# ywq/psnerf

Measured on AMD Instinct MI355X. Metric: ray-samples/sec (train step) on BEAR stage2, higher is better.
Workload: dtype f32

## Files before the change

include/psnerf_hip.h:

```cpp
#ifndef PSNERF_HIP_H
#define PSNERF_HIP_H

#include <stdint.h>

#ifdef __cplusplus
extern "C" {
#endif

#define PSN_OK 0
#define PSN_E_ARG (-1)
#define PSN_E_LAUNCH (-2)
#define PSN_E_UNSUPPORTED (-3)

const char* psn_last_error(void);
int psn_version(void);

int psn_composite_fwd(const float* alpha, const float* rgb, int64_t n_rays, int n_samples, int white_bg,
                      float* weights, float* rgb_out, float* acc_out, void* stream);
int psn_composite_bwd(const float* alpha, const float* rgb, const float* d_rgb_out, const float* d_acc_out,
                      int64_t n_rays, int n_samples, int white_bg, float* d_alpha, float* d_rgb, void* stream);

int psn_pe_encode(const float* x, int64_t n, int n_freqs, float scale, float* out, int out_stride, void* stream);
int psn_app_input(const float* p, const float* v, const float* normal, int64_t n, int n_freqs, float* out, void* stream);

// ... 206 lines not shown

int psn_stage2_loss_fwd(const float* rgb, const float* rgb_gt, int L, const float* alb, const float* alb_j, const float* wgt,
                        const float* wgt_j, int nb, const float* vis, const float* vis_gt, int V, const float* nrm,
                        const float* nrm_gt, const float* nrm_j, const unsigned char* mask_a, const unsigned char* mask_b,
                        int64_t N, int l2, const float* inv_denom, const float* weight, const float* count_dev, float* partial,
                        float* out, void* stream);
int psn_stage2_loss_bwd(const float* g_total, const float* rgb, const float* rgb_gt, int L, float k_rgb, float* d_rgb,
                        const float* alb, const float* alb_j, float k_alb, float* d_alb, float* d_alb_j, const float* wgt,
                        const float* wgt_j, int nb, float k_wgt, float* d_wgt, float* d_wgt_j, const float* vis, const float* vis_gt,
                        int V, float k_vis, float* d_vis, const float* nrm, const float* nrm_gt, const float* nrm_j, float k_nrm,
                        float k_nrmj, float* d_nrm, float* d_nrm_j, const unsigned char* mask_a, const unsigned char* mask_b,
                        int64_t N, int l2, const float* count_dev, void* stream);

int psn_stage1_loss_partial_floats(void);
int psn_stage1_loss_fwd(const float* rgb, const float* rgb_gt, const float* diff, const unsigned char* hit, const float* normal,
                        const float* normal_gt, const unsigned char* norm_mask, const float* acc, const float* mask_gt,
                        const unsigned char* mask_valid, int64_t N, int64_t n_rays, const float* weights, float* partial,
                        float* sums, float* terms, void* stream);
int psn_stage1_loss_terms(const float* sums, int64_t n_rays, const float* weights, int has_grad, int has_norm, int has_mask,
                          float* terms, void* stream);
int psn_stage1_loss_bwd(const float* g_loss, const float* sums, const float* rgb, const float* rgb_gt, const unsigned char* hit,
                        const float* normal, const float* normal_gt, const unsigned char* norm_mask, const float* acc,
                        const float* mask_gt, const unsigned char* mask_valid, int64_t N, int64_t n_rays, const float* weights,
                        float* d_rgb, float* d_diff, float* d_normal, float* d_acc, void* stream);
int psn_surface_normals_fwd(const float* g, const unsigned char* hit, int64_t N, float eps, float* norm_pred, float* diff,
                            void* stream);
int psn_surface_normals_bwd(const float* g, const unsigned char* hit, int64_t N, float eps, const float* d_norm_pred,
                            const float* d_diff, float* dg, void* stream);

#define PSN_PAIR_SUMS_MAX_V 16
#define PSN_PAIR_SUMS_MAX_CHUNKS 2048
int psn_pair_sums(const float* x, int V, int64_t Ns, int C, float* sx, float* sl_part, int* n_chunks, void* stream);
#define PSN_PAIR_GROUP_MAX 4
typedef struct { const float* x; float* sx; float* dWl; float* bias; } PsnPairSumsItem;
int64_t psn_pair_sums_group_workspace(int n_items, int V, int64_t Ns, int C);
int psn_pair_sums_group(int n_items, const PsnPairSumsItem* items, int V, int64_t Ns, int C, const float* pe_l, int64_t ld_pe, int n_pe,
                        int64_t ld_w, float* workspace, void* stream);

#define PSN_ROW_ADAM_MAX 4
typedef struct {
    float* param; const float* grad; float* exp_avg; float* exp_avg_sq;
    int64_t rows; int cols;
    float one_minus_beta1, one_minus_beta2, eps, step_size;
} PsnRowAdamItem;
int psn_row_adam(int n_items, const PsnRowAdamItem* items, const int64_t* idx, int n_idx, void* stream);
int psn_row_adam_dev(int n_items, const PsnRowAdamItem* items, const int64_t* idx, int n_idx, const float* step_sizes_dev, void* stream);

int psn_normalize_rows_fwd(const float* x, int64_t n, float eps, float* y, void* stream);
int psn_normalize_rows_bwd(const float* x, const float* g, int64_t n, float eps, float* dx, void* stream);
int psn_light_rows_fwd(const float* dir_table, const float* int_table, const int64_t* idx, int n_idx, float eps, float* dir_out,
                       float* int_out, void* stream);
int psn_light_rows_bwd(const float* dir_table, const int64_t* idx, int n_idx, int64_t n_rows, float eps, const float* g_dir,
                       const float* g_int, float* d_dir_table, float* d_int_table, void* stream);
int psn_camera_rays(const float* uv, const float* pose, const float* intrinsics, const int64_t* idx, int64_t n, float scale,
                    float* out, void* stream);
int psn_stage1_rays(const float* pix, const float* camera_mat, int k_ld, const float* world_mat, float radius2, int64_t n,
                    float* cam, float* rays, float* far, void* stream);
int psn_surface_points(const float* d_pred, const int* flags, const float* cam, const float* rays, int64_t n, float* d_i,
                       float* dists, unsigned char* obj_mask, float* points, void* stream);
int psn_stage1_targets(const float* pix, int64_t n, int h, int w, const float* img, const float* mask, const float* mask_valid,
                       const float* normal, const float* norm_mask, const float* world_mat, int use_angle, float cos_thresh,
                       float* rgb_gt, float* mask_gt, unsigned char* mask_valid_out, float* normal_gt,
                       unsigned char* norm_mask_out, void* stream);
#define PSN_COPY2D_MAX 24
typedef struct {
    const float* src; int64_t ld_src;
    float* dst; int64_t ld_dst;
    int rows, cols;
} PsnCopy2dItem;
int psn_copy2d_group(int n_items, const PsnCopy2dItem* items, void* stream);
#define PSN_COPY_BYTES_MAX 24
typedef struct { const void* src; void* dst; int64_t n_bytes; int aligned; } PsnCopyBytesItem;
int psn_copy_bytes_group(int n_items, const PsnCopyBytesItem* items, void* stream);
int psn_mask_count(const unsigned char* mask_a, const unsigned char* mask_b, int64_t n, float* out, void* stream);
int psn_surface_index(const unsigned char* mask, int64_t n, int64_t cap, int64_t* idx, float* count, void* stream);
int psn_inverse_index(const int64_t* idx, int64_t ns, int64_t n_pix, int* inv, const float* count, void* stream);
typedef struct {
    const void* images; int image_type; const float* lut;
    const unsigned char* object_mask; const unsigned char* surface_mask;
    const float* points; const float* normal; const float* visibility; const float* vis_plus; const float* light_direction;
    int64_t hw; int width;
    const int64_t* lidx; int n_lights;
    const int64_t* pix; int64_t pix0; int64_t n;
    const int64_t* vidx; int n_vis;
    float* rgb; unsigned char* object_mask_out; unsigned char* surface_mask_out; float* uv; float* points_out; float* normal_out;
    float* visibility_out; float* vis_train_gt; int64_t* sampling_idx_out; float* light_direction_out;
} PsnViewBatch;
int psn_view_batch(const PsnViewBatch* b, void* stream);
#define PSN_ADAM_MAX_SEGS 16
typedef struct {
    int64_t offset, grad_offset, n;
    float neg_step_size;
    float bias_correction2_sqrt;
} PsnAdamSeg;
int psn_adam_flat(float* param, const float* grad, float* exp_avg, float* exp_avg_sq, int n_segs, const PsnAdamSeg* segs,
                  float one_minus_beta1, float beta2, float one_minus_beta2, float eps, void* stream);
int psn_adam_flat_dev(float* param, const float* grad, float* exp_avg, float* exp_avg_sq, int n_segs, const PsnAdamSeg* segs,
                      float one_minus_beta1, float beta2, float one_minus_beta2, float eps, const float* seg_scalars_dev, void* stream);

#define PSN_WN_MAX_ITEMS 16
typedef struct {
    const float* v;
    const float* g;
    float* w;
    const float* dw;
    float* dv;
    float* dg;
    int rows, cols;
    float scale;
} PsnWnItem;
int psn_weight_norm_fwd(int n_items, const PsnWnItem* items, void* stream);
int psn_weight_norm_bwd(int n_items, const PsnWnItem* items, void* stream);

typedef struct {
    int32_t n_hidden;
    int32_t n_out;
    int32_t out_act;
    int32_t reserved;
    uint8_t has_in[PSN_MLP_MAX_LAYERS + 4];
} PsnBf16Desc;

int psn_lowp_pack(const float* W, int64_t ldw, int rows, int cols, int permuted, int n_ot, int ks0, int n_ks, int n_planes,
                  uint16_t* dst, void* stream);
int psn_lowp_pack_bias(const float* V, int64_t n, int n_pieces, uint16_t* dst, void* stream);

int psn_mlp_infer_bf16(const PsnBf16Desc* desc, const uint16_t* packed_w, const float* final_bias, const uint16_t* tab_a,
                       int64_t a_div, int64_t a_mod, const uint16_t* tab_b, int64_t b_div, int64_t b_mod, int64_t n_rows,
                       float* out, void* stream);

int psn_mlp_infer_bf16_grouped(const PsnBf16Desc* desc, const uint16_t* packed_w, const float* final_bias,
                               const uint16_t* tab_a, int64_t rows_per_group, const uint16_t* group_bias, int64_t n_groups,
                               float* out, void* stream);

int psn_mlp_infer_x3_grouped(const PsnBf16Desc* desc, const uint16_t* packed_w, const uint16_t* bias_steps, const float* final_bias,
                             const float* U, int64_t rows_per_group, const float* V, int64_t n_groups, float* out, void* stream);
int psn_mlp_infer_x3_occ(const PsnBf16Desc* desc, const uint16_t* packed_w, const uint16_t* bias_steps, const float* final_bias,
                         const float* points, int64_t n_rows, const long long* n_rows_dev, const int64_t* out_rows, int pe_octaves,
                         float pe_scale, int skip_layer, int pe_first, float* out, void* stream);
int psn_march_sweep_x3(const PsnBf16Desc* desc, const uint16_t* packed_w, const uint16_t* bias_steps, const float* final_bias,
                       const float* origin, const float* dir, const float* far, const float* u, const float* omu, float near,
                       int64_t n_rays, int n_steps, float tau, int pe_octaves, float pe_scale, int skip_layer, int pe_first,
                       int* skip, float* occ, unsigned long long* n_blocks, void* stream);


int psn_sg_shade_fwd(const float* light_dir, const float* view, const float* normal, const float* albedo,
                     const float* weights, const float* lobe, const float* light_int, int int_ch, float light_int_scalar,
                     const float* vis, int L, int64_t Ns, int nb, int specular_rgb, float* rgb, float* spec,
                     void* stream);
int psn_sg_shade_bwd(const float* light_dir, const float* view, const float* normal, const float* albedo,
                     const float* weights, const float* lobe, const float* light_int, float light_int_scalar,
                     const float* vis, int L, int64_t Ns, int nb, int specular_rgb, const float* g_rgb,
                     const float* g_spec, float* d_albedo, float* d_weights, float* d_normal, float* d_vis,
                     float* d_light_dir, float* d_light_int, float* workspace, void* stream);

int psn_mf_shade_fwd(const float* light_dir, const float* view, const float* normal, const float* albedo,
                     const float* rough, const float* light_int, float light_int_scalar, float f0, const float* vis,
                     int L, int64_t Ns, float* rgb, void* stream);
int psn_mf_shade_bwd(const float* light_dir, const float* view, const float* normal, const float* albedo,
                     const float* rough, const float* light_int, float light_int_scalar, float f0, const float* vis,
                     int L, int64_t Ns, const float* g_rgb, float* d_albedo, float* d_rough, float* d_normal,
                     float* d_vis, float* d_light_dir, float* d_light_int, float* workspace, void* stream);

#define PSN_MESH_MAX_RESOLUTION 1024
int psn_mise_collect(unsigned char* flags, int resolution, float box_size, int64_t capacity, int64_t* rows, float* points,
                     long long* count, void* stream);
int psn_mise_refine(const float* grid, unsigned char* flags, unsigned char* vox, int resolution0, int depth, double threshold,
                    long long* pending, void* stream);
int psn_grid_ffill(float* grid, int n, void* stream);
int64_t psn_mc_blocks(int n);
int psn_mc_count(const float* grid, int n, double threshold, unsigned char* code, int* block_v, int* block_t, void* stream);
int psn_mc_emit(const float* grid, int n, double threshold, const unsigned char* code, const int64_t* v_base, const int64_t* t_base,
                int64_t n_vertices, int64_t n_faces, double box_size, int* v_off, double* vertices, int64_t* faces, void* stream);

#define PSN_TRI_GRID_MAX_CELLS_PER_AXIS 256
#define PSN_TRI_GRID_MAX_FACES 2147483646LL
typedef struct {
    double lo[3];
    double hi[3];
    double cell;
    int n[3];
    int max_span;
} PsnTriGrid;
int psn_tri_grid_count(const PsnTriGrid* grid, const double* vertices, const int64_t* faces, int64_t n_faces, int* cell_count,
                       int* over_list, long long* n_over, void* stream);
int psn_tri_grid_fill(const PsnTriGrid* grid, const double* vertices, const int64_t* faces, int64_t n_faces, int* cursor,
                      int64_t n_entries, int* list, void* stream);
int psn_closest_point(const PsnTriGrid* grid, const double* vertices, const int64_t* faces, int64_t n_faces, const int* cell_start,
                      const int* list, const int* over_list, int64_t n_over, const double* points, const int64_t* order,
                      int64_t n_points, double* closest, double* dist, int64_t* tri, long long* n_tests, void* stream);

#define PSN_RAY_FIRST_HIT 0
#define PSN_RAY_ANY_HIT 1
int psn_ray_cast(const PsnTriGrid* grid, const double* vertices, const int64_t* faces, int64_t n_faces, const int* cell_start,
                 const int* list, const int* over_list, int64_t n_over, const double* origins, const double* directions,
                 const int64_t* order, int64_t n_rays, double t_min, double t_max, int mode, double* t, int64_t* tri, double* bary,
                 unsigned char* hit, long long* n_tests, void* stream);

#define PSN_OCC_LOCAL 0
#define PSN_OCC_WORLD 1
#define PSN_OCC_MAX_DIRS 1024
int psn_occlusion_rows(const PsnTriGrid* grid, const double* vertices, const int64_t* faces, int64_t n_faces, const int* cell_start,
                       const int* list, const int* over_list, int64_t n_over, const double* points, const double* normals, int64_t n_rows,
                       const double* table, int n_dirs, int mode, double bias, double t_max, int* hits, int* visible, double* ao,
                       double* bent, int* words, long long* n_tests, void* stream);

#define PSN_CROSSINGS_MAX_POINTS 137438953408LL
int psn_mesh_crossings(const PsnTriGrid* grid, const double* vertices, const int64_t* faces, int64_t n_faces, const int* cell_start,
                       const int* list, const int* over_list, int64_t n_over, const double* points, const int64_t* order,
                       int64_t n_points, int axis, int* above, int* below, int* on, long long* n_tests, void* stream);

#define PSN_CC_MAX_VERTICES 2147483646LL
#define PSN_CC_MAX_FACES 274877906944LL
#define PSN_CC_E_INDEX 1
#define PSN_CC_E_BOUND 2
int psn_cc_label(const int64_t* faces, int64_t n_faces, int64_t n_vertices, int* parent, int* labels, int* status, void* stream);
int psn_cc_stats(const double* vertices, const int64_t* faces, int64_t n_faces, int64_t n_vertices, const int* labels,
                 long long* vertex_count, long long* face_count, double* area, int* status, void* stream);
int psn_cc_flag(const int64_t* faces, int64_t n_faces, int64_t n_vertices, const int* labels, const unsigned char* keep_label,
                unsigned char* face_keep, unsigned char* vertex_keep, void* stream);
int psn_cc_compact(const double* vertices, const void* normals, int normal_bytes, const int64_t* faces, int64_t n_faces,
                   int64_t n_vertices, const unsigned char* face_keep, const unsigned char* vertex_keep, const int64_t* face_pos,
                   const int64_t* vertex_pos, int64_t n_out_faces, int64_t n_out_vertices, double* out_vertices, void* out_normals,
                   int64_t* out_faces, void* stream);

#define PSN_VC_MAX_RESOLUTION 4096
#define PSN_VC_MAX_CLUSTERS 2097151
#define PSN_VC_MAX_FACES 274877906944LL
#define PSN_VC_E_INDEX 1
#define PSN_VC_E_CLUSTER 2
int psn_vc_cell_keys(const double* vertices, int64_t n_vertices, double ox, double oy, double oz, double h, int dx, int dy, int dz,
                     int64_t* keys, void* stream);
int psn_vc_face_keys(const int64_t* faces, int64_t n_faces, int64_t n_vertices, const int64_t* cluster, int64_t* corner_keys,
                     int64_t* face_keys, int64_t* g, int* status, void* stream);
int psn_vc_solve(const double* vertices, const int64_t* faces, int64_t n_faces, int64_t n_vertices, const int64_t* vertex_order,
                 const int64_t* vertex_start, const int64_t* cell_key_sorted, const int64_t* corner_sorted,
                 const int64_t* corner_start, int64_t n_clusters, double ox, double oy, double oz, double h, int dx, int dy, int dz,
                 double regularisation, double* positions, unsigned char* clamped, void* stream);
int psn_vc_face_flags(const double* vertices, const int64_t* faces, int64_t n_faces, int64_t n_vertices, const int64_t* g,
                      const double* positions, int64_t n_clusters, const unsigned char* face_keep, unsigned char* vertex_keep,
                      unsigned char* flipped, void* stream);

#define PSN_IMG_F32 0
#define PSN_IMG_U8 1
#define PSN_IMG_MIN_EXTENT 11
#define PSN_IMG_MAX_EXTENT 16384
#define PSN_IMG_WS_SCALE_SUMS 0
#define PSN_IMG_WS_METRICS 1
#define PSN_IMG_WS_NORMAL_MAE 2
int64_t psn_img_workspace(int which, int B, int H, int W);
int psn_img_scale_sums(const void* pred, const void* gt, int image_type, const unsigned char* mask, int mask_batch, int B, int H, int W,
                       double* partial, double* sums, void* stream);
int psn_img_metrics(const void* pred, const void* gt, int image_type, const unsigned char* mask, int mask_batch, const double* scale, int B,
                    int H, int W, double* partial, double* sums, double* ssim, double* psnr, double* ssim_map, void* stream);
int psn_normal_mae(const float* pred, const float* gt, const unsigned char* mask, int mask_batch, int normalize, int B, int64_t n_pixels,
                   double* partial, double* sums, double* err_map, void* stream);

#define PSN_PS_MAX_LIGHTS 256
#define PSN_PS_MIN_LIGHTS 3
#define PSN_PS_TILE_LIGHTS 96
#define PSN_PS_MAX_PIXELS 1073741824
#define PSN_PS_PATH_AUTO 0
#define PSN_PS_PATH_TILE 1
#define PSN_PS_PATH_REFORM 2
int64_t psn_ps_workspace(int L, int64_t n_pixels);
int psn_ps_normals(const void* images, int image_type, const unsigned char* mask, const double* light_dir, const double* light_int, int L,
                   int64_t n_pixels, double low, double high, double dark, int min_lights, double cond, int path, double* normal,
                   double* albedo, unsigned char* valid, int32_t* kept, void* stream);
int psn_ps_light_intensity(const void* images, int image_type, const double* normal, const double* albedo, const unsigned char* valid,
                           const double* light_dir, int L, int64_t n_pixels, double dark, double bright, double* partial, double* sums,
                           double* intensity, void* stream);
int psn_ps_light_average(const void* images, int image_type, const unsigned char* mask, const double* relat_int, int L, int64_t n_pixels,
                         double* mean, unsigned char* mean_u8, unsigned char* norm_u8, void* stream);

#define PSN_ATLAS_MIN_CELL 4
#define PSN_ATLAS_MAX_SIZE 32768
#define PSN_ATLAS_MAX_CHANNELS 32
int psn_atlas_points(const double* vertices, int64_t n_vertices, const int64_t* faces, int64_t n_faces, const double* vertex_normals, int T,
                     int cell, int64_t f0, int64_t f1, double* points, float* points_f32, double* normals, void* stream);
int psn_atlas_scatter(const float* rows, int C, int T, int cell, int64_t n_faces, int64_t f0, int64_t f1, void* texture, int texture_type,
                      void* stream);
int psn_atlas_fill(float fill, int C, int T, int cell, int64_t n_faces, void* texture, int texture_type, void* stream);
int psn_atlas_sample(const int64_t* face, const double* bary, int64_t n_queries, const float* texture, int C, int T, int cell,
                     int64_t n_faces, double* out, void* stream);

#define PSN_HULL_MAX_RADIUS 64
#define PSN_HULL_VIEW_CHUNK 32
#define PSN_HULL_F32 0
#define PSN_HULL_F64 1
int64_t psn_mask_dilate_workspace(int V, int H, int W);
int psn_mask_dilate(const unsigned char* masks, int V, int H, int W, const int32_t* half_widths, int r, int border, int invert,
                    unsigned long long* workspace, unsigned char* out, void* stream);
int psn_hull_points(const void* points, int point_type, int64_t n_points, const double* views, int V, const unsigned char* masks, int H,
                    int W, unsigned char* keep, int32_t* carved_by, void* stream);
int psn_hull_grid(float* grid, int n, const double* axis, const double* views, int V, const unsigned char* masks, int H, int W, float value,
                  unsigned long long* count, void* stream);

#ifdef __cplusplus
}
#endif
#endif
```

psnerf_amd/csrc/common.h:

```cpp
#pragma once
#include <hip/hip_runtime.h>
#include <stdint.h>
#include <stdio.h>
#include "../../include/psnerf_hip.h"

namespace psn {

void set_error(const char* fmt, ...);

#define PSN_CHECK_ARG(cond, ...)          \
    do {                                  \
        if (!(cond)) {                    \
            psn::set_error(__VA_ARGS__);  \
            return PSN_E_ARG;             \
        }                                 \
    } while (0)

#define PSN_CHECK_LAUNCH(what)                                                   \
    do {                                                                         \
        hipError_t e__ = hipGetLastError();                                      \
        if (e__ != hipSuccess) {                                                 \
            psn::set_error("%s: launch failed: %s", what, hipGetErrorString(e__)); \
            return PSN_E_LAUNCH;                                                 \
        }                                                                        \
    } while (0)

__device__ __forceinline__ void lds_barrier() { asm volatile("s_waitcnt lgkmcnt(0)\n\ts_barrier" ::: "memory"); }


template <int OFF>
__device__ __forceinline__ void lds_dma_16(const void* gbase, unsigned lds, unsigned voff) {
    asm volatile("s_mov_b32 m0, %2\n\ts_nop 0\n\tglobal_load_lds_dwordx4 %0, %1 offset:%3" ::"v"(voff), "s"(gbase), "s"(lds), "n"(OFF));
}
__device__ __forceinline__ unsigned lds_addr(const void* p) {
    return (unsigned)(__UINTPTR_TYPE__)(__attribute__((address_space(3))) const void*)p;
}

typedef float floatx16 __attribute__((ext_vector_type(16)));
typedef float floatx4 __attribute__((ext_vector_type(4)));

__device__ __forceinline__ float relu1(float x) {
    float o;
    asm("v_max_f32 %0, 0, %1" : "=v"(o) : "v"(x));
    return o;
}

__device__ __forceinline__ float exp_neg_abs(float at) {
    const float L2E_HI = 1.44269502162933349609375f;
    const float L2E_LO = 1.925963033500011e-8f;
    float hi = -at * L2E_HI;
    float lo = fmaf(-at, L2E_HI, -hi);
    lo = fmaf(-at, L2E_LO, lo);
    float u = __builtin_amdgcn_exp2f(hi);
    return fmaf(u, lo * 0.693147182464599609375f, u);
}

__device__ __forceinline__ float log1p_unit(float u, float w, float rw) {
    return fmaf(__builtin_amdgcn_logf(w), 0.693147182464599609375f, (u - (w - 1.0f)) * rw);
}

typedef float f32x2 __attribute__((ext_vector_type(2)));
__device__ __forceinline__ f32x2 pk_fma(f32x2 a, f32x2 b, f32x2 c) { return __builtin_elementwise_fma(a, b, c); }
__device__ __forceinline__ f32x2 pk2(float a) { return f32x2{a, a}; }

template <bool WITH_SIG>
__device__ __forceinline__ void softplus100_pair(f32x2 z, f32x2& sp, f32x2& s) {
    const float L2E = 1.44269502162933349609375f;
    const float LN2_HI = 0.693147182464599609375f;
    const float LN2_LO = -1.904654323148236e-9f;
    const float C_HI = 0.00999999977648258209228515625f;
    const float C_LO = 2.2351741811588166e-10f;
    const f32x2 t = z * 100.0f;
    const f32x2 nat = {fminf(t.x, -t.x), fminf(t.y, -t.y)};
    const f32x2 hi = nat * L2E;
    f32x2 r = pk_fma(-hi, pk2(LN2_HI), nat);
    r = pk_fma(-hi, pk2(LN2_LO), r);
    const f32x2 u0 = {__builtin_amdgcn_exp2f(hi.x), __builtin_amdgcn_exp2f(hi.y)};
    const f32x2 u = pk_fma(u0, r, u0);
    const f32x2 w = u + 1.0f;
    const f32x2 lw = {__builtin_amdgcn_logf(w.x), __builtin_amdgcn_logf(w.y)};
    const f32x2 c = w - 1.0f;
    const f32x2 d = u - c;
    f32x2 rw;
    if constexpr (WITH_SIG) {
        const f32x2 r0 = {__builtin_amdgcn_rcpf(w.x), __builtin_amdgcn_rcpf(w.y)};
        rw = pk_fma(pk_fma(-w, r0, pk2(1.0f)), r0, r0);
        const f32x2 ur = u * rw;
        s = f32x2{t.x >= 0.0f ? rw.x : ur.x, t.y >= 0.0f ? rw.y : ur.y};
    } else {
        rw = pk_fma(c, pk_fma(c, pk2(0.5f), pk2(-1.0f)), pk2(1.0f));
    }
    const f32x2 l = pk_fma(lw, pk2(LN2_HI), d * rw);
    const f32x2 zr = {relu1(z.x), relu1(z.y)};
    sp = pk_fma(l, pk2(C_HI), pk_fma(l, pk2(C_LO), zr));
}
__device__ __forceinline__ void softplus100_sig(float z, float& sp, float& s) {
    f32x2 a, b;
    softplus100_pair<true>(f32x2{z, z}, a, b);
    sp = a.x; s = b.x;
}
__device__ __forceinline__ float softplus100(float z) {
    f32x2 a, b;
    softplus100_pair<false>(f32x2{z, z}, a, b);
    return a.x;
}
__device__ __forceinline__ float sigmoidf_(float x) {
    float u = exp_neg_abs(fabsf(x));
    float r = 1.0f / (1.0f + u);
    return x >= 0.0f ? r : u * r;
}

}
```

psnerf_amd/csrc/loss.hip:

```cpp
#include "common.h"

namespace psn {

struct LossArgs {
    const float* rgb; const float* rgb_gt; int L;
    const float* alb; const float* alb_j;
    const float* wgt; const float* wgt_j; int nb;
    const float* vis; const float* vis_gt; int V;
    const float* nrm; const float* nrm_gt; const float* nrm_j;
    const unsigned char* mask_a; const unsigned char* mask_b;
    int64_t N;
    int l2;
    float* partial;
    const float* g_total;
    const float* count_dev;
    float k_rgb, k_alb, k_wgt, k_vis, k_nrm, k_nrmj;
    float* d_rgb; float* d_alb; float* d_alb_j; float* d_wgt; float* d_wgt_j; float* d_vis; float* d_nrm; float* d_nrm_j;
};

__device__ __forceinline__ float img_term(float a, float b, int l2) { const float d = a - b; return l2 ? d * d : fabsf(d); }
__device__ __forceinline__ float img_grad(float a, float b, int l2) {
    const float d = a - b;
    return l2 ? 2.0f * d : (d > 0.0f ? 1.0f : (d < 0.0f ? -1.0f : 0.0f));
}

__global__ __launch_bounds__(256) void stage2_loss_fwd_kernel(LossArgs a) {
    float s[6] = {0.f, 0.f, 0.f, 0.f, 0.f, 0.f};
    const int lc = (a.L + gridDim.y - 1) / gridDim.y;
    const int l0 = blockIdx.y * lc, l1 = min(a.L, l0 + lc);
    for (int64_t n = (int64_t)blockIdx.x * 256 + threadIdx.x; n < a.N; n += (int64_t)gridDim.x * 256) {
        if (!(a.mask_a[n] && a.mask_b[n])) continue;
        if (a.rgb != nullptr) {
#pragma unroll 4
            for (int l = l0; l < l1; ++l) {
                const float* p = a.rgb + ((int64_t)l * a.N + n) * 3;
                const float* q = a.rgb_gt + ((int64_t)l * a.N + n) * 3;
                s[0] += img_term(p[0], q[0], a.l2) + img_term(p[1], q[1], a.l2) + img_term(p[2], q[2], a.l2);
            }
        }
        if (blockIdx.y != 0) continue;
        if (a.alb != nullptr) {
#pragma unroll
            for (int c = 0; c < 3; ++c) s[1] += fabsf(a.alb[n * 3 + c] - a.alb_j[n * 3 + c]);
        }
        if (a.wgt != nullptr) {
            for (int k = 0; k < a.nb; ++k) s[2] += fabsf(a.wgt[n * a.nb + k] - a.wgt_j[n * a.nb + k]);
        }
        if (a.vis != nullptr) {
            for (int v = 0; v < a.V; ++v) s[3] += img_term(a.vis[((int64_t)v * a.N + n) * 3], a.vis_gt[(int64_t)v * a.N + n], a.l2);
        }
        if (a.nrm != nullptr) {
            const float gx = a.nrm_gt[n * 3], gy = a.nrm_gt[n * 3 + 1], gz = a.nrm_gt[n * 3 + 2];
            const float inv = 1.0f / fmaxf(sqrtf(gx * gx + gy * gy + gz * gz), 1e-12f);
            const float dx = a.nrm[n * 3] - gx * inv, dy = a.nrm[n * 3 + 1] - gy * inv, dz = a.nrm[n * 3 + 2] - gz * inv;
            s[4] += dx * dx + dy * dy + dz * dz;
            if (a.nrm_j != nullptr) {
#pragma unroll
                for (int c = 0; c < 3; ++c) s[5] += fabsf(a.nrm[n * 3 + c] - a.nrm_j[n * 3 + c]);
            }
        }
    }
    __shared__ float red[4][6];
#pragma unroll
    for (int i = 0; i < 6; ++i) {
        float v = s[i];
#pragma unroll
        for (int o = 32; o > 0; o >>= 1) v += __shfl_xor(v, o, 64);
        if ((threadIdx.x & 63) == 0) red[threadIdx.x >> 6][i] = v;
    }
    __syncthreads();
    if (threadIdx.x < 6)
        a.partial[((int64_t)blockIdx.y * gridDim.x + blockIdx.x) * 6 + threadIdx.x] = (red[0][threadIdx.x] + red[1][threadIdx.x]) + (red[2][threadIdx.x] + red[3][threadIdx.x]);
}

struct LossScale { float inv_denom[6]; float weight[6]; const float* count_dev; };
__global__ __launch_bounds__(256) void stage2_loss_final_kernel(const float* __restrict__ partial, int blocks, LossScale sc,
                                                               float* __restrict__ out) {
    __shared__ float red[32][8];
    const int i = threadIdx.x & 7, j = threadIdx.x >> 3;
    float s = 0.f;
    if (i < 6)
        for (int b = j; b < blocks; b += 32) s += partial[(int64_t)b * 6 + i];
    red[j][i] = s;
    __syncthreads();
    if (threadIdx.x < 8) {
        float tot = 0.f;
#pragma unroll
        for (int k = 0; k < 32; ++k) tot += red[k][threadIdx.x];
        const float cnt = sc.count_dev != nullptr ? sc.count_dev[0] : 1.0f;
        const float term = (threadIdx.x < 6 && cnt > 0.0f) ? tot * sc.inv_denom[threadIdx.x] / cnt : 0.f;
        if (threadIdx.x < 6) out[threadIdx.x] = term;
        float w = threadIdx.x < 6 ? sc.weight[threadIdx.x] * term : 0.f;
#pragma unroll
        for (int o = 4; o > 0; o >>= 1) w += __shfl_xor(w, o, 64);
        if (threadIdx.x == 0) out[6] = w;
    }
}

__global__ __launch_bounds__(256) void pair_sums_kernel(const float* __restrict__ x, int V, int64_t Ns, int C, int rows_per_block,
                                                        float* __restrict__ sx, float* __restrict__ sl_part) {
    const int cg = threadIdx.x & 63, rl = threadIdx.x >> 6;
    const int64_t n0 = (int64_t)blockIdx.x * rows_per_block, n1 = min(Ns, n0 + rows_per_block);
    const bool live = 4 * cg < C;
    float4 sl[PSN_PAIR_SUMS_MAX_V];
#pragma unroll
    for (int v = 0; v < PSN_PAIR_SUMS_MAX_V; ++v) sl[v] = make_float4(0.f, 0.f, 0.f, 0.f);
    if (live) {
        for (int64_t n = n0 + rl; n < n1; n += 4) {
            float4 acc = make_float4(0.f, 0.f, 0.f, 0.f);
#pragma unroll
            for (int v = 0; v < PSN_PAIR_SUMS_MAX_V; ++v) {
                if (v < V) {
                    const float4 t = *reinterpret_cast<const float4*>(x + ((int64_t)v * Ns + n) * C + 4 * cg);
                    acc.x += t.x; acc.y += t.y; acc.z += t.z; acc.w += t.w;
                    sl[v].x += t.x; sl[v].y += t.y; sl[v].z += t.z; sl[v].w += t.w;
                }
            }
            *reinterpret_cast<float4*>(sx + n * C + 4 * cg) = acc;
        }
#pragma unroll
        for (int v = 0; v < PSN_PAIR_SUMS_MAX_V; ++v)
            if (v < V) *reinterpret_cast<float4*>(sl_part + (((int64_t)blockIdx.x * 4 + rl) * V + v) * C + 4 * cg) = sl[v];
    }
}

struct PairGroupArgs { PsnPairSumsItem it[PSN_PAIR_GROUP_MAX]; int V; int64_t Ns; int C; int rows_per_block; int chunks; float* part;
                       const float* pe_l; int64_t ld_pe; int n_pe; int64_t ld_w;
                       int slices; float* part2; };
__global__ __launch_bounds__(256) void pair_group_sums_kernel(PairGroupArgs a) {
    const PsnPairSumsItem it = a.it[blockIdx.y];
    const int V = a.V, C = a.C;
    const int64_t Ns = a.Ns;
    const int cg = threadIdx.x & 63, rl = threadIdx.x >> 6;
    const int64_t n0 = (int64_t)blockIdx.x * a.rows_per_block, n1 = min(Ns, n0 + a.rows_per_block);
    const bool live = 4 * cg < C;
    float4 sl[PSN_PAIR_SUMS_MAX_V];
#pragma unroll
    for (int v = 0; v < PSN_PAIR_SUMS_MAX_V; ++v) sl[v] = make_float4(0.f, 0.f, 0.f, 0.f);
    if (live) {
        for (int64_t n = n0 + rl; n < n1; n += 4) {
            float4 acc = make_float4(0.f, 0.f, 0.f, 0.f);
#pragma unroll
            for (int v = 0; v < PSN_PAIR_SUMS_MAX_V; ++v) {
                if (v < V) {
                    const float4 t = *reinterpret_cast<const float4*>(it.x + ((int64_t)v * Ns + n) * C + 4 * cg);
                    acc.x += t.x; acc.y += t.y; acc.z += t.z; acc.w += t.w;
                    sl[v].x += t.x; sl[v].y += t.y; sl[v].z += t.z; sl[v].w += t.w;
                }
            }
            *reinterpret_cast<float4*>(it.sx + n * C + 4 * cg) = acc;
        }
    }
    __shared__ float4 red[3][64];
    float* dst = a.part + (((int64_t)blockIdx.y * a.chunks + blockIdx.x) * V) * C;
#pragma unroll
    for (int v = 0; v < PSN_PAIR_SUMS_MAX_V; ++v) {
        if (v < V) {
            __syncthreads();
            if (rl > 0) red[rl - 1][cg] = sl[v];
            __syncthreads();
            if (rl == 0 && live) {
                float4 t = sl[v];
#pragma unroll
                for (int q = 0; q < 3; ++q) { const float4 o = red[q][cg]; t.x += o.x; t.y += o.y; t.z += o.z; t.w += o.w; }
                *reinterpret_cast<float4*>(dst + (int64_t)v * C + 4 * cg) = t;
            }
        }
    }
}
__global__ __launch_bounds__(1024) void pair_group_final_kernel(PairGroupArgs a) {
    const PsnPairSumsItem it = a.it[blockIdx.y];
    const int V = a.V, C = a.C;
    const int c0 = blockIdx.x * 64;
    const int cl = threadIdx.x & 63, v = threadIdx.x >> 6;
    __shared__ float dzl[PSN_PAIR_SUMS_MAX_V][64];
    __shared__ float pel[PSN_PAIR_SUMS_MAX_V][64];
    int ch = 0, ch_end = a.chunks;
    if (a.slices > 1) {
        const int per = (a.chunks + a.slices - 1) / a.slices;
        ch = blockIdx.z * per;
        ch_end = min(a.chunks, ch + per);
    }
    float s = 0.0f;
    if (v < V && c0 + cl < C) {
        const float* p = a.part + ((int64_t)blockIdx.y * a.chunks * V + v) * C + c0 + cl;
        const int64_t step = (int64_t)V * C;
        for (; ch + 4 <= ch_end; ch += 4) {
            const float t0 = p[(int64_t)ch * step], t1 = p[(int64_t)(ch + 1) * step], t2 = p[(int64_t)(ch + 2) * step], t3 = p[(int64_t)(ch + 3) * step];
            s += t0; s += t1; s += t2; s += t3;
        }
        for (; ch < ch_end; ++ch) s += p[(int64_t)ch * step];
        if (a.slices > 1) a.part2[(((int64_t)blockIdx.y * a.slices + blockIdx.z) * V + v) * C + c0 + cl] = s;
    }
    if (a.slices > 1) return;
    dzl[v][cl] = s;
    pel[v][cl] = (v < V && cl < a.n_pe) ? a.pe_l[(int64_t)v * a.ld_pe + cl] : 0.0f;
    __syncthreads();
    for (int e = threadIdx.x; e < 64 * a.n_pe; e += 1024) {
        const int c = e / a.n_pe, k = e - c * a.n_pe;
        if (c0 + c < C) {
            float w = 0.0f;
            for (int u = 0; u < V; ++u) w += dzl[u][c] * pel[u][k];
            it.dWl[(int64_t)(c0 + c) * a.ld_w + k] = w;
        }
    }
    if (it.bias != nullptr && threadIdx.x < 64 && c0 + (int)threadIdx.x < C) {
        float b = 0.0f;
        for (int u = 0; u < V; ++u) b += dzl[u][threadIdx.x];
        it.bias[c0 + threadIdx.x] = b;
    }
}

__global__ __launch_bounds__(256) void stage2_loss_bwd_kernel(LossArgs a) {
    float g = a.g_total[0];
    if (a.count_dev != nullptr) {
        const float cnt = a.count_dev[0];
        g = cnt > 0.0f ? g / cnt : 0.0f;
    }
    const int lc = (a.L + gridDim.y - 1) / gridDim.y;
    const int l0 = blockIdx.y * lc, l1 = min(a.L, l0 + lc);
    for (int64_t n = (int64_t)blockIdx.x * 256 + threadIdx.x; n < a.N; n += (int64_t)gridDim.x * 256) {
        const bool m = a.mask_a[n] && a.mask_b[n];
        if (a.d_rgb != nullptr) {
            const float k = g * a.k_rgb;
#pragma unroll 4
            for (int l = l0; l < l1; ++l) {
                const int64_t o = ((int64_t)l * a.N + n) * 3;
#pragma unroll
                for (int c = 0; c < 3; ++c) a.d_rgb[o + c] = m ? k * img_grad(a.rgb[o + c], a.rgb_gt[o + c], a.l2) : 0.f;
            }
        }
        if (blockIdx.y != 0) continue;
        if (a.d_alb != nullptr) {
            const float k = g * a.k_alb;
#pragma unroll
            for (int c = 0; c < 3; ++c) {
                const float v = m ? k * img_grad(a.alb[n * 3 + c], a.alb_j[n * 3 + c], 0) : 0.f;
                a.d_alb[n * 3 + c] = v;
                a.d_alb_j[n * 3 + c] = -v;
            }
        }
        if (a.d_wgt != nullptr) {
            const float k = g * a.k_wgt;
            for (int q = 0; q < a.nb; ++q) {
                const float v = m ? k * img_grad(a.wgt[n * a.nb + q], a.wgt_j[n * a.nb + q], 0) : 0.f;
                a.d_wgt[n * a.nb + q] = v;
                a.d_wgt_j[n * a.nb + q] = -v;
            }
        }
        if (a.d_vis != nullptr) {
            const float k = g * a.k_vis;
            for (int v = 0; v < a.V; ++v) {
                const int64_t o = ((int64_t)v * a.N + n) * 3;
                a.d_vis[o] = m ? k * img_grad(a.vis[o], a.vis_gt[(int64_t)v * a.N + n], a.l2) : 0.f;
                a.d_vis[o + 1] = 0.f;
                a.d_vis[o + 2] = 0.f;
            }
        }
        if (a.d_nrm != nullptr) {
            float gn[3] = {0.f, 0.f, 0.f}, gj[3] = {0.f, 0.f, 0.f};
            if (m) {
                const float gx = a.nrm_gt[n * 3], gy = a.nrm_gt[n * 3 + 1], gz = a.nrm_gt[n * 3 + 2];
                const float inv = 1.0f / fmaxf(sqrtf(gx * gx + gy * gy + gz * gz), 1e-12f);
                const float t[3] = {gx * inv, gy * inv, gz * inv};
#pragma unroll
                for (int c = 0; c < 3; ++c) gn[c] = g * a.k_nrm * 2.0f * (a.nrm[n * 3 + c] - t[c]);
                if (a.nrm_j != nullptr) {
#pragma unroll
                    for (int c = 0; c < 3; ++c) {
                        const float v = g * a.k_nrmj * img_grad(a.nrm[n * 3 + c], a.nrm_j[n * 3 + c], 0);
                        gn[c] += v;
                        gj[c] = -v;
                    }
                }
            }
#pragma unroll
            for (int c = 0; c < 3; ++c) {
                a.d_nrm[n * 3 + c] = gn[c];
                if (a.d_nrm_j != nullptr) a.d_nrm_j[n * 3 + c] = gj[c];
            }
        }
    }
}

constexpr int kLossBlocksX = 256, kLossChunksY = 8;

}

extern "C" int psn_stage2_loss_fwd(const float* rgb, const float* rgb_gt, int L, const float* alb, const float* alb_j,
                                   const float* wgt, const float* wgt_j, int nb, const float* vis, const float* vis_gt, int V,
                                   const float* nrm, const float* nrm_gt, const float* nrm_j, const unsigned char* mask_a,
                                   const unsigned char* mask_b, int64_t N, int l2, const float* inv_denom, const float* weight,
                                   const float* count_dev, float* partial, float* out, void* stream) {
    using namespace psn;
    PSN_CHECK_ARG(mask_a && mask_b && partial && out && inv_denom && weight, "stage2_loss_fwd: null pointer");
    PSN_CHECK_ARG((rgb == nullptr || rgb_gt) && (alb == nullptr || alb_j) && (wgt == nullptr || (wgt_j && nb > 0)) &&
                  (vis == nullptr || vis_gt) && (nrm == nullptr || nrm_gt), "stage2_loss_fwd: incomplete term");
    LossArgs a = {};
    a.rgb = rgb; a.rgb_gt = rgb_gt; a.L = L; a.alb = alb; a.alb_j = alb_j; a.wgt = wgt; a.wgt_j = wgt_j; a.nb = nb;
    a.vis = vis; a.vis_gt = vis_gt; a.V = V; a.nrm = nrm; a.nrm_gt = nrm_gt; a.nrm_j = nrm_j; a.mask_a = mask_a; a.mask_b = mask_b;
    a.N = N; a.l2 = l2; a.partial = partial;
    int bx = (int)((N + 255) / 256);
    if (bx > kLossBlocksX) bx = kLossBlocksX;
    if (bx < 1) bx = 1;
    const int by = (rgb != nullptr && L >= 2 * kLossChunksY) ? kLossChunksY : 1;
    hipLaunchKernelGGL(stage2_loss_fwd_kernel, dim3(bx, by), dim3(256), 0, (hipStream_t)stream, a);
    PSN_CHECK_LAUNCH("stage2_loss_fwd");
    LossScale sc;
    for (int i = 0; i < 6; ++i) { sc.inv_denom[i] = inv_denom[i]; sc.weight[i] = weight[i]; }
    sc.count_dev = count_dev;
    hipLaunchKernelGGL(stage2_loss_final_kernel, dim3(1), dim3(256), 0, (hipStream_t)stream, partial, bx * by, sc, out);
    PSN_CHECK_LAUNCH("stage2_loss_fwd (final)");
    return PSN_OK;
}

extern "C" int psn_stage2_loss_bwd(const float* g_total, const float* rgb, const float* rgb_gt, int L, float k_rgb, float* d_rgb,
                                   const float* alb, const float* alb_j, float k_alb, float* d_alb, float* d_alb_j,
                                   const float* wgt, const float* wgt_j, int nb, float k_wgt, float* d_wgt, float* d_wgt_j,
                                   const float* vis, const float* vis_gt, int V, float k_vis, float* d_vis,
                                   const float* nrm, const float* nrm_gt, const float* nrm_j, float k_nrm, float k_nrmj, float* d_nrm,
                                   float* d_nrm_j, const unsigned char* mask_a, const unsigned char* mask_b, int64_t N, int l2,
                                   const float* count_dev, void* stream) {
    using namespace psn;
    PSN_CHECK_ARG(g_total && mask_a && mask_b, "stage2_loss_bwd: null pointer");
    LossArgs a = {};
    a.g_total = g_total; a.count_dev = count_dev; a.rgb = rgb; a.rgb_gt = rgb_gt; a.L = L; a.k_rgb = k_rgb; a.d_rgb = d_rgb;
    a.alb = alb; a.alb_j = alb_j; a.k_alb = k_alb; a.d_alb = d_alb; a.d_alb_j = d_alb_j;
    a.wgt = wgt; a.wgt_j = wgt_j; a.nb = nb; a.k_wgt = k_wgt; a.d_wgt = d_wgt; a.d_wgt_j = d_wgt_j;
    a.vis = vis; a.vis_gt = vis_gt; a.V = V; a.k_vis = k_vis; a.d_vis = d_vis;
    a.nrm = nrm; a.nrm_gt = nrm_gt; a.nrm_j = nrm_j; a.k_nrm = k_nrm; a.k_nrmj = k_nrmj; a.d_nrm = d_nrm; a.d_nrm_j = d_nrm_j;
    a.mask_a = mask_a; a.mask_b = mask_b; a.N = N; a.l2 = l2;
    PSN_CHECK_ARG((d_rgb == nullptr || (rgb && rgb_gt)) && (d_alb == nullptr || (alb && alb_j && d_alb_j)) &&
                  (d_wgt == nullptr || (wgt && wgt_j && d_wgt_j)) && (d_vis == nullptr || (vis && vis_gt)) &&
                  (d_nrm == nullptr || (nrm && nrm_gt)), "stage2_loss_bwd: incomplete term");
    if (N <= 0) return PSN_OK;
    int64_t blocks = (N + 255) / 256;
    if (blocks > 1024) blocks = 1024;
    const int by = (d_rgb != nullptr && L >= 2 * kLossChunksY) ? kLossChunksY : 1;
    hipLaunchKernelGGL(stage2_loss_bwd_kernel, dim3((unsigned)blocks, by), dim3(256), 0, (hipStream_t)stream, a);
    PSN_CHECK_LAUNCH("stage2_loss_bwd");
    return PSN_OK;
}

namespace psn {
struct RowAdamArgs { PsnRowAdamItem it[PSN_ROW_ADAM_MAX]; const int64_t* idx; int n_idx; int n;
                     const float* dev; };
__global__ __launch_bounds__(256) void row_adam_kernel(RowAdamArgs a) {
    const int item = blockIdx.y;
    if (item >= a.n) return;
    PsnRowAdamItem it = a.it[item];
    if (a.dev != nullptr) it.step_size = a.dev[item];
    const int64_t r = (int64_t)blockIdx.x * 256 + threadIdx.x;
    __shared__ int64_t sidx[256];
    bool touched = false;
    for (int i0 = 0; i0 < a.n_idx; i0 += 256) {
        const int m = a.n_idx - i0 < 256 ? a.n_idx - i0 : 256;
        __syncthreads();
        if ((int)threadIdx.x < m) sidx[threadIdx.x] = a.idx[i0 + threadIdx.x];
        __syncthreads();
        for (int j = 0; j < m; ++j) touched = touched || sidx[j] == r;
    }
    if (r >= it.rows || !touched) return;
    for (int c = 0; c < it.cols; ++c) {
        const int64_t e = r * it.cols + c;
        const float g = it.grad[e];
        float m = it.exp_avg[e], v = it.exp_avg_sq[e];
        m += (g - m) * it.one_minus_beta1;
        v += (g * g - v) * it.one_minus_beta2;
        it.exp_avg[e] = m;
        it.exp_avg_sq[e] = v;
        it.param[e] += (m / (sqrtf(v) + it.eps)) * (-it.step_size);
    }
}
}

static int row_adam_impl(int n_items, const PsnRowAdamItem* items, const int64_t* idx, int n_idx, const float* step_sizes_dev, void* stream) {
    using namespace psn;
    PSN_CHECK_ARG(items && (idx || n_idx == 0) && n_items >= 1 && n_items <= PSN_ROW_ADAM_MAX && n_idx >= 0, "row_adam: bad arguments");
    RowAdamArgs a = {};
    a.dev = step_sizes_dev;
    int64_t max_rows = 0;
    for (int i = 0; i < n_items; ++i) {
        PSN_CHECK_ARG(items[i].param && items[i].grad && items[i].exp_avg && items[i].exp_avg_sq && items[i].rows >= 0 && items[i].cols >= 1,
                      "row_adam: item %d", i);
        a.it[i] = items[i];
        if (items[i].rows > max_rows) max_rows = items[i].rows;
    }
    a.idx = idx; a.n_idx = n_idx; a.n = n_items;
    if (max_rows <= 0 || n_idx == 0) return PSN_OK;
    hipLaunchKernelGGL(row_adam_kernel, dim3((unsigned)((max_rows + 255) / 256), n_items), dim3(256), 0, (hipStream_t)stream, a);
    PSN_CHECK_LAUNCH("row_adam");
    return PSN_OK;
}

extern "C" int psn_row_adam(int n_items, const PsnRowAdamItem* items, const int64_t* idx, int n_idx, void* stream) {
    return row_adam_impl(n_items, items, idx, n_idx, nullptr, stream);
}

extern "C" int psn_row_adam_dev(int n_items, const PsnRowAdamItem* items, const int64_t* idx, int n_idx, const float* step_sizes_dev,
                                void* stream) {
    PSN_CHECK_ARG(step_sizes_dev != nullptr, "row_adam_dev: step_sizes_dev is required");
    return row_adam_impl(n_items, items, idx, n_idx, step_sizes_dev, stream);
}

constexpr int kPairSlices = 32;

extern "C" int64_t psn_pair_sums_group_workspace(int n_items, int V, int64_t Ns, int C) {
    int rows = 16;
    int64_t chunks = (Ns + rows - 1) / rows;
    while (chunks > PSN_PAIR_SUMS_MAX_CHUNKS) { rows *= 2; chunks = (Ns + rows - 1) / rows; }
    return (int64_t)n_items * ((chunks > 0 ? chunks : 1) + kPairSlices) * V * C;
}

extern "C" int psn_pair_sums_group(int n_items, const PsnPairSumsItem* items, int V, int64_t Ns, int C, const float* pe_l, int64_t ld_pe,
                                   int n_pe, int64_t ld_w, float* workspace, void* stream) {
    using namespace psn;
    PSN_CHECK_ARG(items && pe_l && workspace && n_items >= 1 && n_items <= PSN_PAIR_GROUP_MAX, "pair_sums_group: bad arguments (n_items=%d)", n_items);
    PSN_CHECK_ARG(V >= 1 && V <= PSN_PAIR_SUMS_MAX_V && C >= 4 && C <= 256 && C % 4 == 0 && Ns >= 0, "pair_sums_group: V=%d C=%d", V, C);
    PSN_CHECK_ARG(n_pe >= 1 && n_pe <= 64 && ld_pe >= n_pe && ld_w >= n_pe, "pair_sums_group: n_pe=%d", n_pe);
    PairGroupArgs a = {};
    for (int i = 0; i < n_items; ++i) {
        PSN_CHECK_ARG(items[i].x && items[i].sx && items[i].dWl && ((((uintptr_t)items[i].x | (uintptr_t)items[i].sx)) & 15) == 0, "pair_sums_group: item %d", i);
        a.it[i] = items[i];
    }
    int rows = 16;
    int64_t chunks = (Ns + rows - 1) / rows;
    while (chunks > PSN_PAIR_SUMS_MAX_CHUNKS) { rows *= 2; chunks = (Ns + rows - 1) / rows; }
    a.V = V; a.Ns = Ns; a.C = C; a.rows_per_block = rows; a.chunks = (int)chunks; a.part = workspace;
    a.pe_l = pe_l; a.ld_pe = ld_pe; a.n_pe = n_pe; a.ld_w = ld_w;
    PSN_CHECK_ARG((((uintptr_t)workspace) & 15) == 0, "pair_sums_group: workspace must be 16-byte aligned");
    if (chunks > 0) {
        hipLaunchKernelGGL(pair_group_sums_kernel, dim3((unsigned)chunks, n_items), dim3(256), 0, (hipStream_t)stream, a);
        PSN_CHECK_LAUNCH("pair_sums_group (sums)");
    }
    if (chunks > 128) {
        a.slices = kPairSlices;
        a.part2 = workspace + (int64_t)n_items * chunks * V * C;
        hipLaunchKernelGGL(pair_group_final_kernel, dim3((unsigned)((C + 63) / 64), n_items, kPairSlices), dim3(1024), 0, (hipStream_t)stream, a);
        PSN_CHECK_LAUNCH("pair_sums_group (slices)");
        a.part = a.part2; a.chunks = kPairSlices; a.slices = 1; a.part2 = nullptr;
    }
    hipLaunchKernelGGL(pair_group_final_kernel, dim3((unsigned)((C + 63) / 64), n_items), dim3(1024), 0, (hipStream_t)stream, a);
    PSN_CHECK_LAUNCH("pair_sums_group (final)");
    return PSN_OK;
}

extern "C" int psn_pair_sums(const float* x, int V, int64_t Ns, int C, float* sx, float* sl_part, int* n_chunks, void* stream) {
    using namespace psn;
    PSN_CHECK_ARG(x && sx && sl_part && n_chunks, "pair_sums: null pointer");
    PSN_CHECK_ARG(V >= 1 && V <= PSN_PAIR_SUMS_MAX_V && C >= 1 && C <= 256 && Ns >= 0, "pair_sums: V=%d C=%d (V <= %d, C <= 256)", V, C, PSN_PAIR_SUMS_MAX_V);
    PSN_CHECK_ARG(C % 4 == 0 && (((uintptr_t)x | (uintptr_t)sx | (uintptr_t)sl_part) & 15) == 0, "pair_sums: C must be a multiple of 4, buffers 16-byte aligned");
    int rows = 32;
    int64_t chunks = (Ns + rows - 1) / rows;
    while (chunks * 4 > PSN_PAIR_SUMS_MAX_CHUNKS) { rows *= 2; chunks = (Ns + rows - 1) / rows; }
    *n_chunks = (int)chunks * 4;
    if (Ns <= 0) return PSN_OK;
    hipLaunchKernelGGL(pair_sums_kernel, dim3((unsigned)chunks), dim3(256), 0, (hipStream_t)stream, x, V, Ns, C, rows, sx, sl_part);
    PSN_CHECK_LAUNCH("pair_sums");
    return PSN_OK;
}
```

psnerf_amd/csrc/shade.hip:

```cpp
#include "common.h"

namespace psn {

constexpr int kShadeThreads = 64;

constexpr int kMaxBasis = 9;

struct ShadeArgs {
    const float* light_dir;
    const float* view;
    const float* normal;
    const float* albedo;
    const float* weights;
    const float* lobe;
    const float* light_int;
    int int_ch;
    float light_int_scalar;
    const float* vis;
    int L, nb, specular_rgb;
    int64_t Ns;
};

__device__ __forceinline__ float wave_sum_f(float v) {
#pragma unroll
    for (int d = 32; d >= 1; d >>= 1) v += __shfl_xor(v, d, 64);
    return v;
}

struct PointCtx {
    float v[3], n[3], alb[3];
    float w[3][kMaxBasis];
    float lam[kMaxBasis];
};

__device__ __forceinline__ void load_point(const ShadeArgs& a, int64_t n, bool ok, PointCtx& p) {
    const int nw = a.specular_rgb ? 3 * a.nb : a.nb;
#pragma unroll
    for (int c = 0; c < 3; ++c) {
        p.v[c] = ok ? a.view[n * 3 + c] : 0.f;
        p.n[c] = ok ? a.normal[n * 3 + c] : 0.f;
        p.alb[c] = ok ? a.albedo[n * 3 + c] : 0.f;
    }
#pragma unroll
    for (int k = 0; k < kMaxBasis; ++k) {
        p.lam[k] = k < a.nb ? fmaxf(a.lobe[k], 0.0f) : 0.0f;
#pragma unroll
        for (int c = 0; c < 3; ++c) {
            float wv = 0.f;
            if (ok && k < a.nb) wv = a.specular_rgb ? a.weights[n * nw + c * a.nb + k] : a.weights[n * nw + k];
            p.w[c][k] = wv;
        }
    }
}

struct Fwd {
    float h[3], inv_norm, hn, D[kMaxBasis], s[3], brdf[3], cosv, vcl, I[3], pre[3];
};

__device__ __forceinline__ void shade_one(const ShadeArgs& a, const PointCtx& p, const float l[3], const float I[3],
                                          float vis, bool has_vis, Fwd& f) {
    float u0 = l[0] + p.v[0], u1 = l[1] + p.v[1], u2 = l[2] + p.v[2];
    float nrm = sqrtf(u0 * u0 + u1 * u1 + u2 * u2);
    float den = fmaxf(nrm, 1e-12f);
    f.inv_norm = 1.0f / den;
    f.h[0] = u0 / den;
    f.h[1] = u1 / den;
    f.h[2] = u2 / den;
    f.hn = f.h[0] * p.n[0] + f.h[1] * p.n[1] + f.h[2] * p.n[2];
    float t = f.hn - 1.0f;
    float s0 = 0.f, s1 = 0.f, s2 = 0.f;
#pragma unroll
    for (int k = 0; k < kMaxBasis; ++k) {
        float d = (k < a.nb) ? expf(p.lam[k] * t) : 0.0f;
        f.D[k] = d;
        s0 += p.w[0][k] * d;
        s1 += p.w[1][k] * d;
        s2 += p.w[2][k] * d;
    }
    f.s[0] = s0;
    f.s[1] = a.specular_rgb ? s1 : s0;
    f.s[2] = a.specular_rgb ? s2 : s0;
    f.cosv = l[0] * p.n[0] + l[1] * p.n[1] + l[2] * p.n[2];
    f.vcl = has_vis ? fminf(fmaxf(vis, 0.0f), 1.0f) : 1.0f;
#pragma unroll
    for (int c = 0; c < 3; ++c) {
        f.I[c] = I[c];
        f.brdf[c] = p.alb[c] + fmaxf(f.s[c], 0.0f);
        float x = f.brdf[c] * I[c] * f.cosv;
        if (has_vis) x = x * f.vcl;
        f.pre[c] = x;
    }
}

constexpr int kSgPhases = 4;
__global__ __launch_bounds__(kShadeThreads * kSgPhases) void sg_shade_fwd_kernel(ShadeArgs a, float* __restrict__ rgb, float* __restrict__ spec) {
    const int64_t n = (int64_t)blockIdx.x * kShadeThreads + (threadIdx.x & (kShadeThreads - 1));
    const int phase = threadIdx.x / kShadeThreads;
    const bool ok = n < a.Ns;
    PointCtx p;
    load_point(a, n, ok, p);
    const bool has_vis = a.vis != nullptr;
    const int sc = a.specular_rgb ? 3 : 1;
    for (int l = phase; l < a.L; l += kSgPhases) {
        float ld[3] = {a.light_dir[l * 3 + 0], a.light_dir[l * 3 + 1], a.light_dir[l * 3 + 2]};
        float I[3];
#pragma unroll
        for (int c = 0; c < 3; ++c)
            I[c] = a.light_int != nullptr ? a.light_int[l * a.int_ch + (a.int_ch == 3 ? c : 0)] : a.light_int_scalar;
        const int64_t row = (int64_t)l * a.Ns + n;
        float vis = (has_vis && ok) ? a.vis[row] : 1.0f;
        Fwd f;
        shade_one(a, p, ld, I, vis, has_vis, f);
        if (ok) {
#pragma unroll
            for (int c = 0; c < 3; ++c) rgb[row * 3 + c] = fminf(fmaxf(f.pre[c], 0.0f), 1.0f);
            if (a.specular_rgb) {
#pragma unroll
                for (int c = 0; c < 3; ++c) spec[row * 3 + c] = fmaxf(f.s[c], 0.0f);
            } else {
                spec[row] = fmaxf(f.s[0], 0.0f);
            }
        }
    }
    (void)sc;
}

__global__ __launch_bounds__(kShadeThreads * kSgPhases) void sg_shade_bwd_kernel(ShadeArgs a, const float* __restrict__ g_rgb,
                                                           const float* __restrict__ g_spec,
                                                           float* __restrict__ d_albedo, float* __restrict__ d_weights,
                                                           float* __restrict__ d_normal, float* __restrict__ d_vis,
                                                           float* __restrict__ d_light_partial) {
    const int64_t n = (int64_t)blockIdx.x * kShadeThreads + (threadIdx.x & (kShadeThreads - 1));
    const int phase = threadIdx.x / kShadeThreads;
    const bool ok = n < a.Ns;
    const int lane = threadIdx.x & 63;
    PointCtx p;
    load_point(a, n, ok, p);
    const bool has_vis = a.vis != nullptr;
    float dalb[3] = {0.f, 0.f, 0.f}, dn[3] = {0.f, 0.f, 0.f};
    float dw[3][kMaxBasis];
#pragma unroll
    for (int c = 0; c < 3; ++c)
#pragma unroll
        for (int k = 0; k < kMaxBasis; ++k) dw[c][k] = 0.f;

    for (int l = phase; l < a.L; l += kSgPhases) {
        float ld[3] = {a.light_dir[l * 3 + 0], a.light_dir[l * 3 + 1], a.light_dir[l * 3 + 2]};
        float I[3];
#pragma unroll
        for (int c = 0; c < 3; ++c)
            I[c] = a.light_int != nullptr ? a.light_int[l * a.int_ch + (a.int_ch == 3 ? c : 0)] : a.light_int_scalar;
        const int64_t row = (int64_t)l * a.Ns + n;
        float vis = (has_vis && ok) ? a.vis[row] : 1.0f;
        Fwd f;
        shade_one(a, p, ld, I, vis, has_vis, f);
        float dl[3] = {0.f, 0.f, 0.f}, dI = 0.f, dcos = 0.f, dvcl = 0.f, ds[3];
        if (ok) {
#pragma unroll
            for (int c = 0; c < 3; ++c) {
                float g = g_rgb[row * 3 + c];
                float gp = (f.pre[c] >= 0.0f && f.pre[c] <= 1.0f) ? g : 0.0f;
                float dbrdf = gp * I[c] * f.cosv * f.vcl;
                dI += gp * f.brdf[c] * f.cosv * f.vcl;
                dcos += gp * f.brdf[c] * I[c] * f.vcl;
                dvcl += gp * f.brdf[c] * I[c] * f.cosv;
                dalb[c] += dbrdf;
                float dspec = dbrdf;
                if (g_spec != nullptr) dspec += a.specular_rgb ? g_spec[row * 3 + c] : (c == 0 ? g_spec[row] : 0.0f);
                ds[c] = f.s[c] >= 0.0f ? dspec : 0.0f;
            }
            if (!a.specular_rgb) {
                ds[0] = ds[0] + ds[1] + ds[2];
                ds[1] = 0.f;
                ds[2] = 0.f;
            }
            float dhn = 0.f;
#pragma unroll
            for (int k = 0; k < kMaxBasis; ++k) {
                float dD = ds[0] * p.w[0][k] + ds[1] * p.w[1][k] + ds[2] * p.w[2][k];
                dhn += dD * p.lam[k] * f.D[k];
                dw[0][k] += ds[0] * f.D[k];
                dw[1][k] += ds[1] * f.D[k];
                dw[2][k] += ds[2] * f.D[k];
            }
            float dh[3];
#pragma unroll
            for (int c = 0; c < 3; ++c) {
                dh[c] = dhn * p.n[c];
                dn[c] += dhn * f.h[c] + dcos * ld[c];
                dl[c] = dcos * p.n[c];
            }
            float hd = f.h[0] * dh[0] + f.h[1] * dh[1] + f.h[2] * dh[2];
#pragma unroll
            for (int c = 0; c < 3; ++c) dl[c] += (dh[c] - f.h[c] * hd) * f.inv_norm;
            if (d_vis != nullptr) d_vis[row] = (vis >= 0.0f && vis <= 1.0f) ? dvcl : 0.0f;
        }
        float r0 = wave_sum_f(dl[0]), r1 = wave_sum_f(dl[1]), r2 = wave_sum_f(dl[2]), r3 = wave_sum_f(dI);
        if (lane == 0) *reinterpret_cast<float4*>(d_light_partial + ((int64_t)blockIdx.x * a.L + l) * 4) = make_float4(r0, r1, r2, r3);
    }
    __shared__ float pred[kSgPhases - 1][6 + 3 * kMaxBasis][kShadeThreads];
    if (phase > 0) {
#pragma unroll
        for (int c = 0; c < 3; ++c) {
            pred[phase - 1][c][lane] = dalb[c];
            pred[phase - 1][3 + c][lane] = dn[c];
        }
#pragma unroll
        for (int c = 0; c < 3; ++c)
#pragma unroll
            for (int k = 0; k < kMaxBasis; ++k) pred[phase - 1][6 + c * kMaxBasis + k][lane] = dw[c][k];
    }
    __syncthreads();
    if (phase == 0) {
#pragma unroll
        for (int c = 0; c < 3; ++c) {
            dalb[c] = (dalb[c] + pred[0][c][lane]) + (pred[1][c][lane] + pred[2][c][lane]);
            dn[c] = (dn[c] + pred[0][3 + c][lane]) + (pred[1][3 + c][lane] + pred[2][3 + c][lane]);
        }
#pragma unroll
        for (int c = 0; c < 3; ++c)
#pragma unroll
            for (int k = 0; k < kMaxBasis; ++k)
                dw[c][k] = (dw[c][k] + pred[0][6 + c * kMaxBasis + k][lane]) + (pred[1][6 + c * kMaxBasis + k][lane] + pred[2][6 + c * kMaxBasis + k][lane]);
    }
    if (ok && phase == 0) {
        const int nw = a.specular_rgb ? 3 * a.nb : a.nb;
#pragma unroll
        for (int c = 0; c < 3; ++c) {
            d_albedo[n * 3 + c] = dalb[c];
            d_normal[n * 3 + c] = dn[c];
        }
#pragma unroll
        for (int k = 0; k < kMaxBasis; ++k) {
            if (k < a.nb) {
                if (a.specular_rgb) {
#pragma unroll
                    for (int c = 0; c < 3; ++c) d_weights[n * nw + c * a.nb + k] = dw[c][k];
                } else {
                    d_weights[n * nw + k] = dw[0][k];
                }
            }
        }
    }
}

__global__ __launch_bounds__(256) void sg_light_reduce_kernel(const float* __restrict__ partial, int n_blocks, int L,
                                                              float* __restrict__ d_light_dir,
                                                              float* __restrict__ d_light_int) {
    __shared__ float red[3][64];
    const int i = blockIdx.x * 64 + (threadIdx.x & 63), ph = threadIdx.x >> 6;
    float s = 0.f;
    if (i < L * 4)
        for (int b = ph; b < n_blocks; b += 4) s += partial[(int64_t)b * L * 4 + i];
    if (ph > 0) red[ph - 1][threadIdx.x & 63] = s;
    __syncthreads();
    if (ph > 0 || i >= L * 4) return;
    s = (s + red[0][threadIdx.x]) + (red[1][threadIdx.x] + red[2][threadIdx.x]);
    const int l = i >> 2, c = i & 3;
    if (c < 3) d_light_dir[l * 3 + c] = s;
    else if (d_light_int != nullptr) d_light_int[l] = s;
}

struct MfArgs {
    const float* light_dir;
    const float* view;
    const float* normal;
    const float* albedo;
    const float* rough;
    const float* light_int;
    float light_int_scalar, f0;
    const float* vis;
    int L;
    int64_t Ns;
};

__device__ __forceinline__ float dnn(float x, float y) {
    float a = x / (y + 1e-6f);
    return (isinf(a) || isnan(a)) ? 0.0f : a;
}
__device__ __forceinline__ bool dnn_ok(float x, float y) {
    float a = x / (y + 1e-6f);
    return !(isinf(a) || isnan(a));
}
__device__ __forceinline__ void normalize_eps(const float x[3], float eps, float out[3], float& inv) {
    float n = sqrtf(x[0] * x[0] + x[1] * x[1] + x[2] * x[2]);
    float d = fmaxf(n, eps);
    inv = 1.0f / d;
    out[0] = x[0] / d;
    out[1] = x[1] / d;
    out[2] = x[2] / d;
}
__device__ __forceinline__ void normalize_bwd(const float y[3], float inv, bool clamped, const float dy[3], float dx[3]) {
    if (clamped) {
        dx[0] = dy[0] * inv; dx[1] = dy[1] * inv; dx[2] = dy[2] * inv;
    } else {
        float yd = y[0] * dy[0] + y[1] * dy[1] + y[2] * dy[2];
        dx[0] = (dy[0] - y[0] * yd) * inv;
        dx[1] = (dy[1] - y[1] * yd) * inv;
        dx[2] = (dy[2] - y[2] * yd) * inv;
    }
}

struct MfFwd {
    float lh[3], inv_l, hh[3], inv_h, cm, cv, lhh, ln, a2, F, D, G, fgd, den2, mf, cosv, vcl;
    float t_m, den_d, t_v_raw, t_v, sq, den_g, chi_d, chi_g;
    bool cl_l, cl_h, ok_tm, ok_d, ok_tv, ok_g, ok_mf;
};

__device__ __forceinline__ void mf_one(const float l[3], const float vh[3], const float nh[3], const float nraw[3],
                                       float rough, float f0, float vis, bool has_vis, MfFwd& f) {
    const float PI = 3.14159265358979323846f;
    normalize_eps(l, 1e-6f, f.lh, f.inv_l);
    f.cl_l = sqrtf(l[0] * l[0] + l[1] * l[1] + l[2] * l[2]) < 1e-6f;
    float u[3] = {f.lh[0] + vh[0], f.lh[1] + vh[1], f.lh[2] + vh[2]};
    normalize_eps(u, 1e-6f, f.hh, f.inv_h);
    f.cl_h = sqrtf(u[0] * u[0] + u[1] * u[1] + u[2] * u[2]) < 1e-6f;
    f.lhh = f.lh[0] * f.hh[0] + f.lh[1] * f.hh[1] + f.lh[2] * f.hh[2];
    float om = 1.0f - f.lhh;
    f.F = f0 + (1.0f - f0) * (om * om * om * om * om);
    float alpha = rough * rough;
    f.a2 = alpha * alpha;
    f.cm = f.hh[0] * nh[0] + f.hh[1] * nh[1] + f.hh[2] * nh[2];
    f.chi_d = f.cm > 0.0f ? 1.0f : 0.0f;
    float cm2 = f.cm * f.cm;
    f.ok_tm = dnn_ok(1.0f - cm2, cm2);
    f.t_m = dnn(1.0f - cm2, cm2);
    float q = f.a2 + f.t_m;
    f.den_d = PI * (cm2 * cm2) * (q * q);
    f.ok_d = dnn_ok(f.a2 * f.chi_d, f.den_d);
    f.D = dnn(f.a2 * f.chi_d, f.den_d);
    f.cv = nh[0] * vh[0] + nh[1] * vh[1] + nh[2] * vh[2];
    float hv = f.hh[0] * vh[0] + f.hh[1] * vh[1] + f.hh[2] * vh[2];
    f.chi_g = dnn(hv, f.cv) > 0.0f ? 1.0f : 0.0f;
    float cv2 = fminf(fmaxf(f.cv * f.cv, 0.0f), 1.0f);
    f.ok_tv = dnn_ok(1.0f - cv2, cv2);
    f.t_v_raw = dnn(1.0f - cv2, cv2);
    f.t_v = fmaxf(f.t_v_raw, 0.0f);
    f.sq = sqrtf(1.0f + f.a2 * f.t_v);
    f.den_g = 1.0f + f.sq;
    f.ok_g = dnn_ok(f.chi_g * 2.0f, f.den_g);
    f.G = dnn(f.chi_g * 2.0f, f.den_g);
    f.ln = f.lh[0] * nh[0] + f.lh[1] * nh[1] + f.lh[2] * nh[2];
    f.den2 = 4.0f * fabsf(f.ln) * fabsf(f.cv);
    f.fgd = f.F * f.G * f.D;
    f.ok_mf = dnn_ok(f.fgd, f.den2);
    f.mf = dnn(f.fgd, f.den2);
    f.cosv = l[0] * nraw[0] + l[1] * nraw[1] + l[2] * nraw[2];
    f.vcl = has_vis ? fminf(fmaxf(vis, 0.0f), 1.0f) : 1.0f;
}

__global__ __launch_bounds__(kShadeThreads) void mf_shade_fwd_kernel(MfArgs a, float* __restrict__ rgb) {
    const int64_t n = (int64_t)blockIdx.x * kShadeThreads + threadIdx.x;
    const bool ok = n < a.Ns;
    float v[3], nr[3], alb[3], vh[3], nh[3], inv;
#pragma unroll
    for (int c = 0; c < 3; ++c) {
        v[c] = ok ? a.view[n * 3 + c] : 1.f;
        nr[c] = ok ? a.normal[n * 3 + c] : 1.f;
        alb[c] = ok ? a.albedo[n * 3 + c] : 0.f;
    }
    const float rough = ok ? a.rough[n] : 0.5f;
    normalize_eps(v, 1e-6f, vh, inv);
    normalize_eps(nr, 1e-6f, nh, inv);
    const bool has_vis = a.vis != nullptr;
    for (int l = 0; l < a.L; ++l) {
        float ld[3] = {a.light_dir[l * 3 + 0], a.light_dir[l * 3 + 1], a.light_dir[l * 3 + 2]};
        float I = a.light_int != nullptr ? a.light_int[l] : a.light_int_scalar;
        const int64_t row = (int64_t)l * a.Ns + n;
        float vis = (has_vis && ok) ? a.vis[row] : 1.0f;
        MfFwd f;
        mf_one(ld, vh, nh, nr, rough, a.f0, vis, has_vis, f);
        if (ok) {
#pragma unroll
            for (int c = 0; c < 3; ++c) {
                float x = (f.mf + alb[c] / 3.14159265358979323846f) * I * f.cosv;
                if (has_vis) x = x * f.vcl;
                rgb[row * 3 + c] = fminf(fmaxf(x, 0.0f), 1.0f);
            }
        }
    }
}

__global__ __launch_bounds__(kShadeThreads) void mf_shade_bwd_kernel(MfArgs a, const float* __restrict__ g_rgb,
                                                           float* __restrict__ d_albedo, float* __restrict__ d_rough,
                                                           float* __restrict__ d_normal, float* __restrict__ d_vis,
                                                           float* __restrict__ d_light_partial) {
    const float PI = 3.14159265358979323846f;
    const int64_t n = (int64_t)blockIdx.x * kShadeThreads + threadIdx.x;
    const bool ok = n < a.Ns;
    const int lane = threadIdx.x & 63;
    float v[3], nr[3], alb[3], vh[3], nh[3], inv_v, inv_n;
#pragma unroll
    for (int c = 0; c < 3; ++c) {
        v[c] = ok ? a.view[n * 3 + c] : 1.f;
        nr[c] = ok ? a.normal[n * 3 + c] : 1.f;
        alb[c] = ok ? a.albedo[n * 3 + c] : 0.f;
// ... 9 lines not shown
        float I = a.light_int != nullptr ? a.light_int[l] : a.light_int_scalar;
        const int64_t row = (int64_t)l * a.Ns + n;
        float vis = (has_vis && ok) ? a.vis[row] : 1.0f;
        MfFwd f;
        mf_one(ld, vh, nh, nr, rough, a.f0, vis, has_vis, f);
        float dl[3] = {0.f, 0.f, 0.f}, dI = 0.f;
        if (ok) {
            float dmf = 0.f, dcos = 0.f, dvcl = 0.f;
#pragma unroll
            for (int c = 0; c < 3; ++c) {
                float brdf = f.mf + alb[c] / PI;
                float pre = brdf * I * f.cosv;
                if (has_vis) pre = pre * f.vcl;
                float g = g_rgb[row * 3 + c];
                float gp = (pre >= 0.0f && pre <= 1.0f) ? g : 0.0f;
                float dbrdf = gp * I * f.cosv * f.vcl;
                dI += gp * brdf * f.cosv * f.vcl;
                dcos += gp * brdf * I * f.vcl;
                dvcl += gp * brdf * I * f.cosv;
                dalb[c] += dbrdf / PI;
                dmf += dbrdf;
            }
            float dfgd = 0.f, dden2 = 0.f;
            if (f.ok_mf) {
                float r = 1.0f / (f.den2 + 1e-6f);
                dfgd = dmf * r;
                dden2 = -dmf * f.fgd * r * r;
            }
            float dF = dfgd * f.G * f.D, dG = dfgd * f.F * f.D, dD = dfgd * f.F * f.G;
            float sgn_ln = f.ln > 0.f ? 1.f : (f.ln < 0.f ? -1.f : 0.f);
            float sgn_cv = f.cv > 0.f ? 1.f : (f.cv < 0.f ? -1.f : 0.f);
            float dln = dden2 * 4.0f * sgn_ln * fabsf(f.cv);
            float dcv = dden2 * 4.0f * fabsf(f.ln) * sgn_cv;
            float dlhh = dF * (-5.0f) * (1.0f - a.f0) * ((1.0f - f.lhh) * (1.0f - f.lhh) * (1.0f - f.lhh) * (1.0f - f.lhh));
            float dcm = 0.f, da2_l = 0.f;
            if (f.ok_d) {
                float r = 1.0f / (f.den_d + 1e-6f);
                float dden_d = -dD * f.a2 * f.chi_d * r * r;
                da2_l += dD * f.chi_d * r;
                float cm2 = f.cm * f.cm;
                float q = f.a2 + f.t_m;
                float dq = dden_d * PI * cm2 * cm2 * 2.0f * q;
                float dcm2 = dden_d * PI * 2.0f * cm2 * q * q;
                da2_l += dq;
                if (f.ok_tm) {
                    float rr = 1.0f / (cm2 + 1e-6f);
                    dcm2 += dq * (-(rr) - (1.0f - cm2) * rr * rr);
                }
                dcm += dcm2 * 2.0f * f.cm;
            }
            if (f.ok_g) {
                float r = 1.0f / (f.den_g + 1e-6f);
                float dden_g = -dG * 2.0f * f.chi_g * r * r;
                float dsq = dden_g;
                float dinner = f.sq > 0.f ? dsq * 0.5f / f.sq : 0.f;
                da2_l += dinner * f.t_v;
                float dtv = dinner * f.a2;
                if (f.t_v_raw >= 0.0f && f.ok_tv) {
                    float c2 = f.cv * f.cv;
                    if (c2 >= 0.0f && c2 <= 1.0f) {
                        float cv2 = fminf(fmaxf(c2, 0.0f), 1.0f);
                        float rr = 1.0f / (cv2 + 1e-6f);
                        float dcv2 = dtv * (-(rr) - (1.0f - cv2) * rr * rr);
                        dcv += dcv2 * 2.0f * f.cv;
                    }
                }
            }
            da2 += da2_l;
            float dhh[3], dlh[3];
#pragma unroll
            for (int c = 0; c < 3; ++c) {
                dnh[c] += dcm * f.hh[c] + dcv * vh[c] + dln * f.lh[c];
                dhh[c] = dcm * nh[c] + dlhh * f.lh[c];
                dlh[c] = dlhh * f.hh[c] + dln * nh[c];
                dnraw[c] += dcos * ld[c];
                dl[c] = dcos * nr[c];
            }
            float du[3];
            normalize_bwd(f.hh, f.inv_h, f.cl_h, dhh, du);
#pragma unroll
            for (int c = 0; c < 3; ++c) dlh[c] += du[c];
            float dlraw[3];
            normalize_bwd(f.lh, f.inv_l, f.cl_l, dlh, dlraw);
#pragma unroll
            for (int c = 0; c < 3; ++c) dl[c] += dlraw[c];
            if (d_vis != nullptr) d_vis[row] = (vis >= 0.0f && vis <= 1.0f) ? dvcl : 0.0f;
        }
        float r0 = wave_sum_f(dl[0]), r1 = wave_sum_f(dl[1]), r2 = wave_sum_f(dl[2]), r3 = wave_sum_f(dI);
        if (lane == 0) *reinterpret_cast<float4*>(d_light_partial + ((int64_t)blockIdx.x * a.L + l) * 4) = make_float4(r0, r1, r2, r3);
    }
    if (ok) {
        float dn_from_nh[3];
        normalize_bwd(nh, inv_n, cl_n, dnh, dn_from_nh);
#pragma unroll
        for (int c = 0; c < 3; ++c) {
            d_albedo[n * 3 + c] = dalb[c];
            d_normal[n * 3 + c] = dnraw[c] + dn_from_nh[c];
        }
        d_rough[n] = da2 * 4.0f * rough * rough * rough;
    }
}

static int fill_args(ShadeArgs& a, const float* light_dir, const float* view, const float* normal, const float* albedo,
                     const float* weights, const float* lobe, const float* light_int, int int_ch, float light_int_scalar,
                     const float* vis, int L, int64_t Ns, int nb, int specular_rgb) {
    PSN_CHECK_ARG(light_dir && view && normal && albedo && weights && lobe, "sg_shade: null pointer");
    PSN_CHECK_ARG(L >= 1 && Ns >= 0 && nb >= 1 && nb <= kMaxBasis, "sg_shade: L=%d nb=%d", L, nb);
    a.light_dir = light_dir; a.view = view; a.normal = normal; a.albedo = albedo; a.weights = weights; a.lobe = lobe;
    PSN_CHECK_ARG(int_ch == 1 || int_ch == 3, "sg_shade: light intensity must have 1 or 3 channels");
    a.light_int = light_int; a.int_ch = int_ch; a.light_int_scalar = light_int_scalar; a.vis = vis; a.L = L; a.Ns = Ns; a.nb = nb;
    a.specular_rgb = specular_rgb ? 1 : 0;
    return PSN_OK;
}

}

extern "C" int psn_sg_shade_fwd(const float* light_dir, const float* view, const float* normal, const float* albedo,
                                const float* weights, const float* lobe, const float* light_int, int int_ch,
                                float light_int_scalar, const float* vis, int L, int64_t Ns, int nb, int specular_rgb,
                                float* rgb, float* spec, void* stream) {
    using namespace psn;
    ShadeArgs a;
    int rc = fill_args(a, light_dir, view, normal, albedo, weights, lobe, light_int, int_ch, light_int_scalar, vis, L, Ns, nb, specular_rgb);
    if (rc) return rc;
    PSN_CHECK_ARG(rgb && spec, "sg_shade_fwd: null output");
    if (Ns == 0) return PSN_OK;
    hipLaunchKernelGGL(sg_shade_fwd_kernel, dim3((unsigned)((Ns + kShadeThreads - 1) / kShadeThreads)), dim3(kShadeThreads * kSgPhases), 0, (hipStream_t)stream, a, rgb, spec);
    PSN_CHECK_LAUNCH("sg_shade_fwd");
    return PSN_OK;
}

extern "C" int psn_sg_shade_bwd(const float* light_dir, const float* view, const float* normal, const float* albedo,
                                const float* weights, const float* lobe, const float* light_int,
                                float light_int_scalar, const float* vis, int L, int64_t Ns, int nb, int specular_rgb,
                                const float* g_rgb, const float* g_spec, float* d_albedo, float* d_weights,
                                float* d_normal, float* d_vis, float* d_light_dir, float* d_light_int,
                                float* workspace, void* stream) {
    using namespace psn;
    ShadeArgs a;
    int rc = fill_args(a, light_dir, view, normal, albedo, weights, lobe, light_int, 1, light_int_scalar, vis, L, Ns, nb, specular_rgb);
    if (rc) return rc;
    PSN_CHECK_ARG(g_rgb && d_albedo && d_weights && d_normal && d_light_dir && workspace, "sg_shade_bwd: null pointer");
    if (Ns == 0) return PSN_OK;
    const int n_blocks = (int)((Ns + kShadeThreads - 1) / kShadeThreads);
    hipLaunchKernelGGL(sg_shade_bwd_kernel, dim3(n_blocks), dim3(kShadeThreads * kSgPhases), 0, (hipStream_t)stream, a, g_rgb, g_spec, d_albedo,
                       d_weights, d_normal, d_vis, workspace);
    PSN_CHECK_LAUNCH("sg_shade_bwd");
    hipLaunchKernelGGL(sg_light_reduce_kernel, dim3((L * 4 + 63) / 64), dim3(256), 0, (hipStream_t)stream, workspace,
                       n_blocks, L, d_light_dir, d_light_int);
    PSN_CHECK_LAUNCH("sg_shade_bwd light reduce");
    return PSN_OK;
}

extern "C" int psn_mf_shade_fwd(const float* light_dir, const float* view, const float* normal, const float* albedo,
                                const float* rough, const float* light_int, float light_int_scalar, float f0,
                                const float* vis, int L, int64_t Ns, float* rgb, void* stream) {
    using namespace psn;
    PSN_CHECK_ARG(light_dir && view && normal && albedo && rough && rgb, "mf_shade_fwd: null pointer");
    PSN_CHECK_ARG(L >= 1 && Ns >= 0, "mf_shade_fwd: L=%d", L);
    if (Ns == 0) return PSN_OK;
    MfArgs a{light_dir, view, normal, albedo, rough, light_int, light_int_scalar, f0, vis, L, Ns};
    hipLaunchKernelGGL(mf_shade_fwd_kernel, dim3((unsigned)((Ns + kShadeThreads - 1) / kShadeThreads)), dim3(kShadeThreads), 0, (hipStream_t)stream, a, rgb);
    PSN_CHECK_LAUNCH("mf_shade_fwd");
    return PSN_OK;
}

extern "C" int psn_mf_shade_bwd(const float* light_dir, const float* view, const float* normal, const float* albedo,
                                const float* rough, const float* light_int, float light_int_scalar, float f0,
                                const float* vis, int L, int64_t Ns, const float* g_rgb, float* d_albedo,
                                float* d_rough, float* d_normal, float* d_vis, float* d_light_dir, float* d_light_int,
                                float* workspace, void* stream) {
    using namespace psn;
    PSN_CHECK_ARG(light_dir && view && normal && albedo && rough && g_rgb && d_albedo && d_rough && d_normal &&
                  d_light_dir && workspace, "mf_shade_bwd: null pointer");
    PSN_CHECK_ARG(L >= 1 && Ns >= 0, "mf_shade_bwd: L=%d", L);
    if (Ns == 0) return PSN_OK;
    MfArgs a{light_dir, view, normal, albedo, rough, light_int, light_int_scalar, f0, vis, L, Ns};
    const int n_blocks = (int)((Ns + kShadeThreads - 1) / kShadeThreads);
    hipLaunchKernelGGL(mf_shade_bwd_kernel, dim3(n_blocks), dim3(kShadeThreads), 0, (hipStream_t)stream, a, g_rgb, d_albedo, d_rough,
                       d_normal, d_vis, workspace);
    PSN_CHECK_LAUNCH("mf_shade_bwd");
    hipLaunchKernelGGL(sg_light_reduce_kernel, dim3((L * 4 + 63) / 64), dim3(256), 0, (hipStream_t)stream, workspace,
                       n_blocks, L, d_light_dir, d_light_int);
    PSN_CHECK_LAUNCH("mf_shade_bwd light reduce");
    return PSN_OK;
}
```

psnerf_amd/hip.py:

```python
import ctypes
import os

import torch

from . import cabi

_HERE = os.path.dirname(os.path.abspath(__file__))
LIB_PATH = os.path.join(_HERE, 'libpsnerf_hip.so')

if not os.path.exists(LIB_PATH):
    raise ImportError(
        'psnerf_amd: %s is missing. Build it with `python -m psnerf_amd.build` (hipcc, gfx950). '
        'There is no fallback path.' % LIB_PATH)
_lib = ctypes.CDLL(LIB_PATH)

HEADER_PATH = os.path.join(_HERE, '..', 'include', 'psnerf_hip.h')
if not os.path.exists(HEADER_PATH):
    raise ImportError('psnerf_amd: %s is missing: the binding is derived from it. There is no fallback path.' % HEADER_PATH)

_constants, _structs, SIGNATURES = cabi.parse(HEADER_PATH)
globals().update({_k[len('PSN_'):]: _v for _k, _v in _constants.items()})
globals().update(_structs)
MAX_LAYERS = MLP_MAX_LAYERS
for _name, (_res, _args) in SIGNATURES.items():
# ... 1061 lines not shown
        _check(_lib.psn_weight_norm_bwd(n, ctypes.addressof(arr), _stream()), 'weight_norm_bwd')
    return dvs, dgs


def lowp_pack(W, permuted, n_ot, ks0, n_ks, dst, planes=1):
    assert W.dim() == 2 and W.stride(1) == 1 and W.is_cuda and W.dtype == torch.float32
    assert dst.dtype == torch.bfloat16 and dst.is_contiguous() and dst.numel() == n_ks * n_ot * planes * 512
    _check(_lib.psn_lowp_pack(W.data_ptr(), W.stride(0), W.shape[0], W.shape[1], int(permuted), n_ot, ks0, n_ks, planes,
                              dst.data_ptr(), _stream()), 'lowp_pack')


def lowp_pack_bias(V, pieces, dst=None):
    assert V.is_cuda and V.dtype == torch.float32 and V.is_contiguous() and V.dim() == 2 and V.shape[1] == 256
    if dst is None:
        dst = torch.empty(V.shape[0], 4096, device=V.device, dtype=torch.bfloat16)
    assert dst.dtype == torch.bfloat16 and dst.is_contiguous() and dst.numel() == V.shape[0] * 4096
    _check(_lib.psn_lowp_pack_bias(V.data_ptr(), V.shape[0], pieces, dst.data_ptr(), _stream()), 'lowp_pack_bias')
    return dst


def _bf16_stream(t, name):
    if not (t.is_cuda and t.dtype == torch.bfloat16 and t.is_contiguous()):
        raise RuntimeError('%s: must be a contiguous bfloat16 HIP tensor' % name)
    return t.data_ptr()


def _n_in(desc):
    return sum(1 for l in range(desc.n_hidden) if desc.has_in[l])


def _bf16_table(t, name):
    if t is not None and (t.dim() != 2 or t.shape[1] != 64):
        raise RuntimeError('%s: must be a contiguous [n, 64] bfloat16 HIP tensor' % name)
    return _tptr(t, name, torch.bfloat16, allow_none=True)


def mlp_infer_bf16(desc, packed_w, final_bias, tab_a, a_div, a_mod, tab_b, b_div, b_mod, n_rows, out=None):
    if out is None:
        out = torch.empty(n_rows, desc.n_out, device=packed_w.device, dtype=torch.float32)
    assert packed_w.dtype == torch.bfloat16 and packed_w.is_cuda and packed_w.is_contiguous()
    assert final_bias.numel() == 32
    ptrs = (_tptr(final_bias, 'final_bias'), _bf16_table(tab_a, 'tab_a'), _bf16_table(tab_b, 'tab_b'), _tptr(out, 'out'))
    if n_rows == 0:
        return out
    with _Prof('mlp_infer_bf16', n_rows):
        _check(_lib.psn_mlp_infer_bf16(ctypes.byref(desc), packed_w.data_ptr(), ptrs[0], ptrs[1], a_div, a_mod, ptrs[2], b_div, b_mod,
                                       n_rows, ptrs[3], _stream()), 'mlp_infer_bf16')
    return out


def mlp_infer_bf16_grouped(desc, packed_w, final_bias, tab_a, group_bias, n_groups, out=None):
    rows = tab_a.shape[0]
    if out is None:
        out = torch.empty(n_groups * rows, desc.n_out, device=packed_w.device, dtype=torch.float32)
    assert packed_w.dtype == torch.bfloat16 and packed_w.is_cuda and packed_w.is_contiguous()
    assert final_bias.numel() == 32
    n_in = _n_in(desc)
    if not (group_bias.is_cuda and group_bias.dtype == torch.bfloat16 and group_bias.is_contiguous()
            and group_bias.numel() == n_groups * n_in * 4096):
        raise RuntimeError('group_bias: must be a contiguous [n_groups * %d, 4096] bfloat16 HIP tensor' % n_in)
    assert out.numel() == n_groups * rows * desc.n_out
    ptrs = (_tptr(final_bias, 'final_bias'), _bf16_table(tab_a, 'tab_a'), _tptr(out, 'out'))
    if n_groups * rows == 0:
        return out
    with _Prof('mlp_infer_bf16', n_groups * rows):
        _check(_lib.psn_mlp_infer_bf16_grouped(ctypes.byref(desc), packed_w.data_ptr(), ptrs[0], ptrs[1], rows, group_bias.data_ptr(), n_groups,
                                               ptrs[2], _stream()), 'mlp_infer_bf16_grouped')
    return out


X3_KS = 8 * 3 * 512


def mlp_infer_x3_grouped(desc, packed_w, bias_steps, final_bias, U, V, out=None, macs_per_row=None):
    rows, n_groups = U.shape[0], V.shape[0]
    if out is None:
        out = torch.empty(n_groups * rows, desc.n_out, device=packed_w.device, dtype=torch.float32)
    n_in = _n_in(desc)
    streams = (_bf16_stream(packed_w, 'packed_w'), _bf16_stream(bias_steps, 'bias_steps'))
    assert U.shape[1] == V.shape[1] == n_in * 256 and bias_steps.numel() == desc.n_hidden * 4096
    assert final_bias.numel() == 32 and out.numel() == n_groups * rows * desc.n_out
    ptrs = (_tptr(final_bias, 'final_bias'), _tptr(U, 'U'), _tptr(V, 'V'), _tptr(out, 'out'))
    if n_groups * rows == 0:
        return out
    with _Prof('mlp_infer_x3', n_groups * rows, None if macs_per_row is None else 2.0 * macs_per_row * n_groups * rows):
        _check(_lib.psn_mlp_infer_x3_grouped(ctypes.byref(desc), streams[0], streams[1], ptrs[0],
                                             ptrs[1], rows, ptrs[2], n_groups, ptrs[3], _stream()), 'mlp_infer_x3_grouped')
    return out


def mlp_infer_x3_occ(desc, packed_w, bias_steps, final_bias, points, pe_octaves, pe_scale, skip_layer, pe_first, out=None,
                     n_rows_dev=None, out_rows=None, macs_per_row=None):
    Q = points.shape[0]
    assert points.dim() == 2 and points.shape[1] == 3
    if out is None:
        assert out_rows is None
        out = torch.empty(Q, desc.n_out, device=points.device, dtype=torch.float32)
    streams = (_bf16_stream(packed_w, 'packed_w'), _bf16_stream(bias_steps, 'bias_steps'))
    assert bias_steps.numel() == desc.n_hidden * 4096 and final_bias.numel() == 32 and desc.n_out == 1
    if n_rows_dev is not None:
        assert n_rows_dev.is_cuda and n_rows_dev.dtype == torch.int64 and n_rows_dev.numel() == 1
    if out_rows is not None:
        assert out_rows.is_cuda and out_rows.dtype == torch.int64 and out_rows.is_contiguous() and out_rows.numel() >= Q
    ptrs = (_tptr(final_bias, 'final_bias'), _tptr(points, 'points'), _tptr(out, 'out'))
    if Q == 0:
        return out
    with _Prof('mlp_infer_x3_occ', Q, None if macs_per_row is None else 2.0 * macs_per_row * Q):
        _check(_lib.psn_mlp_infer_x3_occ(ctypes.byref(desc), streams[0], streams[1], ptrs[0],
                                         ptrs[1], Q, None if n_rows_dev is None else n_rows_dev.data_ptr(),
                                         None if out_rows is None else out_rows.data_ptr(), int(pe_octaves), float(pe_scale),
                                         int(skip_layer), int(pe_first), ptrs[2], _stream()), 'mlp_infer_x3_occ')
    return out


def sg_shade_fwd(light_dir, view, normal, albedo, weights, lobe, light_int, light_int_scalar, vis, specular_rgb):
    L, Ns, nb = light_dir.shape[0], view.shape[0], lobe.shape[0]
    rgb = torch.empty(L * Ns, 3, device=view.device, dtype=torch.float32)
    spec = torch.empty(L * Ns, 3 if specular_rgb else 1, device=view.device, dtype=torch.float32)
    if Ns == 0:
        return rgb, spec
    _check(_lib.psn_sg_shade_fwd(_tptr(light_dir, 'light_dir'), _tptr(view, 'view'), _tptr(normal, 'normal'),
                                 _tptr(albedo, 'albedo'), _tptr(weights, 'weights'), _tptr(lobe, 'lobe'),
                                 _tptr(light_int, 'light_int', allow_none=True),
                                 1 if light_int is None or light_int.dim() == 1 else light_int.shape[1],
                                 float(light_int_scalar), _tptr(vis, 'vis', allow_none=True),
                                 L, Ns, nb, int(bool(specular_rgb)), _tptr(rgb, 'rgb'), _tptr(spec, 'spec'), _stream()),
           'sg_shade_fwd')
    return rgb, spec


def sg_shade_bwd(light_dir, view, normal, albedo, weights, lobe, light_int, light_int_scalar, vis, specular_rgb,
                 g_rgb, g_spec, want_vis):
    L, Ns, nb = light_dir.shape[0], view.shape[0], lobe.shape[0]
    dev = view.device
    d_albedo = torch.empty(Ns, 3, device=dev)
    d_weights = torch.empty_like(weights)
    d_normal = torch.empty(Ns, 3, device=dev)
    d_vis = torch.empty(L * Ns, device=dev) if want_vis else None
    d_ldir = torch.empty(L, 3, device=dev)
    d_lint = torch.empty(L, device=dev) if light_int is not None else None
    if Ns == 0:
        return d_albedo, d_weights, d_normal, d_vis, torch.zeros_like(d_ldir), None if d_lint is None else torch.zeros_like(d_lint)
    ws = workspace(((Ns + 63) // 64) * L * 4, dev)
    _check(_lib.psn_sg_shade_bwd(_tptr(light_dir, 'light_dir'), _tptr(view, 'view'), _tptr(normal, 'normal'),
                                 _tptr(albedo, 'albedo'), _tptr(weights, 'weights'), _tptr(lobe, 'lobe'),
                                 _tptr(light_int, 'light_int', allow_none=True), float(light_int_scalar), _tptr(vis, 'vis', allow_none=True),
                                 L, Ns, nb, int(bool(specular_rgb)), _tptr(g_rgb, 'g_rgb'), _tptr(g_spec, 'g_spec', allow_none=True),
                                 _tptr(d_albedo, 'd_albedo'), _tptr(d_weights, 'd_weights'), _tptr(d_normal, 'd_normal'),
                                 _tptr(d_vis, 'd_vis', allow_none=True), _tptr(d_ldir, 'd_ldir'), _tptr(d_lint, 'd_lint', allow_none=True),
                                 ws.data_ptr(), _stream()), 'sg_shade_bwd')
    return d_albedo, d_weights, d_normal, d_vis, d_ldir, d_lint


def mf_shade_fwd(light_dir, view, normal, albedo, rough, light_int, light_int_scalar, f0, vis):
    L, Ns = light_dir.shape[0], view.shape[0]
    rgb = torch.empty(L * Ns, 3, device=view.device, dtype=torch.float32)
    if Ns == 0:
        return rgb
    _check(_lib.psn_mf_shade_fwd(_tptr(light_dir, 'light_dir'), _tptr(view, 'view'), _tptr(normal, 'normal'),
                                 _tptr(albedo, 'albedo'), _tptr(rough, 'rough'), _tptr(light_int, 'light_int', allow_none=True),
                                 float(light_int_scalar), float(f0), _tptr(vis, 'vis', allow_none=True), L, Ns, _tptr(rgb, 'rgb'),
                                 _stream()), 'mf_shade_fwd')
    return rgb


def mf_shade_bwd(light_dir, view, normal, albedo, rough, light_int, light_int_scalar, f0, vis, g_rgb, want_vis):
    L, Ns = light_dir.shape[0], view.shape[0]
    dev = view.device
    d_albedo = torch.empty(Ns, 3, device=dev)
    d_rough = torch.empty(Ns, device=dev)
    d_normal = torch.empty(Ns, 3, device=dev)
    d_vis = torch.empty(L * Ns, device=dev) if want_vis else None
    d_ldir = torch.empty(L, 3, device=dev)
    d_lint = torch.empty(L, device=dev) if light_int is not None else None
    if Ns == 0:
        return d_albedo, d_rough, d_normal, d_vis, torch.zeros_like(d_ldir), None if d_lint is None else torch.zeros_like(d_lint)
    ws = workspace(((Ns + 63) // 64) * L * 4, dev)
    _check(_lib.psn_mf_shade_bwd(_tptr(light_dir, 'light_dir'), _tptr(view, 'view'), _tptr(normal, 'normal'),
                                 _tptr(albedo, 'albedo'), _tptr(rough, 'rough'), _tptr(light_int, 'light_int', allow_none=True),
                                 float(light_int_scalar), float(f0), _tptr(vis, 'vis', allow_none=True), L, Ns, _tptr(g_rgb, 'g_rgb'),
                                 _tptr(d_albedo, 'd_albedo'), _tptr(d_rough, 'd_rough'), _tptr(d_normal, 'd_normal'),
                                 _tptr(d_vis, 'd_vis', allow_none=True), _tptr(d_ldir, 'd_ldir'), _tptr(d_lint, 'd_lint', allow_none=True),
                                 ws.data_ptr(), _stream()), 'mf_shade_bwd')
    return d_albedo, d_rough, d_normal, d_vis, d_ldir, d_lint


def march_sweep_x3(desc, packed_w, bias_steps, final_bias, origin, direction, far, u, omu, near, n_steps, tau, pe_octaves, pe_scale,
                   skip_layer, pe_first, early_exit=True, macs_per_row=None):
    N = origin.shape[0]
    assert origin.shape == (N, 3) and direction.shape == (N, 3) and far.shape == (N,) and u.numel() == n_steps == omu.numel()
    streams = (_bf16_stream(packed_w, 'packed_w'), _bf16_stream(bias_steps, 'bias_steps'))
    occ = torch.empty(N, n_steps, device=origin.device, dtype=torch.float32)
    skip = torch.zeros(N, device=origin.device, dtype=torch.int32) if early_exit else None
    if N == 0:
        return occ, skip
    count = torch.zeros(1, device=origin.device, dtype=torch.int64) if PROFILE_EVENTS is not None else None
    with _Prof('march_sweep_x3', N * n_steps, None if (macs_per_row is None or count is None) else (count, 2.0 * macs_per_row * 128)):
        _check(_lib.psn_march_sweep_x3(ctypes.byref(desc), streams[0], streams[1], _tptr(final_bias, 'final_bias'),
                                       _tptr(origin, 'origin'), _tptr(direction, 'direction'), _tptr(far, 'far'), _tptr(u, 'u'), _tptr(omu, 'omu'),
                                       float(near), N, int(n_steps), float(tau), int(pe_octaves), float(pe_scale), int(skip_layer), int(pe_first),
                                       None if skip is None else skip.data_ptr(), occ.data_ptr(), None if count is None else count.data_ptr(),
                                       _stream()), 'march_sweep_x3')
    return occ, skip


def mise_flags(resolution, device):
    n3 = (resolution + 1) ** 3
    return torch.zeros((n3 + 3) // 4 * 4, dtype=torch.uint8, device=device)


def mise_collect(flags, resolution, box_size, capacity, count):
    assert flags.numel() == ((resolution + 1) ** 3 + 3) // 4 * 4 and count.numel() == 1
    rows = torch.empty(capacity, dtype=torch.int64, device=flags.device)
    points = torch.empty(capacity, 3, dtype=torch.float32, device=flags.device)
    _check(_lib.psn_mise_collect(_tptr(flags, 'flags', torch.uint8), int(resolution), float(box_size), int(capacity), rows.data_ptr(),
                                 points.data_ptr(), _tptr(count, 'count', torch.int64), _stream()), 'mise_collect')
    return rows, points


def mise_refine(grid, flags, vox, resolution0, depth, threshold, pending):
    res = resolution0 << depth
    assert grid.numel() == (res + 1) ** 3 and flags.numel() == ((res + 1) ** 3 + 3) // 4 * 4 and pending.numel() == 1
    assert vox.numel() == sum((resolution0 << l) ** 3 for l in range(depth))
    _check(_lib.psn_mise_refine(_tptr(grid, 'grid'), _tptr(flags, 'flags', torch.uint8), _tptr(vox, 'vox', torch.uint8), int(resolution0),
                                int(depth), float(threshold), _tptr(pending, 'pending', torch.int64), _stream()), 'mise_refine')


def grid_ffill(grid):
    n = grid.shape[0]
    assert grid.shape == (n, n, n)
    with _Prof('grid_ffill', 8 * grid.numel()):
        _check(_lib.psn_grid_ffill(_tptr(grid, 'grid'), n, _stream()), 'grid_ffill')
    return grid


def marching_cubes(grid, threshold, box_size=0.0):
    n = grid.shape[0]
    assert grid.shape == (n, n, n)
    dev = grid.device
    nb = int(_lib.psn_mc_blocks(n))
    if nb == 0:
        raise RuntimeError('marching_cubes: %d points per axis are not supported (2 .. %d)' % (n, MESH_MAX_RESOLUTION + 1))
    n_cells = (n + 1) ** 3
    code = torch.empty(n_cells, dtype=torch.uint8, device=dev)
    blk = torch.empty(2, nb, dtype=torch.int32, device=dev)
    with _Prof('mc_count', 4 * grid.numel()):
        _check(_lib.psn_mc_count(_tptr(grid, 'grid'), n, float(threshold), code.data_ptr(), blk[0].data_ptr(), blk[1].data_ptr(), _stream()),
               'mc_count')
    incl = torch.cumsum(blk, dim=1, dtype=torch.int64)
    base = (incl - blk).contiguous()
    n_v, n_f = (int(x) for x in incl[:, -1].tolist())
    vertices = torch.empty(n_v, 3, dtype=torch.float64, device=dev)
    faces = torch.empty(n_f, 3, dtype=torch.int64, device=dev)
    if n_v == 0:
        return vertices, faces
    v_off = torch.empty(n_cells, dtype=torch.int32, device=dev)
    with _Prof('mc_emit', 24 * n_v + 24 * n_f):
        _check(_lib.psn_mc_emit(_tptr(grid, 'grid'), n, float(threshold), code.data_ptr(), base[0].data_ptr(), base[1].data_ptr(), n_v, n_f,
                                float(box_size), v_off.data_ptr(), vertices.data_ptr(), faces.data_ptr(), _stream()), 'mc_emit')
    return vertices, faces


def tri_grid(lo, hi, cell, n, max_span):
    g = PsnTriGrid()
    for a in range(3):
        g.lo[a], g.hi[a], g.n[a] = float(lo[a]), float(hi[a]), int(n[a])
    g.cell, g.max_span = float(cell), int(max_span)
    return g


def _mesh_ptrs(vertices, faces):
    if vertices.dim() != 2 or vertices.shape[1] != 3 or faces.dim() != 2 or faces.shape[1] != 3:
        raise RuntimeError('mesh: vertices [V, 3] and faces [F, 3] expected, got %s / %s' % (tuple(vertices.shape), tuple(faces.shape)))
    return _tptr(vertices, 'vertices', torch.float64), _tptr(faces, 'faces', torch.int64)


def tri_grid_count(grid, vertices, faces, n_over):
    vp, fp = _mesh_ptrs(vertices, faces)
    cells = grid.n[0] * grid.n[1] * grid.n[2]
    assert n_over.numel() == 1
    cell_count = torch.empty(cells, dtype=torch.int32, device=vertices.device)
    over_list = torch.empty(faces.shape[0], dtype=torch.int32, device=vertices.device)
    with _Prof('tri_grid_count', 96 * faces.shape[0]):
        _check(_lib.psn_tri_grid_count(ctypes.byref(grid), vp, fp, faces.shape[0], cell_count.data_ptr(), over_list.data_ptr(),
                                       _tptr(n_over, 'n_over', torch.int64), _stream()), 'tri_grid_count')
    return cell_count, over_list


def tri_grid_fill(grid, vertices, faces, cursor, n_entries):
    vp, fp = _mesh_ptrs(vertices, faces)
    assert cursor.numel() == grid.n[0] * grid.n[1] * grid.n[2]
    lst = torch.empty(int(n_entries), dtype=torch.int32, device=vertices.device)
    with _Prof('tri_grid_fill', 96 * faces.shape[0]):
        _check(_lib.psn_tri_grid_fill(ctypes.byref(grid), vp, fp, faces.shape[0], _tptr(cursor, 'cursor', torch.int32), int(n_entries),
                                      lst.data_ptr(), _stream()), 'tri_grid_fill')
    return lst


def closest_point(grid, vertices, faces, cell_start, lst, over_list, n_over, points, order=None, n_tests=None):
    vp, fp = _mesh_ptrs(vertices, faces)
    if points.dim() != 2 or points.shape[1] != 3:
        raise RuntimeError('closest_point: points [Q, 3] expected, got %s' % (tuple(points.shape),))
    assert cell_start.numel() == grid.n[0] * grid.n[1] * grid.n[2] + 1 and 0 <= n_over <= over_list.numel()
    q = points.shape[0]
    assert order is None or order.numel() == q
    dev = vertices.device
# ... 510 lines not shown
```

psnerf_amd/ops.py:

```python
import collections

import torch

from . import fused, hip


HITS = collections.Counter()


def _hit(name):
    HITS[name] += 1


import os as _os0
STRICT = _os0.environ.get('PSN_STRICT', '0') == '1'
FALLBACKS = collections.Counter()


def fallback(name, tensor=None, why=''):
    if tensor is not None and not getattr(tensor, 'is_cuda', False):
        return
    FALLBACKS[name] += 1
    if STRICT:
        raise RuntimeError('psnerf_amd.ops.STRICT: %s left the fused engines on a device tensor%s' % (name, (' (' + why + ')') if why else ''))
# ... 172 lines not shown


class FusedPairMLP(torch.autograd.Function):

    @staticmethod
    def forward(ctx, tab_a, tab_b, in_cols, skip_at, *params):
        _hit('FusedPairMLP')
        Ws, bs = params[0::2], params[1::2]
        nA, nB = tab_a.shape[0], tab_b.shape[0]
        din_half = in_cols.numel() // 2
        packed = fused.pack_relu_mlp(list(Ws), list(bs), din_half, din_half, skip_at)
        out = packed(tab_a, nA * nB, a_div=1, a_mod=nA, tab_b=tab_b, b_div=nA, b_mod=nB)
        ctx.save_for_backward(tab_a, tab_b, in_cols, *params)
        ctx.skip_at = skip_at
        return out

    @staticmethod
    def backward(ctx, d_out):
        tab_a, tab_b, in_cols = ctx.saved_tensors[:3]
        params = [p.detach().requires_grad_(True) for p in ctx.saved_tensors[3:]]
        nA, nB = tab_a.shape[0], tab_b.shape[0]
        ta = tab_a.detach().requires_grad_(ctx.needs_input_grad[0])
        tb = tab_b.detach().requires_grad_(ctx.needs_input_grad[1])
        with torch.enable_grad():
            x = torch.cat([ta.tile(nB, 1), tb.repeat_interleave(nA, dim=0)], dim=1)
            out = ReluMLP.apply(x, in_cols, ctx.skip_at, False, *params)
            wanted = [t for t in [ta, tb] + params if t.requires_grad]
            got = torch.autograd.grad(out, wanted, d_out, allow_unused=True)
        it = iter(got)
        res = []
        for t in [ta, tb]:
            res.append(next(it) if t.requires_grad else None)
        pg = [next(it) for _ in params]
        return (res[0], res[1], None, None) + tuple(pg)


class SplitRows(torch.autograd.Function):

    @staticmethod
    def forward(ctx, t, k):
        _hit('SplitRows')
        ctx.k, ctx.shape = k, t.shape
        return t[:k], t[k:]

    @staticmethod
    def backward(ctx, ga, gb):
        k, shape = ctx.k, ctx.shape
        if ga is None:
            ga = gb.new_zeros((k,) + tuple(shape[1:]))
        if gb is None:
            gb = ga.new_zeros((shape[0] - k,) + tuple(shape[1:]))
        return torch.cat([ga, gb], dim=0), None


class ScatterRows(torch.autograd.Function):

    @staticmethod
    def forward(ctx, idx, inv, specs, *rows):
        _hit('ScatterRows')
        ctx.set_materialize_grads(False)
        ctx.specs, ctx.n_pix, ctx.ns = specs, inv.numel(), idx.numel()
        ctx.save_for_backward(idx, inv)
        return tuple(hip.scatter_rows(list(specs), [r.detach() for r in rows], inv, inv.numel(), idx.numel()))

    @staticmethod
    def backward(ctx, *grads):
        idx, inv = ctx.saved_tensors
        sel = [k for k, g in enumerate(grads) if g is not None and ctx.needs_input_grad[3 + k]]
        out = [None] * len(grads)
        if sel:
            got = hip.gather_rows([ctx.specs[k] for k in sel], [grads[k].contiguous() for k in sel], idx, ctx.n_pix, ctx.ns, inv=inv)
            for k, g in zip(sel, got):
                out[k] = g
        return (None, None, None) + tuple(out)


class WeightNormAll(torch.autograd.Function):

    @staticmethod
    def forward(ctx, scales, *gv):
        _hit('WeightNormAll')
        gs, vs = [t.detach().contiguous() for t in gv[0::2]], [t.detach().contiguous() for t in gv[1::2]]
        ctx.scales = scales
        ctx.save_for_backward(*gs, *vs)
        return tuple(hip.weight_norm_fwd(vs, [g.reshape(-1) for g in gs], scales))

    @staticmethod
    def backward(ctx, *dws):
        n = len(ctx.scales)
        sv = ctx.saved_tensors
        gs, vs = sv[:n], sv[n:]
        dws = [torch.zeros_like(v) if d is None else d.contiguous() for d, v in zip(dws, vs)]
        dvs, dgs = hip.weight_norm_bwd(list(vs), [g.reshape(-1) for g in gs], ctx.scales, dws)
        out = [None]
        for g, dg, dv in zip(gs, dgs, dvs):
            out += [dg.view_as(g), dv]
        return tuple(out)


def sg_shade(light_dir, view, normal, albedo, weights, lobe, light_int, vis, specular_rgb):
    return SGShade.apply(light_dir, view, normal, albedo, weights, lobe, light_int, vis, specular_rgb)


class SGShade(torch.autograd.Function):

    @staticmethod
    def forward(ctx, light_dir, view, normal, albedo, weights, lobe, light_int, vis, specular_rgb):
        _hit('SGShade')
        li_t, li_s = None, 0.0
        rgb_lights = False
        if torch.is_tensor(light_int):
            if light_int.dim() == 2 and light_int.shape[1] == 3:
                if any(ctx.needs_input_grad):
                    raise RuntimeError('sg_shade: RGB light intensities are supported on the forward-only path')
                li_t = light_int.contiguous()
                rgb_lights = True
            elif light_int.numel() > 1:
                li_t = light_int.reshape(-1).contiguous()
            else:
                li_t = light_int.reshape(-1).expand(light_dir.shape[0]).contiguous()
        else:
            li_s = float(light_int)
        ctx.set_materialize_grads(False)
        vis_f = None if vis is None else vis.reshape(-1).contiguous()
        args = (light_dir.contiguous(), view.contiguous(), normal.contiguous(), albedo.contiguous(),
                weights.contiguous(), lobe.contiguous())
        rgb, spec = hip.sg_shade_fwd(*args, li_t, li_s, vis_f, specular_rgb)
        ctx.save_for_backward(*args, *([li_t] if li_t is not None else []), *([vis_f] if vis_f is not None else []))
        ctx.has_li, ctx.has_vis, ctx.li_s, ctx.specular_rgb = li_t is not None, vis_f is not None, li_s, specular_rgb
        ctx.li_shape = light_int.shape if torch.is_tensor(light_int) else None
        ctx.vis_shape = None if vis is None else vis.shape
        return rgb, spec

    @staticmethod
    def backward(ctx, g_rgb, g_spec):
        sv = list(ctx.saved_tensors)
        light_dir, view, normal, albedo, weights, lobe = sv[:6]
        k = 6
        li_t = sv[k] if ctx.has_li else None
        k += 1 if ctx.has_li else 0
        vis_f = sv[k] if ctx.has_vis else None
        want_vis = ctx.has_vis and ctx.needs_input_grad[7]
        g_spec_c = None if g_spec is None else g_spec.contiguous()
        if g_rgb is None:
            g_rgb = torch.zeros(light_dir.shape[0] * view.shape[0], 3, device=view.device)
        d_alb, d_w, d_n, d_vis, d_ld, d_li = hip.sg_shade_bwd(light_dir, view, normal, albedo, weights, lobe, li_t,
                                                              ctx.li_s, vis_f, ctx.specular_rgb, g_rgb.contiguous(),
                                                              g_spec_c, want_vis)
        if d_li is not None:
            d_li = d_li.sum().reshape(ctx.li_shape) if int(torch.tensor(ctx.li_shape).prod()) == 1 else d_li.reshape(ctx.li_shape)
        if d_vis is not None:
            d_vis = d_vis.reshape(ctx.vis_shape)
        return d_ld, None, d_n, d_alb, d_w, None, d_li, d_vis, None


def _buf(rows, cols, device):
    pad = (cols + 3) // 4 * 4
    return torch.empty(rows, pad, device=device, dtype=torch.float32)[:, :cols]


class GeoField(torch.autograd.Function):

    @staticmethod
    def forward(ctx, p, n_octaves, scale, skips, with_grad, *params):
        _hit('GeoField')
        Ws, bs = [w.contiguous() for w in params[0::2]], [b.contiguous() for b in params[1::2]]
        n = len(Ws)
        p = p.contiguous()
        Q = p.shape[0]
        dev = p.device
        d_pe = 3 + 6 * n_octaves
        kp = (d_pe + 3) // 4 * 4
        H = Ws[1].shape[1]
        pe = hip.pe_encode(p, n_octaves, kp, scale)
        W0p = torch.nn.functional.pad(Ws[0], (0, kp - d_pe)).contiguous()
        A, S = [None] * n, [None] * (n - 1)
        A[0] = pe
        for l in range(n - 1):
            o = Ws[l].shape[0]
            if (l + 1) in skips:
                nxt = torch.empty(Q, o + d_pe, device=dev, dtype=torch.float32)
                dst = nxt[:, :o]
                nxt[:, o:] = pe[:, :d_pe]
            else:
                nxt = _buf(Q, o, dev)
                dst = nxt
            S[l] = _buf(Q, o, dev)
            hip.gemm(A[l], W0p if l == 0 else Ws[l], trans_b=True, bias=bs[l], epi=hip.EPI_BIAS_SOFTPLUS, out=dst,
                     aux_out=S[l])
            A[l + 1] = nxt
        out = hip.gemm(A[n - 1], Ws[n - 1], trans_b=True, bias=bs[n - 1], epi=hip.EPI_BIAS)
        grad = None
        U, R = [None] * (n - 1), [None] * n
        if with_grad:
            w_last = Ws[n - 1][0:1, :]
            U[n - 2] = S[n - 2] * w_last
            d_pe_acc = None
            for l in range(n - 2, 0, -1):
                in_a = Ws[l].shape[1] - d_pe if l in skips else Ws[l].shape[1]
                R[l] = _buf(Q, in_a, dev)
                U[l - 1] = _buf(Q, in_a, dev)
                hip.gemm(U[l], Ws[l][:, :in_a], epi=hip.EPI_MUL_AUX_RAW, aux_in=S[l - 1], out=U[l - 1], aux_out=R[l])
                if l in skips:
                    g_skip = hip.gemm(U[l], Ws[l][:, in_a:])
                    d_pe_acc = g_skip if d_pe_acc is None else d_pe_acc + g_skip
            d_pe_t = hip.gemm(U[0], W0p)
            if d_pe_acc is not None:
                d_pe_t[:, :d_pe] += d_pe_acc
            grad = hip.pe_encode_bwd(p, d_pe_t, n_octaves, scale)
        if any(ctx.needs_input_grad):
            ctx.n, ctx.skips, ctx.with_grad, ctx.d_pe, ctx.kp = n, list(skips), with_grad, d_pe, kp
            ctx.n_octaves, ctx.scale = n_octaves, scale
            keep = [p, W0p] + Ws + A + S
            if with_grad:
                keep += U + R[1:n - 1]
                if ctx.needs_input_grad[0]:
                    keep.append(d_pe_t)
            ctx.save_for_backward(*keep)
        if grad is None:
            grad = torch.zeros(Q, 3, device=dev)
            ctx.mark_non_differentiable(grad)
        return out, grad

    @staticmethod
    def backward(ctx, d_out, d_grad):
        n, skips, d_pe, kp = ctx.n, ctx.skips, ctx.d_pe, ctx.kp
        sv = list(ctx.saved_tensors)
        p, W0p = sv[0], sv[1]
        Ws = sv[2:2 + n]
        A = sv[2 + n:2 + 2 * n]
        S = sv[2 + 2 * n:2 + 3 * n - 1]
        Q = p.shape[0]
        dev = p.device
        dW = [None] * n
        db = [None] * n
        sweep = ctx.with_grad and d_grad is not None
        dS = [None] * (n - 1)
        need_p, need_w = ctx.needs_input_grad[0], any(ctx.needs_input_grad[5:])
        dz_pe = {}

        def add_dW(l, a_t, b_mat, with_bias=False):
            if not need_w:
                return
            sk = _split_k_for(Q, a_t.shape[1], b_mat.shape[1])
            cs = torch.empty(a_t.shape[1], device=dev) if with_bias else None
            if dW[l] is None:
                dW[l] = hip.gemm(a_t, b_mat, trans_a=True, split_k=sk, colsum_a=cs)
            else:
                hip.gemm(a_t, b_mat, trans_a=True, split_k=sk, out=dW[l], epi=hip.EPI_ACCUM, colsum_a=cs)
            if with_bias:
                db[l] = cs

        if sweep:
            base = 2 + 3 * n - 1
            U = sv[base:base + n - 1]
            R = [None] + sv[base + n - 1:base + n - 1 + (n - 2)] + [None]
            dd_pe = hip.pe_encode_jvp(p, d_grad.contiguous(), ctx.n_octaves, kp, ctx.scale)
            w_last = Ws[n - 1][0:1, :]
            dR = dd_pe
            for l in range(n - 1):
                Wl = W0p if l == 0 else Ws[l]
                o = Wl.shape[0]
                r_next = R[l + 1] if l + 1 <= n - 2 else w_last.expand(Q, -1)
                if (l + 1) in skips:
                    nxt = torch.empty(Q, o + d_pe, device=dev, dtype=torch.float32)
                    dst = nxt[:, :o]
                    nxt[:, o:] = dd_pe[:, :d_pe]
                else:
                    nxt = _buf(Q, o, dev)
                    dst = nxt
                dS[l] = _buf(Q, o, dev)
                hip.gemm(dR, Wl, trans_b=True, epi=hip.EPI_MUL2, aux_in=S[l], aux_in2=r_next, out=dst, aux_out=dS[l])
                add_dW(l, U[l], dR)
                dR = nxt
            if need_w:
                dW[n - 1] = torch.zeros_like(Ws[n - 1])
                dW[n - 1][0] = hip.colsum(dR)

        g = d_out.contiguous()
        add_dW(n - 1, g, A[n - 1], with_bias=True)
        for l in range(n - 1, 0, -1):
            in_a = Ws[l].shape[1] - d_pe if l in skips else Ws[l].shape[1]
            g_prev = _buf(Q, in_a, dev)
            if sweep:
                hip.gemm(g, Ws[l][:, :in_a], epi=hip.EPI_SOFTPLUS_BWD, aux_in=S[l - 1], aux_in2=dS[l - 1], out=g_prev)
            else:
                hip.gemm(g, Ws[l][:, :in_a], epi=hip.EPI_MUL_AUX, aux_in=S[l - 1], out=g_prev)
            g = g_prev
            if need_p and (l - 1 == 0 or (l - 1) in skips):
                dz_pe[l - 1] = g
            add_dW(l - 1, g, A[l - 1], with_bias=True)
        if need_w:
            dW[0] = dW[0][:, :d_pe]
        d_p = None
        if need_p:
            sks = [l for l in sorted(dz_pe) if l > 0]
            first = sks[0] if sks else None
            d_p = hip.geo_point_grad(p, ctx.n_octaves, ctx.scale, dz_pe[0], W0p,
                                     dzs=None if first is None else dz_pe[first],
                                     ws=None if first is None else Ws[first][:, Ws[first].shape[1] - d_pe:],
                                     g_pe=sv[-1] if sweep else None, d_grad=d_grad.contiguous() if sweep else None)
            for l in sks[1:]:
                d_p = d_p + hip.geo_point_grad(p, ctx.n_octaves, ctx.scale, dz_pe[l], Ws[l][:, Ws[l].shape[1] - d_pe:])
        grads = []
        for l in range(n):
            grads += [dW[l], db[l]]
# ... 285 lines not shown

    @staticmethod
    def forward(ctx, x, normal, feat, d_x, chains, *params):
        _hit('AppNetFused')
        n = len(params) // 2
        Q = x.shape[0]
        feat = feat.contiguous()
        need = any(ctx.needs_input_grad)
        H = [torch.empty(Q, 256, device=x.device) for _ in range(n - 1)] if need else None
        out = chains['fwd'](x, Q, act_init=feat, save=H)
        if need:
            ctx.save_for_backward(x, feat, *H, *params[0::2])
            ctx.meta = (n, d_x, chains)
        return out

    @staticmethod
    def backward(ctx, g):
        n, d_x, chains = ctx.meta
        sv = ctx.saved_tensors
        x, feat = sv[0], sv[1]
        H = sv[2:2 + n - 1]
        Ws = sv[2 + n - 1:]
        Q, dev = x.shape[0], x.device
        g = g.contiguous()
        DZ = [torch.empty(Q, 256, device=dev) for _ in range(n - 1)]
        d_feat = torch.empty(Q, 256, device=dev)
        d_normal = chains['bwd'](None, Q, a_div=1, a_mod=Q, rank_init=(g, Ws[n - 1].contiguous()),
                                 mask=[H[n - 2 - j] for j in range(n - 1)] + [None, None], save=DZ + [d_feat])
        dz0 = DZ[n - 2]
        items = [dict(A=dz0, B=x[:, :d_x], colsum=True), dict(A=dz0, B=feat)]
        items += [dict(A=DZ[n - 2 - l], B=H[l - 1], colsum=True) for l in range(1, n - 1)]
        res = hip.gemm_tn_grouped(items)
        grads = [torch.cat([res[0][0], res[1][0]], dim=1), res[0][1]]
        for l in range(1, n - 1):
            grads += [res[l + 1][0], res[l + 1][1]]
        grads += [hip.colsum(H[n - 2], row_weight=g), _rowsum_small(g)]
        return (None, d_normal, d_feat, None, None) + tuple(grads)


class FusedReluNet(torch.autograd.Function):

    @staticmethod
    def pack(Ws, bs, din, skip_at, final_sigmoid, width):
        with torch.no_grad():
            return fused.pack_relu_mlp(list(Ws), list(bs), din, 0, skip_at,
                                       out_act=hip.OUT_SIGMOID if final_sigmoid else hip.OUT_NONE, precompute=False, width=width)

    @staticmethod
    def forward(ctx, pe, din, skip_at, final_sigmoid, width, packed, *params):
        _hit('FusedReluNet')
        Ws, bs = params[0::2], params[1::2]
        n = len(Ws)
        Q = pe.shape[0]
        if packed is None:
            packed = FusedReluNet.pack(Ws, bs, din, skip_at, final_sigmoid, width)
        need = any(ctx.needs_input_grad[6:])
        H = [torch.empty(Q, width, device=pe.device) for _ in range(n - 1)] if need else None
        bits = _sign_bits(Q, n - 1, pe.device) if (need and RELU_SIGN_BITS) else None
        out = packed(pe, Q, save=H, save_bits=bits)
        if need:
            ctx.save_for_backward(pe, out, *H, *Ws)
            ctx.meta = (n, din, skip_at, final_sigmoid, width)
            ctx.bits = bits
        return out

    @staticmethod
    def backward(ctx, g):
        n, din, skip_at, final_sigmoid, width = ctx.meta
        sv = ctx.saved_tensors
        pe, out = sv[0], sv[1]
        H = sv[2:2 + n - 1]
        Ws = sv[2 + n - 1:]
        Q, dev = pe.shape[0], pe.device
        g = g.contiguous()
        if final_sigmoid:
            g = torch.ops.aten.sigmoid_backward(g, out)
        bits = ctx.bits
        chain = fused.pack_relu_bwd(list(Ws), skip_at, width=width, bits=bits is not None, x3=CHAIN_X3)
        DZ = [torch.empty(Q, width, device=dev) for _ in range(n - 1)]
        masks = [(bits if bits is not None else H)[n - 2 - j] for j in range(n - 1)]
        if Ws[n - 1].shape[0] <= 4:
            chain(None, Q, a_div=1, a_mod=Q, rank_init=(g, Ws[n - 1].contiguous()), mask=masks, save=DZ)
        else:
            dh = hip.gemm(g, Ws[n - 1].contiguous())
            chain(None, Q, a_div=1, a_mod=Q, init_a_direct=dh, mask=masks, save=DZ)
        x_in = pe[:, :din]
        items = [dict(A=g, B=H[n - 2], colsum=True)]
        where = [(n - 1, 'w')]
        for l in range(n - 2, -1, -1):
            dz = DZ[n - 2 - l]
            if l == 0:
                items.append(dict(A=dz, B=x_in, colsum=True))
                where.append((0, 'w'))
            else:
                items.append(dict(A=dz, B=H[l - 1], colsum=True))
                where.append((l, 'w'))
                if l - 1 == skip_at:
                    items.append(dict(A=dz, B=x_in))
                    where.append((l, 'x'))
        res = hip.gemm_tn_grouped(items)
        dW, dWx, db = [None] * n, [None] * n, [None] * n
        for (l, kind), (C, cs) in zip(where, res):
            if kind == 'w':
                dW[l], db[l] = C, cs
            else:
                dWx[l] = C
        grads = []
        for l in range(n):
            grads += [dW[l] if dWx[l] is None else torch.cat([dW[l], dWx[l]], dim=1), db[l]]
        return (None, None, None, None, None, None) + tuple(grads)


class Stage2Losses(torch.autograd.Function):

    @staticmethod
    def forward(ctx, rgb, rgb_gt, alb, alb_j, wgt, wgt_j, vis, vis_gt, nrm, nrm_gt, nrm_j, mask_a, mask_b, l2, inv_denom, weight,
                count_dev=None):
        _hit('Stage2Losses')
        c = lambda t: None if t is None else t.detach().contiguous()
        ts = [c(t) for t in (rgb, rgb_gt, alb, alb_j, wgt, wgt_j, vis, vis_gt, nrm, nrm_gt, nrm_j)]
        ma, mb = mask_a.contiguous(), mask_b.contiguous()
        out = hip.stage2_loss_fwd(*ts, ma, mb, l2, inv_denom, weight, count_dev)
        slots = ts + [ma, mb, count_dev]
        ctx.present = [t is not None for t in slots]
        ctx.save_for_backward(*[t for t in slots if t is not None])
        ctx.l2 = l2
        ctx.k = [w * d for w, d in zip(weight, inv_denom)]
        ctx.need = ctx.needs_input_grad
        terms = out[:6]
        ctx.mark_non_differentiable(terms)
        return out[6], terms

    @staticmethod
    def backward(ctx, g_total, _g_terms):
        saved = iter(ctx.saved_tensors)
        slots = [next(saved) if here else None for here in ctx.present]
        rgb, rgb_gt, alb, alb_j, wgt, wgt_j, vis, vis_gt, nrm, nrm_gt, nrm_j, mask_a, mask_b, count_dev = slots
        k, ng = ctx.k, ctx.need
        need = set()
        if rgb is not None and ng[0] and k[0] != 0.0: need.add('rgb')
        if alb is not None and (ng[2] or ng[3]) and k[1] != 0.0: need.add('alb')
        if wgt is not None and (ng[4] or ng[5]) and k[2] != 0.0: need.add('wgt')
        if vis is not None and ng[6] and k[3] != 0.0: need.add('vis')
        if nrm is not None and (ng[8] or ng[10]) and (k[4] != 0.0 or k[5] != 0.0): need.add('nrm')
        d = {}
        if need:
            d = hip.stage2_loss_bwd(g_total.reshape(1).contiguous(), rgb, rgb_gt, k[0], alb, alb_j, k[1], wgt, wgt_j, k[2], vis, vis_gt,
                                    k[3], nrm, nrm_gt, nrm_j, k[4], k[5], mask_a, mask_b, ctx.l2, need, count_dev)
        g = d.get
        return (g('rgb'), None, g('alb'), g('alb_j'), g('wgt'), g('wgt_j'), g('vis'), None, g('nrm'), None, g('nrm_j'),
                None, None, None, None, None, None)


class SurfaceNormals(torch.autograd.Function):

    @staticmethod
    def forward(ctx, g, hit):
        _hit('SurfaceNormals')
        gc, hc = g.detach().contiguous(), hit.contiguous()
        ctx.save_for_backward(gc, hc)
        return hip.surface_normals_fwd(gc, hc)

    @staticmethod
    def backward(ctx, d_norm_pred, d_diff):
        g, hit = ctx.saved_tensors
        c = lambda t: None if t is None else t.contiguous()
        return hip.surface_normals_bwd(g, hit, c(d_norm_pred), c(d_diff)), None


class Stage1Losses(torch.autograd.Function):

    @staticmethod
    def forward(ctx, rgb, rgb_gt, diff, hit, normal, normal_gt, norm_mask, acc, mask_gt, mask_valid, n_rays, weights, reduce_counts=None):
        _hit('Stage1Losses')
        c = lambda t: None if t is None else t.detach().contiguous()
        rgb, rgb_gt, diff, normal, normal_gt, acc, mask_gt = (c(t) for t in (rgb, rgb_gt, diff, normal, normal_gt, acc, mask_gt))
        hit, norm_mask, mask_valid = (c(t) for t in (hit, norm_mask, mask_valid))
        sums, terms = hip.stage1_loss_fwd(rgb, rgb_gt, diff, hit, normal, normal_gt, norm_mask, acc, mask_gt, mask_valid, n_rays, weights,
                                          finish=reduce_counts is None)
        if reduce_counts is not None:
            reduce_counts(sums[4:7])
            terms = hip.stage1_loss_terms(sums, n_rays, weights, diff is not None and weights[1] != 0.0, normal is not None, acc is not None)
        slots = [rgb, rgb_gt, hit, normal, normal_gt, norm_mask, acc, mask_gt, mask_valid, sums]
        ctx.present = [t is not None for t in slots]
        ctx.save_for_backward(*[t for t in slots if t is not None])
        ctx.n_rays, ctx.weights, ctx.has_diff = n_rays, tuple(float(w) for w in weights), diff is not None
        ctx.need = ctx.needs_input_grad
        loss = terms[4]
        ctx.mark_non_differentiable(terms)
        return loss, terms

    @staticmethod
    def backward(ctx, g_loss, _g_terms):
        saved = iter(ctx.saved_tensors)
        rgb, rgb_gt, hit, normal, normal_gt, norm_mask, acc, mask_gt, mask_valid, sums = (next(saved) if here else None for here in ctx.present)
        w, ng = ctx.weights, ctx.need
        need = set()
        if ng[0] and w[0] != 0.0: need.add('rgb')
        if ctx.has_diff and ng[2] and w[1] != 0.0: need.add('diff')
        if normal is not None and ng[4] and w[2] != 0.0: need.add('normal')
        if acc is not None and ng[7] and w[3] != 0.0: need.add('acc')
        d = {}
        if need:
            d = hip.stage1_loss_bwd(g_loss.reshape(1).contiguous(), sums, rgb, rgb_gt, hit, normal, normal_gt, norm_mask, acc, mask_gt,
                                    mask_valid, ctx.n_rays, w, need)
        g = d.get
        return g('rgb'), None, g('diff'), None, g('normal'), None, None, g('acc'), None, None, None, None, None


class NormalizeRows(torch.autograd.Function):

    @staticmethod
    def forward(ctx, x, eps=1e-12):
        _hit('NormalizeRows')
        xc = x.detach().contiguous()
        ctx.save_for_backward(xc)
        ctx.eps = float(eps)
        return hip.normalize_rows_fwd(xc, eps)

    @staticmethod
    def backward(ctx, g):
        (x,) = ctx.saved_tensors
        return hip.normalize_rows_bwd(x, g.contiguous(), ctx.eps), None


def normalize_rows(x, eps=1e-12):
    if x.is_cuda and x.dim() == 2 and x.shape[1] == 3 and x.dtype == torch.float32:
        return NormalizeRows.apply(x, eps)
    return torch.nn.functional.normalize(x, p=2, dim=-1, eps=eps)


class LightRows(torch.autograd.Function):

    @staticmethod
    def forward(ctx, dir_table, int_table, idx):
        _hit('LightRows')
        dt, it, ix = dir_table.detach().contiguous(), int_table.detach().contiguous(), idx.contiguous()
        ctx.save_for_backward(dt, ix)
        d, i = hip.light_rows_fwd(dt, it, ix)
        return d, i

    @staticmethod
    def backward(ctx, g_dir, g_int):
        dt, ix = ctx.saved_tensors
        need_d, need_i = ctx.needs_input_grad[0], ctx.needs_input_grad[1]
        dd, di = hip.light_rows_bwd(dt, ix, g_dir.contiguous() if (need_d and g_dir is not None) else None,
                                    g_int.contiguous() if (need_i and g_int is not None) else None)
        return dd, di, None
```

psnerf_amd/stage2/loss.py:

```python
import torch
from torch import nn
from torch.nn import functional as F


def _masked_mean(diff, mask_b, count, channels):
    return torch.where(mask_b.bool().unsqueeze(-1), diff, diff.new_zeros(())).sum() / float(count * channels)


class MainLoss(nn.Module):

    def __init__(self, sg_rgb_weight, loss_type='L1', albedo_smooth_weight=0, rough_smooth_weight=0, vis_weight=1.0):
        super().__init__()
        self.sg_rgb_weight = sg_rgb_weight
        self.albedo_smooth_weight = albedo_smooth_weight
        self.rough_smooth_weight = rough_smooth_weight
        self.vis_weight = vis_weight
        if loss_type not in ('L1', 'L2'):
            raise Exception('Unknown loss_type!')
        self.loss_type = loss_type
        self.global_count = None

    def _img(self, a, b):
        return (a - b).abs() if self.loss_type == 'L1' else (a - b) ** 2

    def forward(self, model_outputs, ground_truth, model_input=None, count=None):
        m, om = model_outputs['network_object_mask'], model_outputs['object_mask']
        mask = m & om
        dev = mask.device
        if count is None:
            count = int(mask.sum()) if self.global_count is None else self.global_count(mask)
        zero = torch.zeros((), device=dev)
        rgb_gt = ground_truth['rgb'].to(dev)
        L = rgb_gt.shape[0]
        if count == 0:
            rgb_loss = zero
        else:
            rgb_loss = _masked_mean(self._img(model_outputs['sg_rgb_values'], rgb_gt), mask.expand(L, -1), count * L, 3)
        loss = self.sg_rgb_weight * rgb_loss
        a_loss = r_loss = None
        if 'albedo_jitter' in model_outputs and self.albedo_smooth_weight > 0:
            x, xj = model_outputs['albedo_values'], model_outputs['albedo_jitter']
            a_loss = zero if count == 0 else _masked_mean((x - xj).abs(), mask.expand(x.shape[0], -1),
                                                          count * x.shape[0], x.shape[-1])
            loss = loss + self.albedo_smooth_weight * a_loss
        if 'rough_jitter' in model_outputs and self.rough_smooth_weight > 0:
            x, xj = model_outputs['rough_values'], model_outputs['rough_jitter']
            r_loss = zero if count == 0 else _masked_mean((x - xj).abs(), mask.expand(x.shape[0], -1),
                                                          count * x.shape[0], x.shape[-1])
            loss = loss + self.rough_smooth_weight * r_loss
        terms = {'sg_rgb_loss': rgb_loss, 'albedo_smooth_loss': a_loss, 'rough_smooth_loss': r_loss}
        if 'visibility' in model_input and 'visibility' in model_outputs:
            if 'vis_train_gt' in model_input and 'light_vis_train' in model_input and 'vis_train' in model_outputs:
                v, gt = model_outputs['vis_train'][..., 0], model_input['vis_train_gt']
            elif 'light_vis_train' in model_input and 'vis_train' in model_outputs:
                v, gt = model_outputs['vis_train'][..., 0], model_input['visibility']
            else:
                v, gt = model_outputs['visibility'][..., 0], model_input['visibility']
            if count == 0:
                vis_loss = zero
            else:
                vis_loss = _masked_mean(self._img(v, gt).unsqueeze(-1), mask.expand(gt.shape[0], -1), count * gt.shape[0], 1)
            loss = loss + self.vis_weight * vis_loss
            terms['vis_loss'] = vis_loss
        terms['loss'] = loss
        return terms


class NormalLoss(nn.Module):

    def __init__(self, normal_weight, normal_smooth_weight=0):
        super().__init__()
        self.normal_weight, self.normal_smooth_weight = normal_weight, normal_smooth_weight
        self.global_count = None

    def forward(self, model_outputs, count=None):
        gt = F.normalize(model_outputs['normal_values'], dim=-1)
        mask = model_outputs['network_object_mask'] & model_outputs['object_mask']
        dev = mask.device
        if count is None:
            count = int(mask.sum()) if self.global_count is None else self.global_count(mask)
        zero = torch.zeros((), device=dev)
        if count == 0:
            n_loss = zero
        else:
            n_loss = _masked_mean((model_outputs['normal_pred'] - gt) ** 2, mask, count, 3)
        loss = self.normal_weight * n_loss
        s_loss = None
        if 'normal_jitter' in model_outputs and self.normal_smooth_weight > 0:
            s_loss = zero if count == 0 else _masked_mean(
                (model_outputs['normal_pred'] - model_outputs['normal_jitter']).abs(), mask, count, 3)
            loss = loss + self.normal_smooth_weight * s_loss
        return {'loss': loss, 'normal_loss': n_loss, 'normal_smooth_loss': s_loss}


def fused_losses(main, normal, model_outputs, ground_truth, model_input, count):
    from .. import ops
    o = model_outputs
    need = ('sg_rgb_values', 'normal_pred', 'normal_values', 'network_object_mask', 'object_mask')
    if any(k not in o for k in need) or not o['sg_rgb_values'].is_cuda or main.loss_type not in ('L1', 'L2'):
        return None
    ma, mb = o['network_object_mask'][0], o['object_mask'][0]
    if ma.dtype != torch.bool or mb.dtype != torch.bool:
        return None
    rgb, rgb_gt = o['sg_rgb_values'], ground_truth['rgb'].to(o['sg_rgb_values'].device)
    L, N = rgb.shape[0], rgb.shape[1]
    alb = alb_j = wgt = wgt_j = vis = vis_gt = nrm_j = None
    if 'albedo_jitter' in o and main.albedo_smooth_weight > 0:
        alb, alb_j = o['albedo_values'], o['albedo_jitter']
    if 'rough_jitter' in o and main.rough_smooth_weight > 0:
        wgt, wgt_j = o['rough_values'], o['rough_jitter']
    has_vis = 'visibility' in model_input and 'visibility' in o
    if has_vis:
        if 'vis_train_gt' in model_input and 'light_vis_train' in model_input and 'vis_train' in o:
            vis, vis_gt = o['vis_train'], model_input['vis_train_gt']
        elif 'light_vis_train' in model_input and 'vis_train' in o:
            vis, vis_gt = o['vis_train'], model_input['visibility']
        else:
            vis, vis_gt = o['visibility'], model_input['visibility']
        vis_gt = vis_gt.float()
    nrm, nrm_gt = o['normal_pred'], o['normal_values']
    if 'normal_jitter' in o and normal.normal_smooth_weight > 0:
        nrm_j = o['normal_jitter']
    count_dev = count.reshape(1).float() if torch.is_tensor(count) else None
    c = 1.0 if count_dev is not None else float(max(count, 1))
    nb = 1 if wgt is None else wgt.shape[-1]
    V = 1 if vis is None else vis.shape[0]
    inv = [1.0 / (c * L * 3), 1.0 / (c * 3), 1.0 / (c * nb), 1.0 / (c * V), 1.0 / (c * 3), 1.0 / (c * 3)]
    if count_dev is None and count == 0:
        inv = [0.0] * 6
    w = [float(main.sg_rgb_weight), float(main.albedo_smooth_weight) if alb is not None else 0.0,
         float(main.rough_smooth_weight) if wgt is not None else 0.0, float(main.vis_weight) if vis is not None else 0.0,
         float(normal.normal_weight), float(normal.normal_smooth_weight) if nrm_j is not None else 0.0]
    total, t = ops.Stage2Losses.apply(rgb, rgb_gt, alb, alb_j, wgt, wgt_j, vis, vis_gt, nrm, nrm_gt, nrm_j, ma, mb,
                                      1 if main.loss_type == 'L2' else 0, inv, w, count_dev)
    terms = {'sg_rgb_loss': t[0], 'albedo_smooth_loss': t[1] if alb is not None else None,
             'rough_smooth_loss': t[2] if wgt is not None else None, 'loss': total}
    if has_vis:
        terms['vis_loss'] = t[3]
    terms_n = {'loss': total, 'normal_loss': t[4], 'normal_smooth_loss': t[5] if nrm_j is not None else None}
    return total, terms, terms_n
```

psnerf_amd/stage2/renderer.py:

```python
import contextlib
import os

import numpy as np
import torch
import torch.nn as nn
import torch.nn.functional as F

from .. import fused, hip, ops

PE_STRIDE = 64


def camera_rays(uv, pose, intrinsics):
    fx, fy = intrinsics[:, 0, 0], intrinsics[:, 1, 1]
    cx, cy = intrinsics[:, 0, 2], intrinsics[:, 1, 2]
    z = torch.ones_like(uv[:, :, 0])
    x = (uv[:, :, 0] - cx.unsqueeze(-1)) / fx.unsqueeze(-1) * z
    y = (uv[:, :, 1] - cy.unsqueeze(-1)) / fy.unsqueeze(-1) * z
    R = pose[:, :3, :3]
    d = x.unsqueeze(-1) * R[:, None, :, 0] + y.unsqueeze(-1) * R[:, None, :, 1] + z.unsqueeze(-1) * R[:, None, :, 2]
    return F.normalize(d, dim=2), pose[:, :3, 3]


class MLP(fused.PackCached, nn.Module):
# ... 78 lines not shown
            nbasis = conf.get_int('train.nbasis', default=9)
            self.specular_rgb = conf.get_bool('train.specular_rgb', default=False)
            self.sgbasis = SGBasis(nbasis=nbasis, specular_rgb=self.specular_rgb)
            self.albedo_net = MLP(dim_emb, 3, W, depth, skip_at=[skip], final='sigmoid')
            if self.specular_rgb:
                nbasis *= 3
            self.rough_net = MLP(dim_emb, nbasis, conf.get_int('brdf.sgnet.mlp_width', 128),
                                 conf.get_int('brdf.sgnet.mlp_depth', 4),
                                 skip_at=[conf.get_int('brdf.sgnet.mlp_skip_at', 2)])
            self.nbasis = nbasis
        self.light_int = conf.get_float('brdf.light_intensity', default=4.0)
        self.shape_pregen = conf.get_bool('train.shape_pregen', default=False)
        if not self.shape_pregen:
            raise NotImplementedError('train.shape_pregen=False (the reference leaves surface_points undefined there)')
        self.xyz_jitter_std = conf.get_float('brdf.net.xyz_jitter_std', default=0)
        self.normal_mlp = conf.get_bool('train.normal_mlp', default=False)
        if self.normal_mlp:
            self.n_freqs_n = conf.get_int('normal.net.n_freqs_xyz')
            self.normal_net = MLP(3 + 6 * self.n_freqs_n, 3, conf.get_int('normal.net.mlp_width'),
                                  conf.get_int('normal.net.mlp_depth'),
                                  skip_at=[conf.get_int('normal.net.mlp_skip_at')])
            self.normal_joint = conf.get_bool('train.normal_joint', default=False)
            self.normal_jitter_std = conf.get_float('normal.net.xyz_jitter_std', default=0)
            if not self.normal_joint:
                self.normal_net = self.normal_net.eval().requires_grad_(False)
                self.normal_jitter_std = 0
        self.inference_precision = 'fp32'
        self._eval_cache = None
        self._eval_outputs = None
        self.train_vis_bf16 = conf.get_bool('train.vis_bf16', default=False)
        self.train_vis_bf16x6 = conf.get_bool('train.vis_bf16x6', default=False)
        self.train_vis_bf16x3 = conf.get_bool('train.vis_bf16x3', default=False)
        self.overlap_small_nets = conf.get_bool('train.overlap_small_nets', default=True)
        self._side = {}
        self._cols_cache = {}
        self.visibility = conf.get_bool('train.visibility', default=False)
        self.light_vis_detach = conf.get_bool('train.light_vis_detach', default=False)
        if self.visibility:
            self.visibility_net = MLP(dim_emb * 2, 1, conf.get_int('visibility.net.mlp_width'),
                                      conf.get_int('visibility.net.mlp_depth'),
                                      skip_at=[conf.get_int('visibility.net.mlp_skip_at')])

    def invalidate_packs(self, trainable_only=False):
        mlps = self.__dict__.get('_mlp_list')
        if mlps is None:
            mlps = self.__dict__['_mlp_list'] = [m for m in self.modules() if isinstance(m, MLP)]
        live = [m for m in mlps if not trainable_only or any(q.requires_grad for q in m.parameters())]
        if live:
            self.packs.invalidate()
        for m in live:
            m.invalidate_packs()

    def _pe(self, x, n_freqs):
        return ops.positional_encoding(x, n_freqs, PE_STRIDE)

    def _cols(self, n_freqs, device, pair=False):
        key = (n_freqs, str(device), pair)
        c = self._cols_cache.get(key)
        if c is None:
            d = 3 + 6 * n_freqs
            c = torch.arange(d, device=device)
            c = self._cols_cache[key] = torch.cat([c, PE_STRIDE + c]) if pair else c
            c._psn_contiguous_pair = bool(pair)
            if c.is_cuda:
                torch.cuda.current_stream(c.device).synchronize()
        return c

    def _visibility_rows(self, pe_x, light_dirs, fused_ok):
        l_in = light_dirs.detach() if self.light_vis_detach else light_dirs
        pe_l = self._pe(l_in, self.n_freqs)
        net = self.visibility_net
        Ws, bs = net.weights()
        cols = self._cols(self.n_freqs, pe_x.device, pair=True)
        mode = self.inference_precision
        if (fused_ok and net.width == 256 and mode in ('bf16', 'bf16x6', 'bf16x3') and not torch.is_grad_enabled() and pe_x.is_cuda
                and (mode == 'bf16x3' or len(Ws) <= 12)):
            return self._visibility_rows_lowp(mode, pe_x, pe_l)
        if fused_ok and net.width == 256:
            return ops.FusedPairMLP.apply(pe_x, pe_l, cols, net._skip_index(), *fused.interleave(Ws, bs))
        if fused_ok:
            ops.fallback('stage2.visibility rows -> expanded [L Ns, 128] input', pe_x, 'visibility_net width %d' % net.width)
        ns, nl = pe_x.shape[0], pe_l.shape[0]
        x = torch.cat([pe_x.tile(nl, 1), pe_l.repeat_interleave(ns, dim=0)], dim=1)
        return net(x, cols)

    def _visibility_pair_args(self, pe_x, light_dir, light_vis_train):
        pe_l = self._pe(torch.cat([light_dir.detach(), light_vis_train.detach()], dim=0), self.n_freqs)
        net = self.visibility_net
        cols = self._cols(self.n_freqs, pe_x.device, pair=True)
        return pe_x.detach(), pe_l, light_dir.shape[0], cols, net._skip_index(), fused.interleave(*net.weights())

    def _visibility_prepack(self):
        net = self.visibility_net
        if net.width != 256 or not net.linears[0].weight.is_cuda:
            return None
        return self._vis_pack('fp32', lambda prev, *net_args: fused.pack_relu_mlp(*net_args, reuse=prev))

    def _vis_pack(self, slot, build):
        net = self.visibility_net

        def make(prev):
            Ws, bs = net.weights()
            half = 3 + 6 * self.n_freqs
            return build(prev, list(Ws), list(bs), half, half, net._skip_index())
        return self.packs.get(slot, net.parameters(), make)

    def _vis_out_act(self):
        return hip.OUT_SIGMOID if self.visibility_net.final == 'sigmoid' else hip.OUT_NONE

    @torch.no_grad()
    def _visibility_rows_bf16(self, pe_x, pe_l):
        pack = self._vis_pack('bf16', lambda prev, *net_args: fused.pack_relu_mlp_bf16_grouped(*net_args, self._vis_out_act()))
        return pack(pe_x.to(torch.bfloat16), pe_l.contiguous())

    @torch.no_grad()
    def _visibility_rows_x3(self, pe_x, pe_l):
        pack = self._vis_pack('bf16x6', lambda prev, *net_args: fused.pack_relu_mlp_x3_grouped(*net_args, self._vis_out_act()))
        return pack(pe_x.contiguous(), pe_l.contiguous())

    @torch.no_grad()
    def _visibility_rows_b3(self, pe_x, pe_l):
        pack = self._vis_pack('bf16x3', lambda prev, *net_args: fused.pack_relu_mlp(
            *net_args, out_act=self._vis_out_act(), reuse=prev, x3=True))
        ns, nl = pe_x.shape[0], pe_l.shape[0]
        return pack(pe_x.contiguous(), nl * ns, a_div=1, a_mod=ns, tab_b=pe_l.contiguous(), b_div=ns, b_mod=nl)

    def _visibility_rows_lowp(self, mode, pe_x, pe_l):
        rows = {'bf16': self._visibility_rows_bf16, 'bf16x6': self._visibility_rows_x3, 'bf16x3': self._visibility_rows_b3}
        return rows[mode](pe_x, pe_l)

    def _memo(self, tag, input, fn):
        cache = self._eval_cache
        if cache is None or torch.is_grad_enabled():
            return fn()
        key = (tag,) + tuple((input[k].data_ptr(), input[k]._version) for k in ('points', 'surface_mask', 'uv')) \
            + self.packs.key(self.parameters())
        if key not in cache:
            cache[key] = fn()
        return cache[key]

    def _visibility_pair_launch(self, pe_x, light_dir, light_vis_train, live_count=None):
        a = self._visibility_pair_args(pe_x, light_dir, light_vis_train)
        need = any(p.requires_grad for p in a[5])
        return a, ops.VisibilityPair.launch(a[0], a[1], a[2], a[3], a[4], [p.detach() for p in a[5]], need,
                                            packed=self._visibility_prepack(), live_count=live_count)

    def _visibility_pair(self, pe_x, light_dir, light_vis_train, launched=None):
        if launched is not None:
            a, pre = launched
        else:
            a, pre = self._visibility_pair_args(pe_x, light_dir, light_vis_train), None
        return ops.VisibilityPair.apply(a[0], a[1], a[2], a[3], a[4], pre, *a[5])

    def forward(self, input, albedo_new=None, basis_new=None, noise=None):
        noise = noise or {}
        uv, pose, intr = input['uv'], input['pose'], input['intrinsics']
        object_mask = input['object_mask']
        device = uv.device
        surface_mask, points, normals = input['surface_mask'], input['points'], input['normal']
        idx = input.get('surface_idx')
        if idx is None:
            idx = surface_mask[0].nonzero(as_tuple=True)[0]
        ns = idx.shape[0]

        def gather(t):
            return t[0].index_select(0, idx)

        n_pix = points.shape[1]

        def scatter(dense, rows):
            return _Dense(dense.fill, dense.B, dense.C, rows)

        def ones3(b=1):
            return _Dense(1.0, b, 3)

        surf = gather(points).contiguous()
        out_n = {}
        normal_s = None
        pe_x = None
        vis_pair = None
        vis_bf16 = None
        side = None
        pair_ok = False
        if ns > 0 and self.visibility:
            lv0 = input.get('light_vis_train')
            ld0 = input['light_direction']
            pair_ok = (lv0 is not None and self.conf.get_bool('train.vis_rgb_detach', default=False)
                       and self.visibility_net.width == 256 and torch.is_grad_enabled()
                       and (self.light_vis_detach or not (ld0.requires_grad or lv0.requires_grad)))
            if pair_ok:
                pe_x = self._pe(surf, self.n_freqs)
                if self.overlap_small_nets and surf.is_cuda:
                    side = self._side.get(device)
                    if side is None:
                        side = self._side[device] = torch.cuda.Stream(device=device)
                    side.wait_stream(torch.cuda.current_stream(device))
                mode = 'bf16x3' if self.train_vis_bf16x3 else 'bf16x6' if self.train_vis_bf16x6 else 'bf16' if self.train_vis_bf16 else None
                if mode is not None:
                    pe_l0 = self._pe(ld0.detach(), self.n_freqs)
                    vis_bf16 = self._visibility_rows_lowp(mode, pe_x, pe_l0)
                    vis_pair = self._visibility_pair_launch(pe_x, ld0[:0], lv0)
                else:
                    vis_pair = self._visibility_pair_launch(pe_x, ld0, lv0, live_count=input.get('surface_count'))
        on_side = (lambda: torch.cuda.stream(side)) if side is not None else contextlib.nullcontext
        if self.normal_mlp:
            normal_pred = ones3()
            if ns > 0:
              with on_side():
                cols_n = self._cols(self.n_freqs_n, device)
                pe_n = (lambda: pe_x) if (pe_x is not None and self.n_freqs_n == self.n_freqs) else (lambda: self._pe(surf, self.n_freqs_n))
                if self.normal_jitter_std > 0 and torch.is_grad_enabled():
                    nz = noise.get('normal')
                    if nz is None:
                        nz = torch.empty_like(surf).normal_(0.0, self.normal_jitter_std)
                    pe_both_n = torch.cat([pe_n(), self._pe(surf + nz, self.n_freqs_n)], dim=0)
                    normal_s, nj = ops.SplitRows.apply(ops.normalize_rows(self.normal_net(pe_both_n, cols_n)), ns)
                    normal_pred = scatter(normal_pred, normal_s)
                    out_n['normal_jitter'] = scatter(ones3(), nj)
                else:
                    normal_s = self._memo('normal', input, lambda: ops.normalize_rows(self.normal_net(pe_n(), cols_n)))
                    normal_pred = scatter(normal_pred, normal_s)
                    if self.normal_jitter_std > 0:
                        nz = noise.get('normal')
                        if nz is None:
                            nz = torch.empty_like(surf).normal_(0.0, self.normal_jitter_std)
                        nj = self._memo('normal_jitter', input, lambda: ops.normalize_rows(
                            self.normal_net(self._pe(surf + nz, self.n_freqs_n), cols_n)))
                        out_n['normal_jitter'] = scatter(ones3(), nj)
            out_n['normal_pred'] = normal_pred

        sg = self.render_model == 'sgbasis'
        lnum = input['light_direction'].shape[0]
        rgb_values = ones3(lnum)
        albedo_values = ones3()
        rough_values = ones3(lnum) if sg else ones3()
        weight_values = _Dense(0.0, 1, self.nbasis) if sg else None
        vis_values = ones3(lnum)
        jitter = None
        vis_t_pre = None
        if ns > 0:
            normal = gather(normals) if not self.normal_mlp else normal_s
            with on_side():
                if (uv.is_cuda and uv.shape[0] == 1 and uv.dtype == torch.float32 and tuple(pose.shape[1:]) == (4, 4)
                        and tuple(intr.shape[1:]) == (4, 4)):
                    pts2c = hip.camera_rays(uv.contiguous(), pose.contiguous().float(), intr.contiguous().float(), idx, scale=-1.0)
                else:
                    ray_dirs, _ = camera_rays(uv, pose, intr)
                    pts2c = -gather(ray_dirs)
            light_dir = input['light_direction']
            cols = self._cols(self.n_freqs, device)
            if pe_x is None:
                pe_x = self._memo('pe_x', input, lambda: self._pe(surf, self.n_freqs))
            pe_j = None
            with on_side():
              if self.xyz_jitter_std > 0:
                nz = noise.get('xyz')
                if nz is None:
                    nz = torch.empty_like(surf).normal_(0.0, self.xyz_jitter_std)
                def brdf_both():
                    pe_both = torch.cat([pe_x, self._pe(surf + nz, self.n_freqs)], dim=0)
                    return self.albedo_net(pe_both, cols), self.rough_net(pe_both, cols)
                albedo_both, rough_both = self._memo('brdf_both', input, brdf_both)
                albedo, albedo_j = ops.SplitRows.apply(albedo_both, ns)
                if sg:
                    rough_both = F.relu(rough_both)
                rough, rough_j = ops.SplitRows.apply(rough_both, ns)
              else:
                albedo, rough = self._memo('brdf', input, lambda: (self.albedo_net(pe_x, cols), self.rough_net(pe_x, cols)))
              if albedo_new is not None:
                albedo = torch.from_numpy(albedo_new).to(device)[None].expand_as(albedo)
              if sg:
                weights = rough if self.xyz_jitter_std > 0 else F.relu(rough)
                if basis_new is not None:
                    wn = torch.zeros_like(weights)
                    if self.specular_rgb:
                        wn.view(-1, 3, self.nbasis // 3)[:, :, basis_new] = 2 ** basis_new / 100
                    else:
                        wn.view(-1, 1, self.nbasis)[:, :, basis_new] = 2 ** basis_new / 100
                    weights = wn.reshape(-1, self.nbasis)
                weight_values = scatter(weight_values, weights)
            if side is not None:
                main = torch.cuda.current_stream(device)
                main.wait_stream(side)
                for t_ in (pts2c, normal_s, albedo_both if self.xyz_jitter_std > 0 else albedo, rough_both if self.xyz_jitter_std > 0 else rough,
                           weights if sg else None, out_n.get('normal_jitter').rows if 'normal_jitter' in out_n else None):
                    if torch.is_tensor(t_):
                        t_.record_stream(main)
            light_int = input.get('light_intensity', self.light_int)
            vis = None
            vis_for_rgb = None
            vis_t_pre = None
            if self.visibility:
                detach = self.conf.get_bool('train.vis_rgb_detach', default=False)
                if pair_ok:
                    if vis_bf16 is not None:
                        _none, vis_t_pre = self._visibility_pair(pe_x, light_dir[:0], lv0, launched=vis_pair)
                        vis = vis_bf16
                    else:
                        vis, vis_t_pre = self._visibility_pair(pe_x, light_dir, lv0, launched=vis_pair)
                else:
                    vis = self._visibility_rows(pe_x, light_dir, fused_ok=True)
                vis_for_rgb = vis.detach() if detach else vis
            if sg:
                rgb, spec = ops.sg_shade(light_dir, pts2c, normal, albedo, weights, self.sgbasis.lobe, light_int,
                                         vis_for_rgb, self.specular_rgb)
            else:
                rgb = ops.mf_shade(light_dir, pts2c, normal, albedo, rough, light_int, vis_for_rgb, self.f0)
            rgb_values = scatter(rgb_values, rgb)
            if vis is not None:
                vis_values = scatter(vis_values, vis.expand(rgb.shape))
            albedo_values = scatter(albedo_values, albedo)
            if sg:
                rough_values = scatter(rough_values, spec.expand(-1, 3))
            else:
                rough_values = scatter(rough_values, rough.expand(-1, 3))
            if self.xyz_jitter_std > 0:
                aj = scatter(ones3(), albedo_j)
                if sg:
                    rj = scatter(_Dense(1.0, 1, self.nbasis), rough_j)
                    r_ori = weight_values
                else:
                    rj = scatter(ones3(), rough_j.expand(-1, 3))
                    r_ori = rough_values
                jitter = {'albedo_values': albedo_values, 'albedo_jitter': aj,
                          'rough_values': r_ori, 'rough_jitter': rj}

        out = {
            'points': points, 'object_mask': object_mask, 'network_object_mask': surface_mask,
            'sg_rgb_values': rgb_values, 'normal_values': normals,
            'sg_diffuse_albedo_values': albedo_values, 'sg_specular_rgb_values': rough_values,
        }
        if jitter is not None:
            out.update(jitter)
        if self.normal_mlp:
            out.update(out_n)
        if self.visibility:
            out['visibility'] = vis_values
            if 'vis_train_gt' in input or 'light_vis_train' in input:
                lv = input['light_vis_train']
                vnum = lv.shape[0]
                vt = ones3(vnum)
                if ns > 0:
                    if vis_t_pre is not None:
                        vis_t = vis_t_pre
                    else:
                        train = torch.is_grad_enabled() and any(p.requires_grad for p in self.visibility_net.parameters())
                        vis_t = self._visibility_rows(pe_x, lv, fused_ok=not train)
                    vt = scatter(vt, vis_t.expand(-1, 3))
                out['vis_train'] = vt
        if sg:
            out['sg_weight'] = weight_values
        want = self._eval_outputs
        if want is not None:
            if 'sg_rgb_light_sum' in want:
                v = out['sg_rgb_values']
                rows_sum = v.rows.reshape(v.B, -1, v.C).sum(0) if v.rows is not None else None
                out['sg_rgb_light_sum'] = (rows_sum, idx if v.rows is not None else None, v.fill * v.B)
            out = {k: v for k, v in out.items() if k in want}
        lazy = {}
        for v in out.values():
            if isinstance(v, _Dense):
                lazy[id(v)] = v
        with_rows = [v for v in lazy.values() if v.rows is not None]
        done = {}
        if with_rows:
            if idx.is_cuda and idx.dtype == torch.int64:
                inv = hip.inverse_index(idx.contiguous(), n_pix, count=input.get('surface_count'))
            else:
                inv = torch.full((n_pix,), -1, dtype=torch.int32, device=device)
                inv[idx] = torch.arange(ns, dtype=torch.int32, device=device)
            specs = tuple((v.B, v.C, v.fill) for v in with_rows)
            dense = ops.ScatterRows.apply(idx, inv, specs, *[v.rows for v in with_rows])
            for v, d in zip(with_rows, dense):
                done[id(v)] = d
        for v in lazy.values():
            if v.rows is None:
                done[id(v)] = torch.full((v.B, n_pix, v.C), v.fill, device=device)
        for k in list(out.keys()):
            if isinstance(out[k], _Dense):
                out[k] = done[id(out[k])]
        return out
```

psnerf_amd/stage2/trainer.py:

```python
import numpy as np
import torch
import torch.nn as nn
import torch.nn.functional as F

from ..dist import DataParallel
from .. import ops
from ..optim import FlatAdam, RowSparseAdam
from .loss import MainLoss, NormalLoss, fused_losses


class VisPlus(object):

    def __init__(self, views, light_vis_train, vnum, device, rng=None):
        self.vnum, self.device = int(vnum), device
        self.rng = rng if rng is not None else np.random
        self.lights = [torch.cat([v['vis_plus_light'].to(device).float(), lv.to(device).float()], dim=0)
                       for v, lv in zip(views, light_vis_train)]
        self.vis = [torch.cat([v['vis_plus'].to(device).float().reshape(v['vis_plus'].shape[0], -1),
                               v['visibility'].to(device).float()], dim=0) for v in views]
        for l, m in zip(self.lights, self.vis):
            assert l.shape[0] == m.shape[0]

    def select(self, vidx, sampling_idx=None):
        lights, vis = self.lights[int(vidx)], self.vis[int(vidx)]
        sidx = torch.as_tensor(self.rng.choice(np.arange(lights.shape[0]), self.vnum, replace=False)).long().to(self.device)
        if sampling_idx is None:
            return lights[sidx], vis[sidx]
        return lights[sidx], vis[sidx[:, None], sampling_idx.to(self.device).long()[None, :]]


def scheduler_milestones(conf, n_views):
    ms = list(conf.get_list('train.sg_sched_milestones', default=[]))
    ms = [int(m) * int(n_views) for m in ms]
    if conf.get_bool('train.multi_light', default=False):
        ms = [m * conf.get_int('train.light_bs') for m in ms]
    return ms


class TrainStep(object):
    FUSED_LOSSES = True

    def __init__(self, model, conf, n_lights_total, light_init, device, milestones=(), dp=None, vis_plus=None):
        self.model, self.conf, self.device = model, conf, device
        self.light_vis_table = light_init.detach().clone().to(device)
        self.vis_plus = vis_plus
        lk = dict(sg_rgb_weight=1.0, loss_type='L1', albedo_smooth_weight=0.05, rough_smooth_weight=0.01, vis_weight=1)
        lc = conf.get_config('loss', default=None) if hasattr(conf, 'get_config') else None
        if lc:
            lk.update({k: lc[k] for k in lk if k in lc})
        self.loss = MainLoss(**lk)
        nk = dict(normal_weight=1, normal_smooth_weight=0.05)
        nc = conf.get_config('normal.loss', default=None) if hasattr(conf, 'get_config') else None
        if nc:
            nk.update({k: nc[k] for k in nk if k in nc})
        self.loss_n = NormalLoss(**nk)
        self.dp = dp if dp is not None else DataParallel(device)
        if self.dp.enabled:
            self.loss.global_count = self.dp.global_count
            self.loss_n.global_count = self.dp.global_count
        gamma = conf.get_float('train.sg_sched_factor', default=0.0)
        on_gpu = all(p.is_cuda and p.dtype == torch.float32 for p in model.parameters())
        self.sg_optimizer = (FlatAdam if on_gpu else torch.optim.Adam)(model.parameters(), lr=conf.get_float('train.sg_learning_rate'))
        self.sg_scheduler = torch.optim.lr_scheduler.MultiStepLR(self.sg_optimizer, list(milestones), gamma=gamma)
        self.light_para = nn.Embedding(n_lights_total, 3, sparse=False).to(device)
        self.light_para.weight.data.copy_(light_init)
        self.light_train = conf.get_bool('train.light_train', default=False)
        self.ana_fixlight = conf.get_bool('train.ana_fixlight', default=False)
        self.visibility = conf.get_bool('train.visibility', default=False)
        self.vis_loss = self.visibility and conf.get_bool('train.vis_loss', default=False)
        self.normal_train = conf.get_bool('train.normal_mlp', default=False) and conf.get_bool('train.normal_joint', default=False)
        if vis_plus is not None and not self.light_train:
            raise AttributeError("train.vis_plus needs train.light_train (the per-view initial light estimates 'light_vis_train', trainer.py:149,388)")
        self.wgrad_bf16x6 = conf.get_bool('train.wgrad_bf16x6', default=False)
        self.wgrad_mode = conf.get_string('train.wgrad_precision', default='bf16x6' if self.wgrad_bf16x6 else 'fp32')
        self.wgrad_bf16x6 = self.wgrad_mode != 'fp32'
        self.chain_mode = conf.get_string('train.chain_precision', default='fp32')
        assert self.chain_mode in ('fp32', 'bf16x3'), self.chain_mode
        self.light_inten_train = self.light_train and conf.get_bool('train.light_inten_train', default=False)
        if not self.light_train:
            self.light_para.requires_grad_(False)
        self.light_decay = conf.get_bool('train.light_decay', default=False)
        self.light_inten_para = nn.Embedding(n_lights_total, 1, sparse=False).to(device)
        nn.init.constant_(self.light_inten_para.weight, model.light_int)
        lr_l = conf.get_float('train.light_learning_rate', default=5e-4)
        groups = [{'params': list(self.light_para.parameters())}]
        if self.light_inten_train:
            groups.append({'params': list(self.light_inten_para.parameters()), 'lr': conf.get_float('train.light_inten_lr', default=lr_l)})
        else:
            self.light_inten_para.requires_grad_(False)
        self.light_optimizer = RowSparseAdam(groups, lr=lr_l)
        self.light_scheduler = torch.optim.lr_scheduler.MultiStepLR(self.light_optimizer, list(milestones), gamma=gamma)
        self.cur_iter = 0

    def train_fix(self):
        if self.cur_iter == 0:
            self._ori = (self.loss.sg_rgb_weight, self.loss.albedo_smooth_weight,
                         self.loss.rough_smooth_weight, self.loss.vis_weight)
            self.loss.sg_rgb_weight = 0
            self.loss.albedo_smooth_weight = 0
            self.loss.rough_smooth_weight = 0
            self.loss.vis_weight = 10
            self.model.albedo_net.eval().requires_grad_(False)
            self.model.rough_net.eval().requires_grad_(False)
            if self.visibility and not self.vis_loss:
                self.model.visibility_net.eval().requires_grad_(False)
            if self.light_train:
                self.light_para.requires_grad_(False)
                if self.light_inten_train:
                    self.light_inten_para.requires_grad_(False)
        elif self.cur_iter == 5000:
            (self.loss.sg_rgb_weight, self.loss.albedo_smooth_weight,
             self.loss.rough_smooth_weight, self.loss.vis_weight) = self._ori
            self.model.albedo_net.train().requires_grad_(True)
            self.model.rough_net.train().requires_grad_(True)
            if not self.ana_fixlight and self.light_train:
                self.light_para.requires_grad_(True)
                if self.light_inten_train:
                    self.light_inten_para.requires_grad_(True)

    def step(self, model_input, ground_truth, l_slt, train_order=True, noise=None, vidx=None):
        if train_order:
            self.train_fix()
        model_input = self.select_vis_lights(model_input, vidx)
        terms, out, trainable, train_light = self._fwd_bwd(model_input, ground_truth, l_slt, noise=noise)
        self._reduce(trainable)
        self._optimise(l_slt, trainable, train_light)
        self._advance(train_light)
        return terms, out

    def select_vis_lights(self, model_input, vidx):
        if self.vis_plus is None or vidx is None:
            return model_input
        model_input = dict(model_input)
        sidx = model_input.get('sampling_idx')
        if sidx is not None and sidx.dim() == 2:
            sidx = sidx[0]
        model_input['light_vis_train'], model_input['vis_train_gt'] = self.vis_plus.select(vidx, sidx)
        return model_input

    def _fwd_bwd(self, model_input, ground_truth, l_slt, noise=None, count=None):
        if self.chain_mode != 'fp32':
            with ops.chain_precision(self.chain_mode):
                return self._fwd_bwd_exact(model_input, ground_truth, l_slt, noise, count)
        return self._fwd_bwd_exact(model_input, ground_truth, l_slt, noise, count)

    def _fwd_bwd_exact(self, model_input, ground_truth, l_slt, noise=None, count=None):
        model_input = dict(model_input)
        if not self.light_train:
            pass
        elif l_slt.is_cuda and self.light_para.weight.is_cuda:
            d_, i_ = ops.LightRows.apply(self.light_para.weight, self.light_inten_para.weight, l_slt.long())
            model_input['light_direction'] = d_
            if self.light_inten_train:
                model_input['light_intensity'] = i_
        else:
            model_input['light_direction'] = F.normalize(self.light_para(l_slt), p=2, dim=-1)
            if self.light_inten_train:
                model_input['light_intensity'] = self.light_inten_para(l_slt)
        if self.light_train and 'light_vis_train' not in model_input:
            if l_slt.is_cuda and self.light_vis_table.is_cuda:
                from .. import hip
                model_input['light_vis_train'] = hip.light_rows_fwd(self.light_vis_table.contiguous(), None, l_slt.long().contiguous())[0]
            else:
                model_input['light_vis_train'] = F.normalize(self.light_vis_table[l_slt], p=2, dim=-1)
        sm, om = model_input['surface_mask'], model_input['object_mask']
        if count is not None:
            pass
        elif self.FUSED_LOSSES and sm.is_cuda and self.normal_train:
            count = self.dp.masked_count_tensor(sm, om)
        else:
            if sm.is_cuda and torch.cuda.is_current_stream_capturing():
                raise RuntimeError('TrainStep: this configuration (no jointly trained normal net: train.normal_mlp / train.normal_joint off) takes the '
                                   'torch loss formulation, whose mask count is a host value -- the step cannot be captured into a HIP graph; run it eagerly')
            count = self.dp.global_count(sm & om)
        out = self.model(model_input, noise=noise)
        fl = fused_losses(self.loss, self.loss_n, out, ground_truth, model_input, count) if (self.FUSED_LOSSES and self.normal_train) else None
        if fl is None and self.FUSED_LOSSES and self.normal_train:
            ops.fallback('stage2 losses -> torch formulation of MainLoss / NormalLoss', out['sg_rgb_values'], 'loss type or outputs outside csrc/loss.hip')
        if fl is None and torch.is_tensor(count):
            count = int(count.item())
        if fl is not None:
            loss, terms, terms_n = fl
            terms = dict(terms)
        elif not self.normal_train:
            terms = dict(self.loss(out, ground_truth, model_input, count=count))
            terms_n = {'loss': None, 'normal_loss': None, 'normal_smooth_loss': None}
            loss = terms['loss']
        else:
            terms = dict(self.loss(out, ground_truth, model_input, count=count))
            terms_n = self.loss_n(out, count=count)
            loss = terms['loss'] + terms_n['loss']
        train_light = self.light_para.weight.requires_grad
        trainable = None
        if self.dp.enabled:
            trainable = [p for p in self.model.parameters() if p.requires_grad] \
                + (([self.light_para.weight] + ([self.light_inten_para.weight] if self.light_inten_train else [])) if train_light else [])
            self.dp.prepare_grads(list(self.model.parameters()) + [self.light_para.weight, self.light_inten_para.weight])
        else:
            if isinstance(self.sg_optimizer, FlatAdam):
                self.sg_optimizer.attach_grads()
            else:
                self.sg_optimizer.zero_grad()
            if train_light:
                self.light_optimizer.zero_grad()
        if loss.requires_grad:
            seed = getattr(self, '_grad_seed', None)
            if seed is None or seed.device != loss.device or seed.shape != loss.shape:
                seed = self._grad_seed = torch.ones_like(loss)
            if self.wgrad_bf16x6:
                from .. import hip
                with hip.wgrad_precision(self.wgrad_mode):
                    loss.backward(seed)
            else:
                loss.backward(seed)
        if self.dp.enabled:
            self.dp.gather_grads(trainable)
        terms['total'] = loss
        terms['normal_loss'] = terms_n['normal_loss']
        return terms, out, trainable, train_light

    def _reduce(self, trainable):
        if self.dp.enabled:
            self.dp.allreduce_bucket(trainable)

    def _optimise(self, l_slt, trainable, train_light):
        self.sg_optimizer.step()
        if hasattr(self.model, 'invalidate_packs'):
            self.model.invalidate_packs(trainable_only=True)
        if train_light:
            self.light_optimizer.step(rows=l_slt)

    def _advance(self, train_light):
        self.cur_iter += 1
        self.sg_scheduler.step()
        if train_light and self.light_decay:
            self.light_scheduler.step()


def psnr(img1, img2, mask=None):
    if mask is not None:
        m = mask.to(torch.bool)[:, None]
        img1, img2 = torch.masked_select(img1, m).view(-1, 3), torch.masked_select(img2, m).view(-1, 3)
    mse = ((img1 - img2) ** 2).mean()
    return 100.0 if mse == 0 else float(-10.0 * torch.log10(mse))


def mae_error(img1, img2, mask=None, normalize=True):
    if mask is not None:
        m = mask.to(torch.bool)[:, None]
        img1, img2 = torch.masked_select(img1, m).view(-1, 3), torch.masked_select(img2, m).view(-1, 3)
    if normalize:
        img1, img2 = F.normalize(img1, dim=-1), F.normalize(img2, dim=-1)
    err = torch.acos((img1 * img2).sum(-1).clamp(-1, 1)) * 180.0 / np.pi
    return err.mean(), err


@torch.no_grad()
def validate_view(model, model_input, rgb_gt, pixel_chunk=None):
    from .relight import merge_output, split_input
    n = model_input['uv'].shape[1]
    chunks = [model_input] if pixel_chunk is None else split_input(model_input, n, pixel_chunk)
    res = [{k: v.detach() for k, v in model(s).items() if torch.is_tensor(v)} for s in chunks]
    out = merge_output(res, n, 1) if len(res) > 1 else {k: (v.reshape(-1) if v.dim() < 3 else v.reshape(-1, v.shape[-1])) for k, v in res[0].items()}
    mask = torch.logical_and(out['network_object_mask'], out['object_mask'])
    rep = {'psnr': psnr(rgb_gt.to(out['sg_rgb_values'].device), out['sg_rgb_values'], mask), 'outputs': out}
    if 'normal_pred' in out and 'gt_normal' in model_input:
        mae, err = mae_error(model_input['gt_normal'][0], out['normal_pred'], mask)
        emap = torch.zeros_like(out['normal_pred'][..., 0])
        emap[mask] = err
        rep['normal_MAE'], rep['normal_mae'] = float(mae), emap
    return rep
```

Before: 112.2 million.

## Fuse RGB/vis loss gradients into SG shade backward and overlap dense scatter on side stream

Adds a fused SG shading backward kernel that computes the per-row RGB and visibility loss gradients inline from surface rows, masks and ground truth. This removes the dense-image loss-gradient round trip into shade backward. The dense scatter of outputs and the loss forward move to a side stream so they can overlap with the main stream. Separately, the pair-group sums kernel is rewritten with templated V, a fixed block count with a chunk walk, double-buffered row loads and a single batched LDS reduction. The changes add stream-synchronisation complexity and a stricter code path that raises if the fused losses do not take the step.

```diff
diff --git a/include/psnerf_hip.h b/include/psnerf_hip.h
--- a/include/psnerf_hip.h
+++ b/include/psnerf_hip.h
@@ -382,6 +382,14 @@
                      const float* vis, int L, int64_t Ns, int nb, int specular_rgb, const float* g_rgb,
                      const float* g_spec, float* d_albedo, float* d_weights, float* d_normal, float* d_vis,
                      float* d_light_dir, float* d_light_int, float* workspace, void* stream);
+int psn_sg_shade_loss_bwd(const float* light_dir, const float* view, const float* normal, const float* albedo,
+                          const float* weights, const float* lobe, const float* light_int, int int_ch, float light_int_scalar,
+                          const float* vis, int L, int64_t Ns, int nb, int specular_rgb, const float* rgb_rows,
+                          const float* rgb_gt, const int64_t* surface_idx, const unsigned char* mask_a,
+                          const unsigned char* mask_b, int64_t P, const float* g_total, const float* count_dev,
+                          const float* live_count, float k_rgb, int l2, const float* g_spec, const float* vis_t_rows,
+                          const float* vis_gt, int V, float k_vis, float* g_vis, float* d_albedo, float* d_weights,
+                          float* d_normal, float* d_vis, float* d_light_dir, float* d_light_int, float* workspace, void* stream);
 
 int psn_mf_shade_fwd(const float* light_dir, const float* view, const float* normal, const float* albedo,
                      const float* rough, const float* light_int, float light_int_scalar, float f0, const float* vis,
diff --git a/psnerf_amd/csrc/common.h b/psnerf_amd/csrc/common.h
--- a/psnerf_amd/csrc/common.h
+++ b/psnerf_amd/csrc/common.h
@@ -110,4 +110,10 @@
     return x >= 0.0f ? r : u * r;
 }
 
+__device__ __forceinline__ float img_term(float a, float b, int l2) { const float d = a - b; return l2 ? d * d : fabsf(d); }
+__device__ __forceinline__ float img_grad(float a, float b, int l2) {
+    const float d = a - b;
+    return l2 ? 2.0f * d : (d > 0.0f ? 1.0f : (d < 0.0f ? -1.0f : 0.0f));
 }
+
+}
diff --git a/psnerf_amd/csrc/loss.hip b/psnerf_amd/csrc/loss.hip
--- a/psnerf_amd/csrc/loss.hip
+++ b/psnerf_amd/csrc/loss.hip
@@ -18,12 +18,6 @@
     float* d_rgb; float* d_alb; float* d_alb_j; float* d_wgt; float* d_wgt_j; float* d_vis; float* d_nrm; float* d_nrm_j;
 };
 
-__device__ __forceinline__ float img_term(float a, float b, int l2) { const float d = a - b; return l2 ? d * d : fabsf(d); }
-__device__ __forceinline__ float img_grad(float a, float b, int l2) {
-    const float d = a - b;
-    return l2 ? 2.0f * d : (d > 0.0f ? 1.0f : (d < 0.0f ? -1.0f : 0.0f));
-}
-
 __global__ __launch_bounds__(256) void stage2_loss_fwd_kernel(LossArgs a) {
     float s[6] = {0.f, 0.f, 0.f, 0.f, 0.f, 0.f};
     const int lc = (a.L + gridDim.y - 1) / gridDim.y;
@@ -126,44 +120,68 @@
 
 struct PairGroupArgs { PsnPairSumsItem it[PSN_PAIR_GROUP_MAX]; int V; int64_t Ns; int C; int rows_per_block; int chunks; float* part;
                        const float* pe_l; int64_t ld_pe; int n_pe; int64_t ld_w;
-                       int slices; float* part2; };
+                       int slices; float* part2;
+                       int walk; };
+template <int MAXV, bool FULL>
 __global__ __launch_bounds__(256) void pair_group_sums_kernel(PairGroupArgs a) {
     const PsnPairSumsItem it = a.it[blockIdx.y];
-    const int V = a.V, C = a.C;
+    const int V = FULL ? MAXV : a.V, C = a.C, rows = a.rows_per_block;
     const int64_t Ns = a.Ns;
     const int cg = threadIdx.x & 63, rl = threadIdx.x >> 6;
-    const int64_t n0 = (int64_t)blockIdx.x * a.rows_per_block, n1 = min(Ns, n0 + a.rows_per_block);
     const bool live = 4 * cg < C;
-    float4 sl[PSN_PAIR_SUMS_MAX_V];
-#pragma unroll
-    for (int v = 0; v < PSN_PAIR_SUMS_MAX_V; ++v) sl[v] = make_float4(0.f, 0.f, 0.f, 0.f);
-    if (live) {
-        for (int64_t n = n0 + rl; n < n1; n += 4) {
-            float4 acc = make_float4(0.f, 0.f, 0.f, 0.f);
-#pragma unroll
-            for (int v = 0; v < PSN_PAIR_SUMS_MAX_V; ++v) {
-                if (v < V) {
-                    const float4 t = *reinterpret_cast<const float4*>(it.x + ((int64_t)v * Ns + n) * C + 4 * cg);
-                    acc.x += t.x; acc.y += t.y; acc.z += t.z; acc.w += t.w;
-                    sl[v].x += t.x; sl[v].y += t.y; sl[v].z += t.z; sl[v].w += t.w;
+    const float* __restrict__ x = it.x + (live ? 4 * cg : 0);
+    float* __restrict__ sx = it.sx + 4 * cg;
+    const int ch0 = blockIdx.x * a.walk, ch1 = min(a.chunks, ch0 + a.walk);
+    const int iters = rows / 4;
+    __shared__ float4 red[3][MAXV][64];
+    float4 sl[MAXV], ra[MAXV], rb[MAXV];
+    auto load_row = [&](int64_t n, float4 (&t)[MAXV]) {
+        const float* p = x + min(n, Ns - 1) * C;
+#pragma unroll
+        for (int v = 0; v < MAXV; ++v)
+            if (FULL || v < V) t[v] = *reinterpret_cast<const float4*>(p + (int64_t)v * Ns * C);
+    };
+    auto step = [&](int ch, int i, float4 (&cur)[MAXV], float4 (&nxt)[MAXV]) {
+        const int64_t n = (int64_t)ch * rows + rl + 4 * i;
+        load_row(i + 1 < iters ? n + 4 : ch + 1 < ch1 ? (int64_t)(ch + 1) * rows + rl : n, nxt);
+        const bool has = n < Ns;
+        float4 acc = make_float4(0.f, 0.f, 0.f, 0.f);
+#pragma unroll
+        for (int v = 0; v < MAXV; ++v) {
+            if (FULL || v < V) {
+                float4 t = cur[v];
+                t.x = has ? t.x : 0.f; t.y = has ? t.y : 0.f; t.z = has ? t.z : 0.f; t.w = has ? t.w : 0.f;
+                acc.x += t.x; acc.y += t.y; acc.z += t.z; acc.w += t.w;
+                sl[v].x += t.x; sl[v].y += t.y; sl[v].z += t.z; sl[v].w += t.w;
+            }
+        }
+        if (has && live) *reinterpret_cast<float4*>(sx + n * C) = acc;
+    };
+    load_row((int64_t)ch0 * rows + rl, ra);
+    for (int ch = ch0; ch < ch1; ++ch) {
+#pragma unroll
+        for (int v = 0; v < MAXV; ++v) sl[v] = make_float4(0.f, 0.f, 0.f, 0.f);
+        for (int i = 0; i < iters; i += 2) {
+            step(ch, i, ra, rb);
+            step(ch, i + 1, rb, ra);
+        }
+        __syncthreads();
+        if (rl > 0) {
+#pragma unroll
+            for (int v = 0; v < MAXV; ++v)
+                if (FULL || v < V) red[rl - 1][v][cg] = sl[v];
+        }
+        __syncthreads();
+        if (rl == 0 && live) {
+            float* dst = a.part + (((int64_t)blockIdx.y * a.chunks + ch) * V) * C + 4 * cg;
+#pragma unroll
+            for (int v = 0; v < MAXV; ++v) {
+                if (FULL || v < V) {
+                    float4 t = sl[v];
+#pragma unroll
+                    for (int q = 0; q < 3; ++q) { const float4 o = red[q][v][cg]; t.x += o.x; t.y += o.y; t.z += o.z; t.w += o.w; }
+                    *reinterpret_cast<float4*>(dst + (int64_t)v * C) = t;
                 }
-            }
-            *reinterpret_cast<float4*>(it.sx + n * C + 4 * cg) = acc;
-        }
-    }
-    __shared__ float4 red[3][64];
-    float* dst = a.part + (((int64_t)blockIdx.y * a.chunks + blockIdx.x) * V) * C;
-#pragma unroll
-    for (int v = 0; v < PSN_PAIR_SUMS_MAX_V; ++v) {
-        if (v < V) {
-            __syncthreads();
-            if (rl > 0) red[rl - 1][cg] = sl[v];
-            __syncthreads();
-            if (rl == 0 && live) {
-                float4 t = sl[v];
-#pragma unroll
-                for (int q = 0; q < 3; ++q) { const float4 o = red[q][cg]; t.x += o.x; t.y += o.y; t.z += o.z; t.w += o.w; }
-                *reinterpret_cast<float4*>(dst + (int64_t)v * C + 4 * cg) = t;
             }
         }
     }
@@ -403,6 +421,7 @@
     return row_adam_impl(n_items, items, idx, n_idx, step_sizes_dev, stream);
 }
 
+constexpr int kPairSumsBlocks = 768;
 constexpr int kPairSlices = 32;
 
 extern "C" int64_t psn_pair_sums_group_workspace(int n_items, int V, int64_t Ns, int C) {
@@ -430,7 +449,11 @@
     a.pe_l = pe_l; a.ld_pe = ld_pe; a.n_pe = n_pe; a.ld_w = ld_w;
     PSN_CHECK_ARG((((uintptr_t)workspace) & 15) == 0, "pair_sums_group: workspace must be 16-byte aligned");
     if (chunks > 0) {
-        hipLaunchKernelGGL(pair_group_sums_kernel, dim3((unsigned)chunks, n_items), dim3(256), 0, (hipStream_t)stream, a);
+        a.walk = (int)((chunks * n_items + kPairSumsBlocks - 1) / kPairSumsBlocks);
+        const dim3 grid((unsigned)((chunks + a.walk - 1) / a.walk), n_items);
+        if (V == 8) hipLaunchKernelGGL((pair_group_sums_kernel<8, true>), grid, dim3(256), 0, (hipStream_t)stream, a);
+        else if (V < 8) hipLaunchKernelGGL((pair_group_sums_kernel<8, false>), grid, dim3(256), 0, (hipStream_t)stream, a);
+        else hipLaunchKernelGGL((pair_group_sums_kernel<PSN_PAIR_SUMS_MAX_V, false>), grid, dim3(256), 0, (hipStream_t)stream, a);
         PSN_CHECK_LAUNCH("pair_sums_group (sums)");
     }
     if (chunks > 128) {
diff --git a/psnerf_amd/csrc/shade.hip b/psnerf_amd/csrc/shade.hip
--- a/psnerf_amd/csrc/shade.hip
+++ b/psnerf_amd/csrc/shade.hip
@@ -125,11 +125,26 @@
     (void)sc;
 }
 
-__global__ __launch_bounds__(kShadeThreads * kSgPhases) void sg_shade_bwd_kernel(ShadeArgs a, const float* __restrict__ g_rgb,
-                                                           const float* __restrict__ g_spec,
-                                                           float* __restrict__ d_albedo, float* __restrict__ d_weights,
-                                                           float* __restrict__ d_normal, float* __restrict__ d_vis,
-                                                           float* __restrict__ d_light_partial) {
+struct RowLossArgs {
+    const float* rgb_rows;
+    const float* rgb_gt;
+    const int64_t* surface_idx;
+    const unsigned char* mask_a; const unsigned char* mask_b;
+    const float* g_total;
+    const float* count_dev;
+    const float* live_count;
+    float k_rgb, k_vis;
+    int l2;
+    int64_t P;
+    const float* vis_t_rows; const float* vis_gt; int V; float* g_vis;
+};
+
+template <bool LOSS>
+__device__ __forceinline__ void sg_shade_bwd_body(const ShadeArgs& a, const RowLossArgs& r, const float* __restrict__ g_rgb,
+                                                  const float* __restrict__ g_spec,
+                                                  float* __restrict__ d_albedo, float* __restrict__ d_weights,
+                                                  float* __restrict__ d_normal, float* __restrict__ d_vis,
+                                                  float* __restrict__ d_light_partial) {
     const int64_t n = (int64_t)blockIdx.x * kShadeThreads + (threadIdx.x & (kShadeThreads - 1));
     const int phase = threadIdx.x / kShadeThreads;
     const bool ok = n < a.Ns;
@@ -137,6 +152,27 @@
     PointCtx p;
     load_point(a, n, ok, p);
     const bool has_vis = a.vis != nullptr;
+    bool m = false;
+    int64_t pix = 0;
+    float k_rgb = 0.f;
+    if (LOSS) {
+        float g = r.g_total[0];
+        if (r.count_dev != nullptr) {
+            const float cnt = r.count_dev[0];
+            g = cnt > 0.0f ? g / cnt : 0.0f;
+        }
+        k_rgb = g * r.k_rgb;
+        if (ok && (r.live_count == nullptr || n < (int64_t)r.live_count[0])) {
+            pix = r.surface_idx[n];
+            const bool first = n == 0 || r.surface_idx[n - 1] != pix;
+            m = first && r.mask_a[pix] && r.mask_b[pix];
+        }
+        const float k_vis = g * r.k_vis;
+        if (ok) {
+            for (int v = phase; v < r.V; v += kSgPhases)
+                r.g_vis[(int64_t)v * a.Ns + n] = m ? k_vis * img_grad(r.vis_t_rows[(int64_t)v * a.Ns + n], r.vis_gt[(int64_t)v * r.P + pix], r.l2) : 0.f;
+        }
+    }
     float dalb[3] = {0.f, 0.f, 0.f}, dn[3] = {0.f, 0.f, 0.f};
     float dw[3][kMaxBasis];
 #pragma unroll
@@ -158,7 +194,9 @@
         if (ok) {
 #pragma unroll
             for (int c = 0; c < 3; ++c) {
-                float g = g_rgb[row * 3 + c];
+                float g;
+                if (LOSS) g = m ? k_rgb * img_grad(r.rgb_rows[row * 3 + c], r.rgb_gt[((int64_t)l * r.P + pix) * 3 + c], r.l2) : 0.f;
+                else g = g_rgb[row * 3 + c];
                 float gp = (f.pre[c] >= 0.0f && f.pre[c] <= 1.0f) ? g : 0.0f;
                 float dbrdf = gp * I[c] * f.cosv * f.vcl;
                 dI += gp * f.brdf[c] * f.cosv * f.vcl;
@@ -242,6 +280,22 @@
             }
         }
     }
+}
+
+__global__ __launch_bounds__(kShadeThreads * kSgPhases) void sg_shade_bwd_kernel(ShadeArgs a, const float* __restrict__ g_rgb,
+                                                           const float* __restrict__ g_spec,
+                                                           float* __restrict__ d_albedo, float* __restrict__ d_weights,
+                                                           float* __restrict__ d_normal, float* __restrict__ d_vis,
+                                                           float* __restrict__ d_light_partial) {
+    sg_shade_bwd_body<false>(a, RowLossArgs{}, g_rgb, g_spec, d_albedo, d_weights, d_normal, d_vis, d_light_partial);
+}
+
+__global__ __launch_bounds__(kShadeThreads * kSgPhases) void sg_shade_loss_bwd_kernel(ShadeArgs a, RowLossArgs r,
+                                                           const float* __restrict__ g_spec,
+                                                           float* __restrict__ d_albedo, float* __restrict__ d_weights,
+                                                           float* __restrict__ d_normal, float* __restrict__ d_vis,
+                                                           float* __restrict__ d_light_partial) {
+    sg_shade_bwd_body<true>(a, r, nullptr, g_spec, d_albedo, d_weights, d_normal, d_vis, d_light_partial);
 }
 
 __global__ __launch_bounds__(256) void sg_light_reduce_kernel(const float* __restrict__ partial, int n_blocks, int L,
@@ -557,6 +611,38 @@
     return PSN_OK;
 }
 
+extern "C" int psn_sg_shade_loss_bwd(const float* light_dir, const float* view, const float* normal, const float* albedo,
+                                     const float* weights, const float* lobe, const float* light_int, int int_ch,
+                                     float light_int_scalar, const float* vis, int L, int64_t Ns, int nb, int specular_rgb,
+                                     const float* rgb_rows, const float* rgb_gt, const int64_t* surface_idx,
+                                     const unsigned char* mask_a, const unsigned char* mask_b, int64_t P, const float* g_total,
+                                     const float* count_dev, const float* live_count, float k_rgb, int l2, const float* g_spec,
+                                     const float* vis_t_rows, const float* vis_gt, int V, float k_vis, float* g_vis,
+                                     float* d_albedo, float* d_weights, float* d_normal, float* d_vis, float* d_light_dir,
+                                     float* d_light_int, float* workspace, void* stream) {
+    using namespace psn;
+    ShadeArgs a;
+    int rc = fill_args(a, light_dir, view, normal, albedo, weights, lobe, light_int, int_ch, light_int_scalar, vis, L, Ns, nb, specular_rgb);
+    if (rc) return rc;
+    PSN_CHECK_ARG(rgb_rows && rgb_gt && surface_idx && mask_a && mask_b && g_total && d_albedo && d_weights && d_normal && d_light_dir &&
+                  workspace, "sg_shade_loss_bwd: null pointer");
+    PSN_CHECK_ARG(P >= 1 && V >= 0 && (V == 0 || (vis_t_rows && vis_gt && g_vis)), "sg_shade_loss_bwd: P=%lld V=%d", (long long)P, V);
+    PSN_CHECK_ARG(int_ch == 1 || d_light_int == nullptr, "sg_shade_loss_bwd: RGB light intensities have no intensity gradient");
+    if (Ns == 0) return PSN_OK;
+    RowLossArgs r = {};
+    r.rgb_rows = rgb_rows; r.rgb_gt = rgb_gt; r.surface_idx = surface_idx; r.mask_a = mask_a; r.mask_b = mask_b; r.g_total = g_total;
+    r.count_dev = count_dev; r.live_count = live_count; r.k_rgb = k_rgb; r.k_vis = k_vis; r.l2 = l2 ? 1 : 0; r.P = P;
+    r.vis_t_rows = vis_t_rows; r.vis_gt = vis_gt; r.V = V; r.g_vis = g_vis;
+    const int n_blocks = (int)((Ns + kShadeThreads - 1) / kShadeThreads);
+    hipLaunchKernelGGL(sg_shade_loss_bwd_kernel, dim3(n_blocks), dim3(kShadeThreads * kSgPhases), 0, (hipStream_t)stream, a, r, g_spec,
+                       d_albedo, d_weights, d_normal, d_vis, workspace);
+    PSN_CHECK_LAUNCH("sg_shade_loss_bwd");
+    hipLaunchKernelGGL(sg_light_reduce_kernel, dim3((L * 4 + 63) / 64), dim3(256), 0, (hipStream_t)stream, workspace,
+                       n_blocks, L, d_light_dir, d_light_int);
+    PSN_CHECK_LAUNCH("sg_shade_loss_bwd light reduce");
+    return PSN_OK;
+}
+
 extern "C" int psn_mf_shade_fwd(const float* light_dir, const float* view, const float* normal, const float* albedo,
                                 const float* rough, const float* light_int, float light_int_scalar, float f0,
                                 const float* vis, int L, int64_t Ns, float* rgb, void* stream) {
diff --git a/psnerf_amd/hip.py b/psnerf_amd/hip.py
--- a/psnerf_amd/hip.py
+++ b/psnerf_amd/hip.py
@@ -1237,6 +1237,41 @@
     return d_albedo, d_weights, d_normal, d_vis, d_ldir, d_lint
 
 
+def sg_shade_loss_bwd(light_dir, view, normal, albedo, weights, lobe, light_int, light_int_scalar, vis, specular_rgb,
+                      rgb_rows, rgb_gt, surface_idx, mask_a, mask_b, g_total, k_rgb, l2, count_dev=None, live_count=None,
+                      g_spec=None, vis_t_rows=None, vis_gt=None, k_vis=0.0, want_vis=False):
+    L, Ns, nb = light_dir.shape[0], view.shape[0], lobe.shape[0]
+    dev = view.device
+    P = mask_a.numel()
+    V = 0 if vis_t_rows is None else vis_gt.shape[0]
+    int_ch = 1 if light_int is None or light_int.dim() == 1 else light_int.shape[1]
+    assert rgb_rows.shape == (L * Ns, 3) and rgb_gt.shape == (L, P, 3) and surface_idx.shape == (Ns,) and mask_b.numel() == P
+    assert V == 0 or (vis_t_rows.numel() == V * Ns and vis_gt.shape == (V, P))
+    d_albedo = torch.empty(Ns, 3, device=dev)
+    d_weights = torch.empty_like(weights)
+    d_normal = torch.empty(Ns, 3, device=dev)
+    d_vis = torch.empty(L * Ns, device=dev) if want_vis else None
+    d_ldir = torch.empty(L, 3, device=dev)
+    d_lint = torch.empty(L, device=dev) if (light_int is not None and int_ch == 1) else None
+    g_vis = torch.empty(V * Ns, device=dev) if V else None
+    if Ns == 0:
+        return d_albedo, d_weights, d_normal, d_vis, torch.zeros_like(d_ldir), None if d_lint is None else torch.zeros_like(d_lint), g_vis
+    ws = workspace(((Ns + 63) // 64) * L * 4, dev)
+    f = lambda t, name: _tptr(t, name, allow_none=True)
+    _check(_lib.psn_sg_shade_loss_bwd(_tptr(light_dir, 'light_dir'), _tptr(view, 'view'), _tptr(normal, 'normal'),
+                                      _tptr(albedo, 'albedo'), _tptr(weights, 'weights'), _tptr(lobe, 'lobe'),
+                                      f(light_int, 'light_int'), int_ch, float(light_int_scalar), f(vis, 'vis'),
+                                      L, Ns, nb, int(bool(specular_rgb)), _tptr(rgb_rows, 'rgb_rows'), _tptr(rgb_gt, 'rgb_gt'),
+                                      _tptr(surface_idx, 'surface_idx', torch.int64), _tptr(mask_a, 'mask_a', torch.bool),
+                                      _tptr(mask_b, 'mask_b', torch.bool), P, _tptr(g_total, 'g_total'), f(count_dev, 'count_dev'),
+                                      f(live_count, 'live_count'), float(k_rgb), int(l2), f(g_spec, 'g_spec'),
+                                      f(vis_t_rows, 'vis_t_rows'), f(vis_gt, 'vis_gt'), V, float(k_vis), f(g_vis, 'g_vis'),
+                                      _tptr(d_albedo, 'd_albedo'), _tptr(d_weights, 'd_weights'), _tptr(d_normal, 'd_normal'),
+                                      f(d_vis, 'd_vis'), _tptr(d_ldir, 'd_ldir'), f(d_lint, 'd_lint'), ws.data_ptr(), _stream()),
+           'sg_shade_loss_bwd')
+    return d_albedo, d_weights, d_normal, d_vis, d_ldir, d_lint, g_vis
+
+
 def mf_shade_fwd(light_dir, view, normal, albedo, rough, light_int, light_int_scalar, f0, vis):
     L, Ns = light_dir.shape[0], view.shape[0]
     rgb = torch.empty(L * Ns, 3, device=view.device, dtype=torch.float32)
diff --git a/psnerf_amd/ops.py b/psnerf_amd/ops.py
--- a/psnerf_amd/ops.py
+++ b/psnerf_amd/ops.py
@@ -348,6 +348,69 @@
         if d_vis is not None:
             d_vis = d_vis.reshape(ctx.vis_shape)
         return d_ld, None, d_n, d_alb, d_w, None, d_li, d_vis, None
+
+
+class RowsLoss(object):
+
+    def __init__(self):
+        self.anchor = None
+        self.bound = False
+        self.stream = None
+
+    def bind(self, rgb_gt, vis_gt, mask_a, mask_b, k_rgb, k_vis, l2, count_dev):
+        self.rgb_gt, self.vis_gt, self.mask_a, self.mask_b = rgb_gt, vis_gt, mask_a, mask_b
+        self.k_rgb, self.k_vis, self.l2, self.count_dev = float(k_rgb), float(k_vis), int(l2), count_dev
+        self.bound = True
+
+
+class SGShadeLossRows(torch.autograd.Function):
+
+    @staticmethod
+    def forward(ctx, box, light_dir, view, normal, albedo, weights, lobe, light_int, vis, specular_rgb, vis_t, idx, live_count):
+        _hit('SGShade')
+        li_t, li_s = None, 0.0
+        if torch.is_tensor(light_int):
+            if light_int.dim() == 2 and light_int.shape[1] == 3:
+                raise RuntimeError('SGShadeLossRows: RGB light intensities are supported on the forward-only path')
+            li_t = light_int.reshape(-1).contiguous() if light_int.numel() > 1 else light_int.reshape(-1).expand(light_dir.shape[0]).contiguous()
+        else:
+            li_s = float(light_int)
+        vis_f = None if vis is None else vis.detach().reshape(-1).contiguous()
+        args = (light_dir.contiguous(), view.contiguous(), normal.contiguous(), albedo.contiguous(), weights.contiguous(), lobe.contiguous())
+        rgb, spec = hip.sg_shade_fwd(*args, li_t, li_s, vis_f, specular_rgb)
+        vt = vis_t.detach().reshape(-1).contiguous()
+        ctx.save_for_backward(*args, rgb, vt, idx.contiguous(), *([li_t] if li_t is not None else []), *([vis_f] if vis_f is not None else []),
+                              *([live_count] if live_count is not None else []))
+        ctx.has_li, ctx.has_vis, ctx.has_live, ctx.li_s, ctx.specular_rgb = li_t is not None, vis_f is not None, live_count is not None, li_s, specular_rgb
+        ctx.li_shape = light_int.shape if torch.is_tensor(light_int) else None
+        ctx.vt_shape, ctx.box = vis_t.shape, box
+        ctx.set_materialize_grads(False)
+        ctx.mark_non_differentiable(rgb, spec)
+        return rgb, spec, rgb.new_empty(1)
+
+    @staticmethod
+    def backward(ctx, _g_rgb, _g_spec, g_total):
+        box = ctx.box
+        if g_total is None:
+            return (None,) * 13
+        if not box.bound:
+            raise RuntimeError('SGShadeLossRows: the loss of this step was not bound (stage2.loss.fused_losses(..., rows=box))')
+        sv = list(ctx.saved_tensors)
+        light_dir, view, normal, albedo, weights, lobe, rgb, vt, idx = sv[:9]
+        rest = sv[9:]
+        li_t = rest.pop(0) if ctx.has_li else None
+        vis_f = rest.pop(0) if ctx.has_vis else None
+        live = rest.pop(0) if ctx.has_live else None
+        sup = box.vis_gt is not None and box.k_vis != 0.0 and ctx.needs_input_grad[10]
+        d_alb, d_w, d_n, _, d_ld, d_li, g_vis = hip.sg_shade_loss_bwd(
+            light_dir, view, normal, albedo, weights, lobe, li_t, ctx.li_s, vis_f, ctx.specular_rgb, rgb, box.rgb_gt, idx,
+            box.mask_a, box.mask_b, g_total.reshape(1).contiguous(), box.k_rgb, box.l2, count_dev=box.count_dev, live_count=live,
+            vis_t_rows=vt if sup else None, vis_gt=box.vis_gt if sup else None, k_vis=box.k_vis if sup else 0.0)
+        if d_li is not None:
+            d_li = d_li.sum().reshape(ctx.li_shape) if int(torch.tensor(ctx.li_shape).prod()) == 1 else d_li.reshape(ctx.li_shape)
+        if g_vis is not None:
+            g_vis = g_vis.reshape(ctx.vt_shape)
+        return None, d_ld, None, d_n, d_alb, d_w, None, d_li, None, None, g_vis, None, None
 
 
 def _buf(rows, cols, device):
@@ -939,6 +1002,17 @@
                 None, None, None, None, None, None)
 
 
+class JoinTotal(torch.autograd.Function):
+
+    @staticmethod
+    def forward(ctx, total, anchor):
+        return total.view_as(total)
+
+    @staticmethod
+    def backward(ctx, g):
+        return g, g.reshape(1)
+
+
 class SurfaceNormals(torch.autograd.Function):
 
     @staticmethod
diff --git a/psnerf_amd/stage2/loss.py b/psnerf_amd/stage2/loss.py
--- a/psnerf_amd/stage2/loss.py
+++ b/psnerf_amd/stage2/loss.py
@@ -1,3 +1,5 @@
+import contextlib
+
 import torch
 from torch import nn
 from torch.nn import functional as F
@@ -93,7 +95,12 @@
         return {'loss': loss, 'normal_loss': n_loss, 'normal_smooth_loss': s_loss}
 
 
-def fused_losses(main, normal, model_outputs, ground_truth, model_input, count):
+def fused_applies(main, model_input):
+    sm, om = model_input['surface_mask'], model_input['object_mask']
+    return sm.is_cuda and sm.dtype == torch.bool and om.dtype == torch.bool and main.loss_type in ('L1', 'L2')
+
+
+def fused_losses(main, normal, model_outputs, ground_truth, model_input, count, rows=None):
     from .. import ops
     o = model_outputs
     need = ('sg_rgb_values', 'normal_pred', 'normal_values', 'network_object_mask', 'object_mask')
@@ -131,8 +138,14 @@
     w = [float(main.sg_rgb_weight), float(main.albedo_smooth_weight) if alb is not None else 0.0,
          float(main.rough_smooth_weight) if wgt is not None else 0.0, float(main.vis_weight) if vis is not None else 0.0,
          float(normal.normal_weight), float(normal.normal_smooth_weight) if nrm_j is not None else 0.0]
-    total, t = ops.Stage2Losses.apply(rgb, rgb_gt, alb, alb_j, wgt, wgt_j, vis, vis_gt, nrm, nrm_gt, nrm_j, ma, mb,
-                                      1 if main.loss_type == 'L2' else 0, inv, w, count_dev)
+    with (torch.cuda.stream(rows.stream) if (rows is not None and rows.stream is not None) else contextlib.nullcontext()):
+        total, t = ops.Stage2Losses.apply(rgb, rgb_gt, alb, alb_j, wgt, wgt_j, vis, vis_gt, nrm, nrm_gt, nrm_j, ma, mb,
+                                          1 if main.loss_type == 'L2' else 0, inv, w, count_dev)
+    if rows is not None:
+        k_vis = w[3] * inv[3] if (vis is not None and 'vis_train' in o and vis is o['vis_train']) else 0.0
+        rows.bind(rgb_gt.contiguous(), None if k_vis == 0.0 else vis_gt.contiguous(), ma.contiguous(), mb.contiguous(), w[0] * inv[0], k_vis,
+                  1 if main.loss_type == 'L2' else 0, count_dev)
+        total = ops.JoinTotal.apply(total, rows.anchor)
     terms = {'sg_rgb_loss': t[0], 'albedo_smooth_loss': t[1] if alb is not None else None,
              'rough_smooth_loss': t[2] if wgt is not None else None, 'loss': total}
     if has_vis:
diff --git a/psnerf_amd/stage2/renderer.py b/psnerf_amd/stage2/renderer.py
--- a/psnerf_amd/stage2/renderer.py
+++ b/psnerf_amd/stage2/renderer.py
@@ -254,6 +254,9 @@
             a, pre = self._visibility_pair_args(pe_x, light_dir, light_vis_train), None
         return ops.VisibilityPair.apply(a[0], a[1], a[2], a[3], a[4], pre, *a[5])
 
+    loss_on_rows = False
+    _rows_loss = None
+
     def forward(self, input, albedo_new=None, basis_new=None, noise=None):
         noise = noise or {}
         uv, pose, intr = input['uv'], input['pose'], input['intrinsics']
@@ -283,6 +286,8 @@
         vis_pair = None
         vis_bf16 = None
         side = None
+        post = None
+        self._rows_loss = None
         pair_ok = False
         if ns > 0 and self.visibility:
             lv0 = input.get('light_vis_train')
@@ -403,7 +408,19 @@
                 else:
                     vis = self._visibility_rows(pe_x, light_dir, fused_ok=True)
                 vis_for_rgb = vis.detach() if detach else vis
-            if sg:
+            if (sg and self.loss_on_rows and pair_ok and vis_t_pre is not None and idx.is_cuda and idx.dtype == torch.int64
+                    and not (torch.is_tensor(light_int) and light_int.dim() == 2 and light_int.shape[1] == 3)):
+                self._rows_loss = ops.RowsLoss()
+                rgb, spec, self._rows_loss.anchor = ops.SGShadeLossRows.apply(
+                    self._rows_loss, light_dir, pts2c, normal, albedo, weights, self.sgbasis.lobe, light_int, vis_for_rgb, self.specular_rgb,
+                    vis_t_pre, idx, input.get('surface_count'))
+                vis_t_pre = vis_t_pre.detach()
+                if side is not None:
+                    shaded = torch.cuda.Event()
+                    shaded.record(torch.cuda.current_stream(device))
+                    side.wait_event(shaded)
+                    post = self._rows_loss.stream = side
+            elif sg:
                 rgb, spec = ops.sg_shade(light_dir, pts2c, normal, albedo, weights, self.sgbasis.lobe, light_int,
                                          vis_for_rgb, self.specular_rgb)
             else:
@@ -465,19 +482,23 @@
                 lazy[id(v)] = v
         with_rows = [v for v in lazy.values() if v.rows is not None]
         done = {}
-        if with_rows:
-            if idx.is_cuda and idx.dtype == torch.int64:
-                inv = hip.inverse_index(idx.contiguous(), n_pix, count=input.get('surface_count'))
-            else:
-                inv = torch.full((n_pix,), -1, dtype=torch.int32, device=device)
-                inv[idx] = torch.arange(ns, dtype=torch.int32, device=device)
-            specs = tuple((v.B, v.C, v.fill) for v in with_rows)
-            dense = ops.ScatterRows.apply(idx, inv, specs, *[v.rows for v in with_rows])
-            for v, d in zip(with_rows, dense):
-                done[id(v)] = d
-        for v in lazy.values():
-            if v.rows is None:
-                done[id(v)] = torch.full((v.B, n_pix, v.C), v.fill, device=device)
+        with (torch.cuda.stream(post) if post is not None else contextlib.nullcontext()):
+            if with_rows:
+                if idx.is_cuda and idx.dtype == torch.int64:
+                    inv = hip.inverse_index(idx.contiguous(), n_pix, count=input.get('surface_count'))
+                else:
+                    inv = torch.full((n_pix,), -1, dtype=torch.int32, device=device)
+                    inv[idx] = torch.arange(ns, dtype=torch.int32, device=device)
+                specs = tuple((v.B, v.C, v.fill) for v in with_rows)
+                dense = ops.ScatterRows.apply(idx, inv, specs, *[v.rows for v in with_rows])
+                for v, d in zip(with_rows, dense):
+                    done[id(v)] = d
+                if post is not None:
+                    for v in with_rows:
+                        v.rows.record_stream(post)
+            for v in lazy.values():
+                if v.rows is None:
+                    done[id(v)] = torch.full((v.B, n_pix, v.C), v.fill, device=device)
         for k in list(out.keys()):
             if isinstance(out[k], _Dense):
                 out[k] = done[id(out[k])]
diff --git a/psnerf_amd/stage2/trainer.py b/psnerf_amd/stage2/trainer.py
--- a/psnerf_amd/stage2/trainer.py
+++ b/psnerf_amd/stage2/trainer.py
@@ -6,7 +6,7 @@
 from ..dist import DataParallel
 from .. import ops
 from ..optim import FlatAdam, RowSparseAdam
-from .loss import MainLoss, NormalLoss, fused_losses
+from .loss import MainLoss, NormalLoss, fused_applies, fused_losses
 
 
 class VisPlus(object):
@@ -173,8 +173,17 @@
                 raise RuntimeError('TrainStep: this configuration (no jointly trained normal net: train.normal_mlp / train.normal_joint off) takes the '
                                    'torch loss formulation, whose mask count is a host value -- the step cannot be captured into a HIP graph; run it eagerly')
             count = self.dp.global_count(sm & om)
-        out = self.model(model_input, noise=noise)
-        fl = fused_losses(self.loss, self.loss_n, out, ground_truth, model_input, count) if (self.FUSED_LOSSES and self.normal_train) else None
+        fuse = self.FUSED_LOSSES and self.normal_train
+        self.model.loss_on_rows = bool(fuse and fused_applies(self.loss, model_input))
+        self.model._rows_loss = None
+        try:
+            out = self.model(model_input, noise=noise)
+        finally:
+            self.model.loss_on_rows = False
+        rows, self.model._rows_loss = self.model._rows_loss, None
+        fl = fused_losses(self.loss, self.loss_n, out, ground_truth, model_input, count, rows=rows) if fuse else None
+        if fl is None and rows is not None:
+            raise RuntimeError('TrainStep: the model formed its loss gradients on the surface rows, but the fused losses do not take this step')
         if fl is None and self.FUSED_LOSSES and self.normal_train:
             ops.fallback('stage2 losses -> torch formulation of MainLoss / NormalLoss', out['sg_rgb_values'], 'loss type or outputs outside csrc/loss.hip')
         if fl is None and torch.is_tensor(count):
@@ -213,6 +222,12 @@
                     loss.backward(seed)
             else:
                 loss.backward(seed)
+        if rows is not None and rows.stream is not None:
+            main = torch.cuda.current_stream(loss.device)
+            main.wait_stream(rows.stream)
+            for t_ in list(out.values()) + list(terms.values()) + list(terms_n.values()):
+                if torch.is_tensor(t_):
+                    t_.record_stream(main)
         if self.dp.enabled:
             self.dp.gather_grads(trainable)
         terms['total'] = loss
```

After: 112.5 million, median of 6. About the same (+0.3%).
